# IlzeAmandaA/VAE-GP-ODE

Measured on AMD Instinct MI355X. Metric: latent_trajectories_per_sec, higher is better.
Workload: dtype f32; 1 GPU; configs[1]: ode1 DF q=6 M=100 S=256 T=16 batch=256; step = full ELBO training step (encoder, GP draw, rk4 rollout, decoder, ELBO, backward, Adam), L=1; global_batch=256, mc_draws=1, solver=rk4 (3/8 rule), parallelism=dp1, hip_graph=True, graph_scope=whole, gp_side_stream=True, batchnorm=per-process statistics

## Files before the change

### include/gpode.h

```cpp
#ifndef GPODE_H
#define GPODE_H
#include <stddef.h>
#ifdef __cplusplus
extern "C" {
#endif

#define GPODE_KERNEL_RBF 0
#define GPODE_KERNEL_DF 1
#define GPODE_METHOD_EULER 0
#define GPODE_METHOD_RK4 1
#define GPODE_METHOD_MIDPOINT 2
#define GPODE_METHOD_DOPRI5 3

const char* gpode_version(void);
const char* gpode_last_error(void);
const char* gpode_last_launch(void);
int gpode_supported(int kernel, int Di, int Do);

int gpode_cache_sizes(int kernel, int Di, int Do, int M, int S, size_t* pack_floats, size_t* ws_floats);

int gpode_cache_build_fwd(int kernel, int Di, int Do, int M, int S,
                          const float* raw_ell, const float* raw_var, const float* Z,
                          const float* Um, const float* Us_packed,
                          const float* eps_u, const float* rff_w, const float* rff_eps, const float* rff_u,
// ... 95 lines not shown
                              const float* pack, const float* xstage, const float* gzt, const float* ts, int N, int T,
                              float* gz0, float* astage, float* slab, int nchunk, float* gpack, void* stream);
int gpode_param_grad_n(int kernel, int Di, int Do, int M, int S, int ndraws, const float* pack,
                       const float* x, const float* a, int R, float* slab, int nchunk, float* gpack, int accumulate,
                       void* stream);
int gpode_cache_bwd_sizes_n(int kernel, int Di, int Do, int M, int S, int ndraws, size_t* bws_floats);
int gpode_cache_build_bwd_n(int kernel, int Di, int Do, int M, int S, int ndraws,
                            const float* raw_ell, const float* raw_var, const float* Z, const float* eps_u,
                            const float* pack, const float* ws, float* gpack, float* bws,
                            float* g_raw_ell, float* g_raw_var, float* g_Z, float* g_Um, float* g_Us, int prepared, void* stream);
int gpode_cache_bwd_prepare_n(int kernel, int Di, int Do, int M, int S, int ndraws, const float* ws, float* bws, void* stream);

int gpode_cache_info(const float* ws, int* host_info, void* stream);
int gpode_cache_pivots(const float* ws, float* host_min_max, void* stream);
int gpode_set_backward_solves(int mode);

int gpode_kernel_matrix(int kernel, int Di, int Do, const float* raw_ell, const float* raw_var,
                        const float* X, int N, const float* X2, int M2, float* out, void* stream);

size_t gpode_kern_scratch(int kernel, int Di, int Do, int M, int S);
int gpode_kern_cache(int kernel, int Di, int Do, int S, const float* raw_ell, const float* raw_var, const float* rff_w,
                     const float* rff_eps, const float* rff_u, float* pack, float* omega, float* phase, void* stream);
int gpode_compute_nu_ws(int kernel, int Di, int Do, int M, size_t* ws_floats);
int gpode_compute_nu(int kernel, int Di, int Do, int M, const float* Ku, const float* u_prior, const float* u, float* nu, float* ws,
                     void* stream);
int gpode_f_update(int kernel, int Di, int Do, int M, const float* raw_ell, const float* raw_var, const float* x2, const float* nu,
                   const float* x, int N, float* out, float* scratch, void* stream);

int gpode_conditional_ws(int Di, int Do, int M, int N, size_t* ws_floats);
int gpode_conditional(int Di, int Do, int M, int N, const float* raw_ell, const float* raw_var, const float* Z,
                      const float* Um, const float* Us, int us_rank1, const float* x, int full_cov, float* mean,
                      float* var, float* ws, void* stream);

int gpode_conditional_df_ws(int D, int M, int N, size_t* ws_floats);
int gpode_conditional_df(int D, int M, int N, const float* raw_ell, const float* raw_var, const float* Z, const float* Um,
                         const float* Us_packed, const float* x, int cov_mode, float* mean, float* var, float* ws,
                         void* stream);

int gpode_svgp_kl_fwd(int M, int Do, const float* Um, const float* Us_packed, float* kl, void* stream);
int gpode_svgp_kl_bwd(int M, int Do, const float* Um, const float* Us_packed, const float* g,
                      float* dUm, float* dUs, void* stream);

int gpode_conv2d_fwd(const float* x, const float* w, const float* bias, float* y, int B, int Ci, int H, int W, int Co,
                     int K, int S, int P, int Ho, int Wo, void* stream);
int gpode_conv2d_bwd_data(const float* gy, const float* w, const float* bias, float* gx, int B, int Ci, int H, int W, int Co,
                          int K, int S, int P, int Ho, int Wo, void* stream);
int gpode_conv2d_bwd_data_bn(const float* gy, const float* gy_bn, const float* w, const float* bias, float* gx, int B, int Ci, int H,
                             int W, int Co, int K, int S, int P, int Ho, int Wo, void* stream);
int gpode_conv2d_fwd_bs(const float* x, size_t x_batch_stride, const float* w, const float* bias, float* y, int B, int Ci, int H, int W, int Co,
                        int K, int S, int P, int Ho, int Wo, void* stream);
int gpode_conv2d_bwd_weight_bs(const float* x, size_t x_batch_stride, const float* gy, float* gw, float* gbias, float* scratch, int B, int Ci,
                               int H, int W, int Co, int K, int S, int P, int Ho, int Wo, void* stream);
size_t gpode_convT_fwd_stats_scratch(int Cout);
int gpode_convT_fwd_stats(const float* x, const float* x_bn, const float* w, const float* bias, float* y, int B, int Ci, int H, int W, int Co,
                          int K, int S, int P, int Ho, int Wo, const float* gamma, const float* beta, float* save_mean, float* save_invstd,
                          float* running_mean, float* running_var, long long* num_batches_tracked, float momentum, float eps, float* table,
                          float* scratch, int slot, void* stream);
size_t gpode_conv_wgrad_scratch(int B, int Ci, int Co, int K);
int gpode_conv2d_bwd_weight(const float* x, const float* gy, float* gw, float* gbias, float* scratch, int B, int Ci, int H, int W,
                            int Co, int K, int S, int P, int Ho, int Wo, void* stream);
int gpode_conv2d_bwd_weight_bn(const float* x, const float* gy, const float* gy_bn, float* gw, float* gbias, float* scratch, int B, int Ci,
                               int H, int W, int Co, int K, int S, int P, int Ho, int Wo, void* stream);
size_t gpode_bn_scratch(int B, int C);
int gpode_bn_fwd(const float* x, const float* gamma, const float* beta, float* y, float* save_mean, float* save_invstd,
                 float* running_mean, float* running_var, long long* num_batches_tracked, float momentum, float eps, int B, int C,
                 int HW, int relu, float* scratch, void* stream);
int gpode_bn_bwd(const float* x, const float* gy, const float* gamma, const float* beta, const float* save_mean,
                 const float* save_invstd, float* gx, float* ggamma, float* gbeta, float* gx_chansum, int B, int C, int HW,
                 int relu, float* scratch, void* stream);
int gpode_bn_stats(const float* x, const float* gamma, const float* beta, float* save_mean, float* save_invstd, float* running_mean,
                   float* running_var, long long* num_batches_tracked, float momentum, float eps, float* table, int B, int C, int HW,
                   float* scratch, void* stream);
int gpode_bn_moments(const float* x, float* moments, int B, int C, int HW, float* scratch, void* stream);
int gpode_bn_finalize(const float* gathered, int nranks, const float* gamma, const float* beta, float* save_mean, float* save_invstd,
                      float* running_mean, float* running_var, long long* num_batches_tracked, float momentum, float eps, float* table,
                      int C, void* stream);
int gpode_bn_apply(const float* x, const float* table, float* y, int B, int C, int HW, int relu, void* stream);
int gpode_bn_bwd_sums(const float* x, const float* gy, const float* gamma, const float* beta, const float* save_mean,
                      const float* save_invstd, float* sums, int B, int C, int HW, int relu, float* scratch, void* stream);
int gpode_bn_bwd_apply(const float* x, const float* gy, const float* gamma, const float* beta, const float* save_mean,
                       const float* save_invstd, const float* sums_gathered, const float* weights, int nranks, float count_all,
                       float* gx, float* ggamma, float* gbeta, float* gx_chansum, int B, int C, int HW, int relu, float* scratch,
                       void* stream);
void gpode_defer_reductions(int mode);
int gpode_flush_reductions(void* stream);
int gpode_dec10_bn_wgrad_scratch_floats(void);
int gpode_dec10_bn_bwd_sums_wgrad(const float* c, const float* gy, const float* w, const float* gamma, const float* beta, const float* save_mean,
                                  const float* save_invstd, float* sums, float* gw, float* gbias, int B, float* scratch, float* wscratch,
                                  void* stream);
int gpode_dec10_bn_scratch_floats(void);
int gpode_dec10_bn_bwd_sums(const float* c, const float* gy, const float* w, const float* gamma, const float* beta, const float* save_mean,
                            const float* save_invstd, float* sums, int B, float* scratch, void* stream);
int gpode_dec10_bn_bwd_apply(const float* c, const float* gy, const float* w, const float* gamma, const float* beta, const float* save_mean,
                             const float* save_invstd, const float* sums_gathered, const float* weights, int nranks, float count_all,
                             float* gc, float* ggamma, float* gbeta, float* gc_chansum, int B, float* scratch, void* stream);
int gpode_bn_eval(const float* x, const float* gy, const float* gamma, const float* beta, const float* running_mean,
                  const float* running_var, float eps, float* out, int B, int C, int HW, int relu, void* stream);
int gpode_bn_eval_table(const float* gamma, const float* beta, const float* running_mean, const float* running_var, float eps, float* table,
                        int C, void* stream);
int gpode_dec10_predict(const float* c, const float* table, const float* w, const float* bias, const float* X, int Lc, int F, int Th,
                        int T_obs, int done, float* pred_mean, float* pred_m2, float* se_state, void* stream);
int gpode_dec10_predict_ll(const float* c, const float* table, const float* w, const float* bias, const float* X, int Lc, int F, int Th,
                           int T_obs, int done, float* pred_mean, float* pred_m2, float* se_state, float* ell, int L_total, void* stream);
int gpode_dec10_predict_len(const float* c, const float* table, const float* w, const float* bias, const float* X, int Lc, int F, int Th,
                            int T_obs, int done, float* pred_mean, float* pred_m2, float* se_state, const int* n_obs, void* stream);
int gpode_dec10_predict_ll_len(const float* c, const float* table, const float* w, const float* bias, const float* X, int Lc, int F, int Th,
                               int T_obs, int done, float* pred_mean, float* pred_m2, float* se_state, float* ell, int L_total,
                               const int* n_obs, void* stream);
int gpode_chan_sum(const float* v, float* out, int B, int C, int HW, float* scratch, void* stream);
int gpode_act_fwd(const float* x, float* y, size_t n, int mode, void* stream);
int gpode_act_bwd(const float* y, const float* gy, float* gx, size_t n, int mode, void* stream);
int gpode_linear_fwd(const float* x, const float* w, const float* bias, float* y, int B, int In, int Out, void* stream);
size_t gpode_linear_bwd_scratch(int B, int In, int Out);
int gpode_linear_bwd(const float* x, const float* w, const float* gy, float* gx, float* gw, float* gb, int B, int In, int Out,
                     float* scratch, void* stream);
int gpode_linear_relu_fwd(const float* x, const float* w, const float* bias, float* y, int B, int In, int Out, void* stream);
int gpode_linear_relu_bwd(const float* x, const float* w, const float* gy, float* gx, float* gw, float* gb, int B, int In, int Out,
                          void* stream);

int gpode_loglik_fwd(const float* X, const float* z, float* ll, size_t n, size_t nX, void* stream);
int gpode_loglik_bwd(const float* X, const float* z, const float* g, float* gz, size_t n, size_t nX, void* stream);
int gpode_loglik_rowsum_fwd(const float* X, const float* z, float* out, size_t rows, size_t inner, size_t nX, void* stream);
int gpode_loglik_rowsum_bwd(const float* X, const float* z, const float* grow, float* gz, size_t rows, size_t inner, size_t nX,
                            void* stream);

int gpode_loglik_rowsum_fwd_len(const float* X, const float* z, float* out, size_t rows, size_t inner, size_t nX, const int* n_obs, int T,
                                size_t frame, void* stream);
int gpode_loglik_rowsum_bwd_len(const float* X, const float* z, const float* grow, float* gz, size_t rows, size_t inner, size_t nX,
                                const int* n_obs, int T, size_t frame, void* stream);

int gpode_sigmoid_loglik_splits(size_t rows, size_t inner);
int gpode_sigmoid_loglik_fwd(const float* X, const float* a, float* z, float* part, size_t rows, size_t inner, size_t nX, int nsplit,
                             void* stream);
int gpode_sigmoid_loglik_bwd(const float* X, const float* z, const float* grow, float* ga, size_t rows, size_t inner, size_t nX,
                             void* stream);
int gpode_elbo_all_fwd(const float* lpart, int nl_rows, int nl_values, const float* hs, const float* hv, int N, int q, int M, int Do,
                       const float* Um, const float* Us, float nobs, float* out, void* stream);
int gpode_elbo_all_bwd(const float* g_loss, const float* g_nll, const float* g_kl, const float* g_klu, int nl_rows, const float* hs,
                       const float* hv, int N, int q, int M, int Do, const float* Um, const float* Us, float nobs, float* glrow, float* ghs,
                       float* ghv, float* dUm, float* dUs, void* stream);
int gpode_elbo_all_bwd_ll(const float* g_loss, const float* g_nll, const float* g_kl, const float* g_klu, int nl_rows, const float* hs,
                          const float* hv, int N, int q, int M, int Do, const float* Um, const float* Us, float nobs, float* glrow, float* ghs,
                          float* ghv, float* dUm, float* dUs, const float* X, const float* z, float* ga, size_t n_logits, size_t nX,
                          void* stream);
int gpode_sigmoid_loglik_fwd_len(const float* X, const float* a, float* z, float* part, size_t rows, size_t inner, size_t nX, int nsplit,
                                 const int* n_obs, int T, size_t frame, void* stream);
int gpode_sigmoid_loglik_bwd_len(const float* X, const float* z, const float* grow, float* ga, size_t rows, size_t inner, size_t nX,
                                 const int* n_obs, int T, size_t frame, void* stream);
int gpode_elbo_all_bwd_ll_len(const float* g_loss, const float* g_nll, const float* g_kl, const float* g_klu, int nl_rows, const float* hs,
                              const float* hv, int N, int q, int M, int Do, const float* Um, const float* Us, float nobs, float* glrow, float* ghs,
                              float* ghv, float* dUm, float* dUs, const float* X, const float* z, float* ga, size_t n_logits, size_t nX,
                              const int* n_obs, int T, size_t frame, void* stream);
int gpode_gather_frames_fwd(const float* zt, int ld, int q, const int* src, int L, int N, int T, int P, float* out, void* stream);
int gpode_gather_frames_bwd(const float* gout, int ld, int q, const int* src, const int* off, int L, int N, int T, int P, float* gzt,
                            void* stream);
int gpode_sigmoid_loglik_fwd_pk(const float* X, const float* a, float* z, float* part, size_t rows, const int* off, int T, size_t frame,
                                size_t nX, int nsplit, void* stream);
int gpode_sigmoid_loglik_bwd_pk(const float* X, const float* z, const float* grow, float* ga, size_t rows, const int* src, int P, int T,
                                size_t frame, size_t nX, void* stream);
int gpode_noise_fill(float* out, long long n_normal, long long n_uniform, unsigned long long seed, unsigned long long* state, void* stream);
int gpode_reparam_kl_fwd(const float* mu, const float* logvar, int ld, const float* eps, float* z, float* klpart, int N, int q, void* stream);
int gpode_reparam_kl_bwd(const float* gz, const float* gklpart, const float* mu, const float* logvar, int ld, const float* eps, float* gmu,
                         float* glogvar, int ldg, int N, int q, void* stream);
int gpode_elbo_all_fwd_kl(const float* lpart, int nl_rows, int nl_values, const float* kls, int nks, const float* klv, int nkv, int N, int M,
                          int Do, const float* Um, const float* Us, float nobs, float* out, void* stream);
int gpode_elbo_all_bwd_ll_kl(const float* g_loss, const float* g_nll, const float* g_kl, const float* g_klu, int nl_rows, int N, int M, int Do,
// ... 27 lines not shown
```

### vae-gp-ode_amd/_lib.py

```python
import ctypes
import os

_HERE = os.path.dirname(os.path.abspath(__file__))
LIB_PATH = os.path.join(_HERE, 'libgpode_hip.so')

_vp = ctypes.c_void_p
_i = ctypes.c_int
_f = ctypes.c_float
_sz = ctypes.c_size_t
_sz_p = ctypes.POINTER(_sz)

SIGNATURES = {
    'gpode_version': (ctypes.c_char_p, []),
    'gpode_last_error': (ctypes.c_char_p, []),
    'gpode_last_launch': (ctypes.c_char_p, []),
    'gpode_supported': (_i, [_i, _i, _i]),
    'gpode_cache_sizes': (_i, [_i, _i, _i, _i, _i, _sz_p, _sz_p]),
    'gpode_cache_build_fwd': (_i, [_i] * 5 + [_vp] * 20),
    'gpode_cache_bwd_sizes': (_i, [_i, _i, _i, _i, _i, _sz_p]),
    'gpode_cache_build_bwd': (_i, [_i] * 5 + [_vp] * 13 + [_i, _vp]),
    'gpode_cache_bwd_prepare': (_i, [_i] * 5 + [_vp] * 2 + [_vp]),
    'gpode_cache_info': (_i, [_vp, ctypes.POINTER(_i), _vp]),
    'gpode_cache_pivots': (_i, [_vp, ctypes.POINTER(_f), _vp]),
    'gpode_set_backward_solves': (_i, [_i]),
    'gpode_kernel_matrix': (_i, [_i, _i, _i, _vp, _vp, _vp, _i, _vp, _i, _vp, _vp]),
    'gpode_conditional_ws': (_i, [_i, _i, _i, _i, _sz_p]),
    'gpode_conditional': (_i, [_i, _i, _i, _i] + [_vp] * 5 + [_i, _vp, _i] + [_vp] * 3 + [_vp]),
    'gpode_conditional_df_ws': (_i, [_i, _i, _i, _sz_p]),
    'gpode_conditional_df': (_i, [_i, _i, _i] + [_vp] * 6 + [_i] + [_vp] * 3 + [_vp]),
    'gpode_svgp_kl_fwd': (_i, [_i, _i, _vp, _vp, _vp, _vp]),
    'gpode_svgp_kl_bwd': (_i, [_i, _i] + [_vp] * 5 + [_vp]),
    'gpode_rhs_fwd': (_i, [_i] * 5 + [_vp, _vp, _i, _vp, _i, _vp]),
    'gpode_rollout_fwd': (_i, [_i] * 7 + [_vp, _vp, _vp, _i, _i, _vp, _vp, _vp]),
    'gpode_rollout_bwd': (_i, [_i] * 7 + [_vp] * 4 + [_i, _i, _vp, _vp, _vp]),
    'gpode_rhs_vjp': (_i, [_i] * 5 + [_vp, _vp, _vp, _i, _vp, _vp]),
    'gpode_param_grad': (_i, [_i] * 5 + [_vp, _vp, _vp, _i, _vp, _i, _vp, _i, _vp]),
    'gpode_cache_sizes_n': (_i, [_i] * 6 + [_sz_p, _sz_p]),
    'gpode_cache_build_fwd_n': (_i, [_i] * 6 + [_vp] * 20),
    'gpode_rollout_fwd_n': (_i, [_i] * 8 + [_vp, _vp, _vp, _i, _i, _vp, _vp, _vp]),
    'gpode_rollout_bwd_n': (_i, [_i] * 8 + [_vp] * 4 + [_i, _i, _vp, _vp, _vp]),
    'gpode_rollout_adaptive_fwd_n': (_i, [_i] * 8 + [_vp] * 3 + [_i, _i, _f, _f, _i] + [_vp] * 5 + [_vp]),
    'gpode_rollout_adaptive_bwd_n': (_i, [_i] * 8 + [_vp] * 5 + [_i, _i, _i, _vp, _vp, _vp]),
    'gpode_rollout_dense_fwd_n': (_i, [_i] * 8 + [_vp] * 3 + [_i, _i, _f, _f, _i] + [_vp] * 6 + [_vp]),
    'gpode_rollout_dense_bwd_n': (_i, [_i] * 8 + [_vp] * 6 + [_i, _i, _i, _vp, _vp, _vp]),
    'gpode_rollout_fwd_nz': (_i, [_i] * 8 + [_vp, _vp, _vp, _i, _i, _vp, _vp, _i, _vp]),
    'gpode_rollout_adaptive_fwd_nz': (_i, [_i] * 8 + [_vp] * 3 + [_i, _i, _f, _f, _i] + [_vp] * 5 + [_i, _vp]),
    'gpode_rollout_dense_fwd_nz': (_i, [_i] * 8 + [_vp] * 3 + [_i, _i, _f, _f, _i] + [_vp] * 6 + [_i, _vp]),
    'gpode_rollout_fwd_nt': (_i, [_i] * 8 + [_vp, _vp, _vp, _i, _i, _vp, _vp, _i, _i, _vp]),
    'gpode_rollout_adaptive_fwd_nt': (_i, [_i] * 8 + [_vp] * 3 + [_i, _i, _f, _f, _i] + [_vp] * 5 + [_i, _i, _vp]),
    'gpode_rollout_dense_fwd_nt': (_i, [_i] * 8 + [_vp] * 3 + [_i, _i, _f, _f, _i] + [_vp] * 6 + [_i, _i, _vp]),
    'gpode_rollout_bwd_nt': (_i, [_i] * 8 + [_vp] * 4 + [_i, _i, _vp, _vp, _i, _vp]),
    'gpode_rollout_bwd_pgrad_nt': (_i, [_i] * 8 + [_vp] * 4 + [_i, _i, _vp, _vp, _vp, _i, _vp, _i, _vp]),
    'gpode_test_substep_kernels': (_i, [_i]),
    'gpode_rollout_fwd_ns': (_i, [_i] * 8 + [_vp, _vp, _vp, _i, _i, _vp, _vp, _i, _i, _i, _vp]),
    'gpode_rollout_bwd_ns': (_i, [_i] * 8 + [_vp] * 4 + [_i, _i, _vp, _vp, _i, _i, _vp]),
    'gpode_rollout_bwd_pgrad_ns': (_i, [_i] * 8 + [_vp] * 4 + [_i, _i, _vp, _vp, _vp, _i, _vp, _i, _i, _vp]),
    'gpode_rollout_bwd_pgrad_chunks': (_i, [_i] * 8),
    'gpode_rollout_bwd_pgrad_n': (_i, [_i] * 8 + [_vp] * 4 + [_i, _i, _vp, _vp, _vp, _i, _vp, _vp]),
    'gpode_param_grad_n': (_i, [_i] * 6 + [_vp, _vp, _vp, _i, _vp, _i, _vp, _i, _vp]),
    'gpode_cache_bwd_sizes_n': (_i, [_i] * 6 + [_sz_p]),
    'gpode_cache_build_bwd_n': (_i, [_i] * 6 + [_vp] * 13 + [_i, _vp]),
    'gpode_cache_bwd_prepare_n': (_i, [_i] * 6 + [_vp] * 2 + [_vp]),
    'gpode_kern_scratch': (_sz, [_i] * 5),
    'gpode_kern_cache': (_i, [_i] * 4 + [_vp] * 8 + [_vp]),
    'gpode_compute_nu_ws': (_i, [_i] * 4 + [_sz_p]),
    'gpode_compute_nu': (_i, [_i] * 4 + [_vp] * 5 + [_vp]),
    'gpode_f_update': (_i, [_i] * 4 + [_vp] * 5 + [_i, _vp, _vp, _vp]),
    'gpode_conv2d_fwd': (_i, [_vp] * 4 + [_i] * 10 + [_vp]),
    'gpode_conv2d_bwd_data': (_i, [_vp] * 4 + [_i] * 10 + [_vp]),
    'gpode_conv2d_fwd_bs': (_i, [_vp, _sz] + [_vp] * 3 + [_i] * 10 + [_vp]),
    'gpode_conv2d_bwd_weight_bs': (_i, [_vp, _sz] + [_vp] * 4 + [_i] * 10 + [_vp]),
    'gpode_convT_fwd_stats_scratch': (_sz, [_i]),
    'gpode_convT_fwd_stats': (_i, [_vp] * 5 + [_i] * 10 + [_vp] * 6 + [_vp, _f, _f, _vp, _vp, _i, _vp]),
    'gpode_conv_wgrad_scratch': (_sz, [_i, _i, _i, _i]),
    'gpode_conv2d_bwd_weight': (_i, [_vp] * 5 + [_i] * 10 + [_vp]),
    'gpode_bn_scratch': (_sz, [_i, _i]),
    'gpode_bn_fwd': (_i, [_vp] * 8 + [_vp, _f, _f, _i, _i, _i, _i, _vp, _vp]),
    'gpode_bn_bwd': (_i, [_vp] * 10 + [_i, _i, _i, _i, _vp, _vp]),
    'gpode_conv2d_bwd_data_bn': (_i, [_vp] * 5 + [_i] * 10 + [_vp]),
    'gpode_conv2d_bwd_weight_bn': (_i, [_vp] * 6 + [_i] * 10 + [_vp]),
    'gpode_bn_stats': (_i, [_vp] * 7 + [_vp, _f, _f, _vp, _i, _i, _i, _vp, _vp]),
    'gpode_bn_moments': (_i, [_vp, _vp, _i, _i, _i, _vp, _vp]),
    'gpode_bn_finalize': (_i, [_vp, _i] + [_vp] * 6 + [_vp, _f, _f, _vp, _i, _vp]),
    'gpode_bn_apply': (_i, [_vp, _vp, _vp, _i, _i, _i, _i, _vp]),
    'gpode_bn_bwd_sums': (_i, [_vp] * 7 + [_i, _i, _i, _i, _vp, _vp]),
    'gpode_bn_bwd_apply': (_i, [_vp] * 8 + [_i, _f] + [_vp] * 4 + [_i, _i, _i, _i, _vp, _vp]),
    'gpode_defer_reductions': (None, [_i]),
    'gpode_flush_reductions': (_i, [_vp]),
    'gpode_dec10_bn_scratch_floats': (_i, []),
    'gpode_dec10_bn_wgrad_scratch_floats': (_i, []),
    'gpode_dec10_bn_bwd_sums_wgrad': (_i, [_vp] * 10 + [_i, _vp, _vp, _vp]),
    'gpode_dec10_bn_bwd_sums': (_i, [_vp] * 8 + [_i, _vp, _vp]),
    'gpode_dec10_bn_bwd_apply': (_i, [_vp] * 9 + [_i, _f] + [_vp] * 4 + [_i, _vp, _vp]),
    'gpode_bn_eval': (_i, [_vp] * 6 + [_f, _vp, _i, _i, _i, _i, _vp]),
    'gpode_bn_eval_table': (_i, [_vp] * 4 + [_f, _vp, _i, _vp]),
    'gpode_dec10_predict': (_i, [_vp] * 5 + [_i] * 5 + [_vp] * 3 + [_vp]),
    'gpode_dec10_predict_ll': (_i, [_vp] * 5 + [_i] * 5 + [_vp] * 4 + [_i, _vp]),
    'gpode_chan_sum': (_i, [_vp, _vp, _i, _i, _i, _vp, _vp]),
    'gpode_act_fwd': (_i, [_vp, _vp, _sz, _i, _vp]),
    'gpode_act_bwd': (_i, [_vp, _vp, _vp, _sz, _i, _vp]),
    'gpode_linear_fwd': (_i, [_vp] * 4 + [_i, _i, _i, _vp]),
    'gpode_linear_bwd_scratch': (_sz, [_i, _i, _i]),
    'gpode_linear_bwd': (_i, [_vp] * 6 + [_i, _i, _i, _vp, _vp]),
    'gpode_linear_relu_fwd': (_i, [_vp] * 4 + [_i, _i, _i, _vp]),
    'gpode_linear_relu_bwd': (_i, [_vp] * 6 + [_i, _i, _i, _vp]),
    'gpode_loglik_fwd': (_i, [_vp] * 3 + [_sz, _sz, _vp]),
    'gpode_loglik_bwd': (_i, [_vp] * 4 + [_sz, _sz, _vp]),
    'gpode_loglik_rowsum_fwd': (_i, [_vp] * 3 + [_sz, _sz, _sz, _vp]),
    'gpode_noise_fill': (_i, [_vp, ctypes.c_longlong, ctypes.c_longlong, ctypes.c_ulonglong, _vp, _vp]),
    'gpode_reparam_kl_fwd': (_i, [_vp, _vp, _i, _vp, _vp, _vp, _i, _i, _vp]),
    'gpode_reparam_kl_bwd': (_i, [_vp] * 4 + [_i] + [_vp] * 3 + [_i, _i, _i, _vp]),
    'gpode_elbo_all_fwd_kl': (_i, [_vp, _i, _i, _vp, _i, _vp, _i, _i, _i, _i, _vp, _vp, _f, _vp, _vp]),
    'gpode_elbo_all_bwd_ll_kl': (_i, [_vp] * 4 + [_i, _i, _i, _i, _vp, _vp, _f, _vp, _vp, _i, _vp, _i] + [_vp] * 5 + [_sz, _sz, _vp]),
    'gpode_reparam_fwd': (_i, [_vp, _vp, _i, _vp, _vp, _i, _i, _vp]),
    'gpode_reparam_draws_fwd': (_i, [_vp, _vp, _i, _vp, _vp, _i, _vp, _i, _i, _i, _i, _vp]),
    'gpode_reparam_bwd': (_i, [_vp, _vp, _i, _vp, _vp, _vp, _i, _i, _i, _vp]),
    'gpode_normal_kl_fwd': (_i, [_vp, _vp, _i, _vp, _i, _i, _vp]),
    'gpode_normal_kl_bwd': (_i, [_vp, _vp, _vp, _i, _vp, _vp, _i, _i, _i, _vp]),
    'gpode_sigmoid_loglik_splits': (_i, [_sz, _sz]),
    'gpode_sigmoid_loglik_fwd': (_i, [_vp] * 4 + [_sz, _sz, _sz, _i, _vp]),
    'gpode_sigmoid_loglik_bwd': (_i, [_vp] * 4 + [_sz, _sz, _sz, _vp]),
    'gpode_elbo_all_fwd': (_i, [_vp, _i, _i, _vp, _vp, _i, _i, _i, _i, _vp, _vp, _f, _vp, _vp]),
    'gpode_elbo_all_bwd': (_i, [_vp] * 4 + [_i, _vp, _vp, _i, _i, _i, _i, _vp, _vp, _f] + [_vp] * 5 + [_vp]),
    'gpode_elbo_all_bwd_ll': (_i, [_vp] * 4 + [_i, _vp, _vp, _i, _i, _i, _i, _vp, _vp, _f] + [_vp] * 8 + [_sz, _sz, _vp]),
    'gpode_elbo_fwd': (_i, [_vp, _i, _vp, _i, _vp, _f, _vp, _vp]),
    'gpode_elbo_bwd': (_i, [_vp, _i, _i, _f, _vp, _vp, _vp, _vp]),
    'gpode_gather_multi': (_i, [_vp, _vp, _i, ctypes.c_longlong, _vp, _vp]),
    'gpode_adam_multi': (_i, [_vp, _vp, _vp, _vp, _vp, _i, ctypes.c_longlong, _f, _f, _f, _f, _i, _vp, _vp]),
    'gpode_loglik_rowsum_bwd': (_i, [_vp] * 4 + [_sz, _sz, _sz, _vp]),
    'gpode_sigmoid_loglik_fwd_len': (_i, [_vp] * 4 + [_sz, _sz, _sz, _i, _vp, _i, _sz, _vp]),
    'gpode_sigmoid_loglik_bwd_len': (_i, [_vp] * 4 + [_sz, _sz, _sz, _vp, _i, _sz, _vp]),
    'gpode_loglik_rowsum_fwd_len': (_i, [_vp] * 3 + [_sz, _sz, _sz, _vp, _i, _sz, _vp]),
    'gpode_loglik_rowsum_bwd_len': (_i, [_vp] * 4 + [_sz, _sz, _sz, _vp, _i, _sz, _vp]),
    'gpode_elbo_all_bwd_ll_len': (_i, [_vp] * 4 + [_i, _vp, _vp, _i, _i, _i, _i, _vp, _vp, _f] + [_vp] * 8 + [_sz, _sz, _vp, _i, _sz, _vp]),
    'gpode_elbo_all_bwd_ll_kl_len': (_i, [_vp] * 4 + [_i, _i, _i, _i, _vp, _vp, _f, _vp, _vp, _i, _vp, _i] + [_vp] * 5 + [_sz, _sz, _vp, _i, _sz, _vp]),
    'gpode_gather_frames_fwd': (_i, [_vp, _i, _i, _vp, _i, _i, _i, _i, _vp, _vp]),
    'gpode_gather_frames_bwd': (_i, [_vp, _i, _i, _vp, _vp, _i, _i, _i, _i, _vp, _vp]),
    'gpode_sigmoid_loglik_fwd_pk': (_i, [_vp] * 4 + [_sz, _vp, _i, _sz, _sz, _i, _vp]),
    'gpode_sigmoid_loglik_bwd_pk': (_i, [_vp] * 4 + [_sz, _vp, _i, _i, _sz, _sz, _vp]),
    'gpode_dec10_predict_len': (_i, [_vp] * 5 + [_i] * 5 + [_vp] * 3 + [_vp, _vp]),
    'gpode_dec10_predict_ll_len': (_i, [_vp] * 5 + [_i] * 5 + [_vp] * 4 + [_i, _vp, _vp]),
}

_lib = None


class GpodeError(RuntimeError):
    pass


def load():
    global _lib
    if _lib is not None:
        return _lib
    if not os.path.exists(LIB_PATH):
        raise GpodeError('libgpode_hip.so not found at %s -- build the HIP extension first '
                         '(__graft_entry__.build()); there is no CPU fallback' % LIB_PATH)
    lib = ctypes.CDLL(LIB_PATH)
    for name, (res, args) in SIGNATURES.items():
        fn = getattr(lib, name)
        fn.restype = res
        fn.argtypes = args
    _lib = lib
    return lib


def call(name, *args):
    lib = load()
    rc = getattr(lib, name)(*args)
# ... 4 lines not shown
```

### vae-gp-ode_amd/csrc/bn_math.hpp

```cpp
#pragma once
#include <hip/hip_runtime.h>

namespace gp {

__device__ __forceinline__ float bn_xhat(float x, float m, float is) { return __fmul_rn(__fsub_rn(x, m), is); }
__device__ __forceinline__ float bn_affine(float x, float m, float is, float g, float b) { return __fmaf_rn(bn_xhat(x, m, is), g, b); }
__device__ __forceinline__ float bn_relu(float x, const float4& t) { return fmaxf(bn_affine(x, t.x, t.y, t.z, t.w), 0.f); }

}
```

### vae-gp-ode_amd/csrc/capi.hip

```cpp
#include "../../include/gpode.h"
#include "gp_launch.hpp"

namespace gp {
char* error_slot() {
  static thread_local char buf[512] = {0};
  return buf;
}
const char** last_launch_slot() {
  static thread_local const char* tag = "";
  return &tag;
}
bool* force_substep_kernels() {
  static bool on = false;
  return &on;
}
}

extern "C" {

const char* gpode_version(void) { return "gpode-hip 0.1 (gfx950)"; }
const char* gpode_last_error(void) { return gp::error_slot(); }
const char* gpode_last_launch(void) { return *gp::last_launch_slot(); }
int gpode_supported(int kernel, int Di, int Do) { return gp::dims_supported(kernel, Di, Do); }

// ... 447 lines not shown
  if (!x || !w || !y) return gp::set_error("gpode_conv2d_fwd_bs: null pointer");
  if (x_batch_stride < (size_t)Ci * H * W) return gp::set_error("gpode_conv2d_fwd_bs: images overlap");
  return gp::conv2d_fwd(x, w, bias, y, B, Ci, H, W, Co, K, S, P, Ho, Wo, GP_ST, x_batch_stride);
}
int gpode_conv2d_bwd_weight_bs(const float* x, size_t x_batch_stride, const float* gy, float* gw, float* gbias, float* scratch, int B, int Ci,
                               int H, int W, int Co, int K, int S, int P, int Ho, int Wo, void* stream) {
  if (!x || !gy || !gw || !scratch) return gp::set_error("gpode_conv2d_bwd_weight_bs: null pointer");
  if (x_batch_stride < (size_t)Ci * H * W) return gp::set_error("gpode_conv2d_bwd_weight_bs: images overlap");
  return gp::conv2d_bwd_weight(x, gy, gw, gbias, scratch, B, Ci, H, W, Co, K, S, P, Ho, Wo, nullptr, GP_ST, x_batch_stride);
}
size_t gpode_convT_fwd_stats_scratch(int Cout) { return gp::convT_fwd_stats_scratch(Cout); }
int gpode_convT_fwd_stats(const float* x, const float* x_bn, const float* w, const float* bias, float* y, int B, int Ci, int H, int W, int Co,
                          int K, int S, int P, int Ho, int Wo, const float* gamma, const float* beta, float* save_mean, float* save_invstd,
                          float* running_mean, float* running_var, long long* num_batches_tracked, float momentum, float eps, float* table,
                          float* scratch, int slot, void* stream) {
  if (!x || !w || !y || !gamma || !beta || !save_mean || !save_invstd || !table || !scratch)
    return gp::set_error("gpode_convT_fwd_stats: null pointer");
  if ((running_mean == nullptr) != (running_var == nullptr)) return gp::set_error("gpode_convT_fwd_stats: running_mean and running_var go together");
  return gp::convT_fwd_stats(x, x_bn, w, bias, y, B, Ci, H, W, Co, K, S, P, Ho, Wo, gamma, beta, save_mean, save_invstd, running_mean,
                             running_var, num_batches_tracked, momentum, eps, table, scratch, slot, GP_ST);
}
size_t gpode_conv_wgrad_scratch(int B, int Ci, int Co, int K) { return gp::conv_wgrad_scratch(B, Ci, Co, K); }
int gpode_conv2d_bwd_weight(const float* x, const float* gy, float* gw, float* gbias, float* scratch, int B, int Ci, int H, int W,
                            int Co, int K, int S, int P, int Ho, int Wo, void* stream) {
  if (!x || !gy || !gw || !scratch) return gp::set_error("gpode_conv2d_bwd_weight: null pointer");
  return gp::conv2d_bwd_weight(x, gy, gw, gbias, scratch, B, Ci, H, W, Co, K, S, P, Ho, Wo, nullptr, GP_ST);
}
int gpode_conv2d_bwd_weight_bn(const float* x, const float* gy, const float* gy_bn, float* gw, float* gbias, float* scratch, int B, int Ci,
                               int H, int W, int Co, int K, int S, int P, int Ho, int Wo, void* stream) {
  if (!x || !gy || !gy_bn || !gw || !scratch) return gp::set_error("gpode_conv2d_bwd_weight_bn: null pointer");
  return gp::conv2d_bwd_weight(x, gy, gw, gbias, scratch, B, Ci, H, W, Co, K, S, P, Ho, Wo, gy_bn, GP_ST);
}
size_t gpode_bn_scratch(int B, int C) { return gp::bn_scratch(B, C); }
int gpode_bn_fwd(const float* x, const float* gamma, const float* beta, float* y, float* save_mean, float* save_invstd,
                 float* running_mean, float* running_var, long long* num_batches_tracked, float momentum, float eps, int B, int C,
                 int HW, int relu, float* scratch, void* stream) {
  if (!x || !gamma || !beta || !y || !save_mean || !save_invstd || !scratch) return gp::set_error("gpode_bn_fwd: null pointer");
  return gp::bn_fwd(x, gamma, beta, y, save_mean, save_invstd, running_mean, running_var, num_batches_tracked, momentum, eps, B, C, HW, relu,
                    scratch, GP_ST);
}
int gpode_bn_bwd(const float* x, const float* gy, const float* gamma, const float* beta, const float* save_mean,
                 const float* save_invstd, float* gx, float* ggamma, float* gbeta, float* gx_chansum, int B, int C, int HW,
                 int relu, float* scratch, void* stream) {
  if (!x || !gy || !gamma || !beta || !save_mean || !save_invstd || !gx || !ggamma || !gbeta || !scratch)
    return gp::set_error("gpode_bn_bwd: null pointer");
  return gp::bn_bwd(x, gy, gamma, beta, save_mean, save_invstd, gx, ggamma, gbeta, gx_chansum, B, C, HW, relu, scratch, GP_ST);
}
int gpode_bn_stats(const float* x, const float* gamma, const float* beta, float* save_mean, float* save_invstd, float* running_mean,
                   float* running_var, long long* num_batches_tracked, float momentum, float eps, float* table, int B, int C, int HW,
                   float* scratch, void* stream) {
  if (!x || !gamma || !beta || !save_mean || !save_invstd || !table || !scratch) return gp::set_error("gpode_bn_stats: null pointer");
  return gp::bn_stats(x, gamma, beta, save_mean, save_invstd, running_mean, running_var, num_batches_tracked, momentum, eps, table, B, C, HW,
                      scratch, GP_ST);
}
int gpode_bn_moments(const float* x, float* moments, int B, int C, int HW, float* scratch, void* stream) {
  if (!x || !moments || !scratch) return gp::set_error("gpode_bn_moments: null pointer");
  return gp::bn_moments(x, moments, B, C, HW, scratch, GP_ST);
}
int gpode_bn_finalize(const float* gathered, int nranks, const float* gamma, const float* beta, float* save_mean, float* save_invstd,
                      float* running_mean, float* running_var, long long* num_batches_tracked, float momentum, float eps, float* table,
                      int C, void* stream) {
  if (!gathered || !gamma || !beta || !save_mean || !save_invstd || !table) return gp::set_error("gpode_bn_finalize: null pointer");
  return gp::bn_finalize(gathered, nranks, gamma, beta, save_mean, save_invstd, running_mean, running_var, num_batches_tracked, momentum, eps,
                         table, C, GP_ST);
}
int gpode_bn_apply(const float* x, const float* table, float* y, int B, int C, int HW, int relu, void* stream) {
  if (!x || !table || !y) return gp::set_error("gpode_bn_apply: null pointer");
  return gp::bn_apply(x, table, y, B, C, HW, relu, GP_ST);
}
int gpode_bn_bwd_sums(const float* x, const float* gy, const float* gamma, const float* beta, const float* save_mean,
                      const float* save_invstd, float* sums, int B, int C, int HW, int relu, float* scratch, void* stream) {
  if (!x || !gy || !gamma || !beta || !save_mean || !save_invstd || !sums || !scratch) return gp::set_error("gpode_bn_bwd_sums: null pointer");
  return gp::bn_bwd_sums(x, gy, gamma, beta, save_mean, save_invstd, sums, B, C, HW, relu, scratch, GP_ST);
}
int gpode_bn_bwd_apply(const float* x, const float* gy, const float* gamma, const float* beta, const float* save_mean,
                       const float* save_invstd, const float* sums_gathered, const float* weights, int nranks, float count_all,
                       float* gx, float* ggamma, float* gbeta, float* gx_chansum, int B, int C, int HW, int relu, float* scratch,
                       void* stream) {
  if (!x || !gy || !gamma || !beta || !save_mean || !save_invstd || !sums_gathered || !weights || !gx || !ggamma || !gbeta || !scratch)
    return gp::set_error("gpode_bn_bwd_apply: null pointer");
  return gp::bn_bwd_apply(x, gy, gamma, beta, save_mean, save_invstd, sums_gathered, weights, nranks, count_all, gx, ggamma, gbeta, gx_chansum, B, C, HW, relu,
                          scratch, GP_ST);
}
void gpode_defer_reductions(int mode) { gp::defer_reductions(mode); }
int gpode_flush_reductions(void* stream) { return gp::flush_reductions(GP_ST); }
int gpode_dec10_bn_scratch_floats(void) { return gp::dec10_bn_scratch_floats(); }
int gpode_dec10_bn_bwd_sums(const float* c, const float* gy, const float* w, const float* gamma, const float* beta, const float* save_mean,
                            const float* save_invstd, float* sums, int B, float* scratch, void* stream) {
  if (!c || !gy || !w || !gamma || !beta || !save_mean || !save_invstd || !scratch) return gp::set_error("gpode_dec10_bn_bwd_sums: null pointer");
  if (B < 1) return gp::set_error("gpode_dec10_bn_bwd_sums: B >= 1");
  return gp::dec10_bn_bwd_sums(c, gy, w, gamma, beta, save_mean, save_invstd, sums, B, scratch, GP_ST);
}
int gpode_dec10_bn_wgrad_scratch_floats(void) { return gp::dec10_bn_wgrad_scratch_floats(); }
int gpode_dec10_bn_bwd_sums_wgrad(const float* c, const float* gy, const float* w, const float* gamma, const float* beta, const float* save_mean,
                                  const float* save_invstd, float* sums, float* gw, float* gbias, int B, float* scratch, float* wscratch,
                                  void* stream) {
  if (!c || !gy || !w || !gamma || !beta || !save_mean || !save_invstd || !scratch || !gw || !wscratch)
    return gp::set_error("gpode_dec10_bn_bwd_sums_wgrad: null pointer");
  if (B < 1) return gp::set_error("gpode_dec10_bn_bwd_sums_wgrad: B >= 1");
  return gp::dec10_bn_bwd_sums(c, gy, w, gamma, beta, save_mean, save_invstd, sums, B, scratch, GP_ST, gw, wscratch, gbias);
}
int gpode_dec10_bn_bwd_apply(const float* c, const float* gy, const float* w, const float* gamma, const float* beta, const float* save_mean,
                             const float* save_invstd, const float* sums_gathered, const float* weights, int nranks, float count_all,
                             float* gc, float* ggamma, float* gbeta, float* gc_chansum, int B, float* scratch, void* stream) {
  if (!c || !gy || !w || !gamma || !beta || !save_mean || !save_invstd || !gc || !ggamma || !gbeta || !scratch)
    return gp::set_error("gpode_dec10_bn_bwd_apply: null pointer");
  if (B < 1) return gp::set_error("gpode_dec10_bn_bwd_apply: B >= 1");
  return gp::dec10_bn_bwd_apply(c, gy, w, gamma, beta, save_mean, save_invstd, sums_gathered, weights, nranks, count_all, gc, ggamma, gbeta, gc_chansum,
                                B, scratch, GP_ST);
}
int gpode_bn_eval(const float* x, const float* gy, const float* gamma, const float* beta, const float* running_mean,
                  const float* running_var, float eps, float* out, int B, int C, int HW, int relu, void* stream) {
  if (!x || !gamma || !beta || !running_mean || !running_var || !out) return gp::set_error("gpode_bn_eval: null pointer");
  return gp::bn_eval(x, gy, gamma, beta, running_mean, running_var, eps, out, B, C, HW, relu, GP_ST);
}
int gpode_bn_eval_table(const float* gamma, const float* beta, const float* running_mean, const float* running_var, float eps, float* table,
                        int C, void* stream) {
  if (!gamma || !beta || !running_mean || !running_var || !table) return gp::set_error("gpode_bn_eval_table: null pointer");
  return gp::bn_eval_table(gamma, beta, running_mean, running_var, eps, table, C, GP_ST);
}
int gpode_dec10_predict(const float* c, const float* table, const float* w, const float* bias, const float* X, int Lc, int F, int Th,
                        int T_obs, int done, float* pred_mean, float* pred_m2, float* se_state, void* stream) {
  if (!c || !table || !w || !X || !se_state) return gp::set_error("gpode_dec10_predict: null pointer");
  return gp::dec10_predict(c, table, w, bias, X, Lc, F, Th, T_obs, done, pred_mean, pred_m2, se_state, GP_ST);
}
int gpode_dec10_predict_ll(const float* c, const float* table, const float* w, const float* bias, const float* X, int Lc, int F, int Th,
                           int T_obs, int done, float* pred_mean, float* pred_m2, float* se_state, float* ell, int L_total, void* stream) {
  if (!c || !table || !w || !X || !se_state) return gp::set_error("gpode_dec10_predict_ll: null pointer");
  return gp::dec10_predict_ll(c, table, w, bias, X, Lc, F, Th, T_obs, done, pred_mean, pred_m2, se_state, ell, L_total, GP_ST);
}
int gpode_dec10_predict_len(const float* c, const float* table, const float* w, const float* bias, const float* X, int Lc, int F, int Th,
                            int T_obs, int done, float* pred_mean, float* pred_m2, float* se_state, const int* n_obs, void* stream) {
  if (!c || !table || !w || !X || !se_state) return gp::set_error("gpode_dec10_predict_len: null pointer");
  return gp::dec10_predict_len(c, table, w, bias, X, Lc, F, Th, T_obs, done, pred_mean, pred_m2, se_state, n_obs, GP_ST);
}
int gpode_dec10_predict_ll_len(const float* c, const float* table, const float* w, const float* bias, const float* X, int Lc, int F, int Th,
                               int T_obs, int done, float* pred_mean, float* pred_m2, float* se_state, float* ell, int L_total,
                               const int* n_obs, void* stream) {
  if (!c || !table || !w || !X || !se_state) return gp::set_error("gpode_dec10_predict_ll_len: null pointer");
  return gp::dec10_predict_ll_len(c, table, w, bias, X, Lc, F, Th, T_obs, done, pred_mean, pred_m2, se_state, ell, L_total, n_obs, GP_ST);
}
int gpode_chan_sum(const float* v, float* out, int B, int C, int HW, float* scratch, void* stream) {
  if (!v || !out || !scratch) return gp::set_error("gpode_chan_sum: null pointer");
  return gp::chan_sum(v, out, B, C, HW, scratch, GP_ST);
}
int gpode_act_fwd(const float* x, float* y, size_t n, int mode, void* stream) { return gp::act_fwd(x, y, n, mode, GP_ST); }
int gpode_act_bwd(const float* y, const float* gy, float* gx, size_t n, int mode, void* stream) { return gp::act_bwd(y, gy, gx, n, mode, GP_ST); }
int gpode_linear_fwd(const float* x, const float* w, const float* bias, float* y, int B, int In, int Out, void* stream) {
  if (!x || !w || !y) return gp::set_error("gpode_linear_fwd: null pointer");
  return gp::linear_fwd(x, w, bias, y, B, In, Out, GP_ST);
}
size_t gpode_linear_bwd_scratch(int B, int In, int Out) { return gp::linear_bwd_scratch(B, In, Out); }
int gpode_linear_bwd(const float* x, const float* w, const float* gy, float* gx, float* gw, float* gb, int B, int In, int Out,
                     float* scratch, void* stream) {
  if (!x || !w || !gy) return gp::set_error("gpode_linear_bwd: null pointer");
  return gp::linear_bwd(x, w, gy, gx, gw, gb, B, In, Out, scratch, GP_ST);
}
int gpode_linear_relu_fwd(const float* x, const float* w, const float* bias, float* y, int B, int In, int Out, void* stream) {
  if (!x || !w || !y) return gp::set_error("gpode_linear_relu_fwd: null pointer");
  return gp::linear_relu_fwd(x, w, bias, y, B, In, Out, GP_ST);
}
int gpode_linear_relu_bwd(const float* x, const float* w, const float* gy, float* gx, float* gw, float* gb, int B, int In, int Out,
                          void* stream) {
  if (!x || !w || !gy) return gp::set_error("gpode_linear_relu_bwd: null pointer");
  return gp::linear_relu_bwd(x, w, gy, gx, gw, gb, B, In, Out, GP_ST);
}
// ... 201 lines not shown
```

### vae-gp-ode_amd/csrc/conv_bwd_v2.hpp

```cpp
#pragma once
#include "conv_mfma.hpp"

namespace gp {

template <class L> struct BdV2 {
  using PL = BwdDataPolicy<L, L::CI>;
  static constexpr int KC = L::CO, NC = L::CI, KK = L::K * L::K;
  static constexpr int NCT = NC / 16;
  static constexpr int NKS = KK * (KC / 4);
  static constexpr int NPX = L::HI * L::HI;
  static constexpr int SRC = KC * L::HO * L::HO;
  static constexpr int PS = PL::PS, HP = PL::HP, IMG = KC * PS;
  static constexpr int CPS = NKS <= 100 ? 2 : 1;
  static constexpr int NCW = 4 * CPS, NTHR = 64 * (NCW + 4), NLT = NTHR - 64 * NCW;
  static constexpr int TSPLIT = NCW / NCT;
  static constexpr int TPW = CPS == 2 ? 2 : 4;
  static constexpr int WIN = 16 * TSPLIT * TPW;
  static constexpr int PF = 2;
  static constexpr int NTMIN = CPS == 2 ? 1 : TPW;
  static constexpr int NBUF = (2 * WIN - 2) / NPX + 2;
  static_assert(NCW % NCT == 0 && TSPLIT * NCT == NCW, "the consumers split the ci tiles evenly");
  static_assert(TPW * (PF + 1) <= 15, "LDS reads in flight within what lgkmcnt counts");
  static_assert(KC % 4 == 0 && SRC % 4 == 0, "float4 source");
  static constexpr bool ROW4 = L::HO % 4 == 0;
  static_assert(ROW4 || L::HO * L::HO <= NLT, "producer offset table");
  static constexpr int koff(int s) { return (s / (KC / 4)) / L::K * HP + (s / (KC / 4)) % L::K + (s % (KC / 4)) * 4 * PS; }
  static_assert(4 * koff(NKS - 1) < 65536, "operand offsets fit the ds_read immediate");
  static constexpr size_t lds_bytes() { return sizeof(float) * (size_t)NBUF * IMG; }
};

template <class E, int NT>
__device__ __forceinline__ void bdv2_tiles(const float* __restrict__ s_buf, const int (&base)[E::TPW], const float (&wr)[E::NKS],
                                           f32x4 (&acc)[E::TPW]) {
  float bf[E::PF + 1][NT];
  auto fetch = [&](auto sc) {
    constexpr int s = decltype(sc)::value;
#pragma unroll
    for (int t = 0; t < NT; ++t) bf[s % (E::PF + 1)][t] = s_buf[base[t] + E::koff(s)];
  };
#pragma unroll
  for (int t = 0; t < NT; ++t) acc[t] = f32x4{0.f, 0.f, 0.f, 0.f};
  static_for<E::PF>([&](auto sc) { fetch(sc); });
  static_for<E::NKS>([&](auto sc) {
    constexpr int s = decltype(sc)::value;
    if constexpr (s + E::PF < E::NKS) fetch(std::integral_constant<int, s + E::PF>{});
    __builtin_amdgcn_sched_barrier(0);
#pragma unroll
    for (int t = 0; t < NT; ++t) acc[t] = __builtin_amdgcn_mfma_f32_16x16x4f32(wr[s], bf[s % (E::PF + 1)][t], acc[t], 0, 0, 0);
    __builtin_amdgcn_sched_barrier(0);
  });
}

template <class E, int NT>
__device__ __forceinline__ void bdv2_window(int nt, const float* __restrict__ s_buf, const int (&base)[E::TPW], const float (&wr)[E::NKS],
                                            f32x4 (&acc)[E::TPW]) {
  if constexpr (NT > E::NTMIN) {
    if (nt < NT) { bdv2_window<E, NT - 1>(nt, s_buf, base, wr, acc); return; }
  }
  bdv2_tiles<E, NT>(s_buf, base, wr, acc);
}

template <class L>
__global__ __launch_bounds__(BdV2<L>::NTHR) void k_conv_bwd_data_v2(const float* __restrict__ gy, const float* __restrict__ w,
                                                                    float* __restrict__ gx, int B) {
  using E = BdV2<L>;
  using PL = typename E::PL;
  constexpr int KC = E::KC, NC = E::NC, KK = E::KK, NPX = E::NPX, IMG = E::IMG, PS = E::PS, HP = E::HP, WIN = E::WIN, NKS = E::NKS;
  constexpr int HO = L::HO, P = L::P, NLT = E::NLT, NBUF = E::NBUF, TPW = E::TPW, TSPLIT = E::TSPLIT;
  float* s_buf = igemm_smem;
  const int tid = threadIdx.x, lane = tid & 63, wave = __builtin_amdgcn_readfirstlane(tid >> 6);
  const int nit = ((int)blockIdx.x < B) ? (B - 1 - (int)blockIdx.x) / (int)gridDim.x + 1 : 0;
  const int npx = nit * NPX, nwin = (npx + WIN - 1) / WIN;
  auto last_img = [&](int i) { return min(nit - 1, (i * WIN + WIN - 1) / NPX); };

  for (int e = tid; e < NBUF * IMG / 4; e += E::NTHR) reinterpret_cast<float4*>(s_buf)[e] = float4{0.f, 0.f, 0.f, 0.f};
  __syncthreads();

  if (wave >= E::NCW) {
    __builtin_amdgcn_s_setprio(3);
    const int lt = tid - 64 * E::NCW;
    constexpr int N4 = E::SRC / 4;
    int otab[4];
#pragma unroll
    for (int k = 0; k < 4; ++k) {
      const int e = 4 * min(lt, HO * HO - 1) + k, pl = e / (HO * HO), q = e % (HO * HO);
      otab[k] = pl * PS + (q / HO + P) * HP + q % HO + P;
    }
    auto stage = [&](int j) __attribute__((always_inline)) {
      const float4* src = reinterpret_cast<const float4*>(gy) + (size_t)((int)blockIdx.x + j * (int)gridDim.x) * N4;
      float* buf = s_buf + (j % NBUF) * IMG;
      if constexpr (E::ROW4) {
        constexpr int NLD = (N4 + NLT - 1) / NLT;
        float4 v[NLD];
#pragma unroll
        for (int i = 0; i < NLD; ++i) v[i] = src[min(lt + NLT * i, N4 - 1)];
#pragma unroll
        for (int i = 0; i < NLD; ++i) {
          const int f = lt + NLT * i;
          const int pl = (4 * f) / (HO * HO), q = (4 * f) % (HO * HO), row = q / HO, col = q % HO;
          float* d = buf + pl * PS + (row + P) * HP + col + P;
          if (f < N4) { d[0] = v[i].x; d[1] = v[i].y; d[2] = v[i].z; d[3] = v[i].w; }
        }
      } else if (lt < HO * HO) {
        float4 v[KC / 4];
#pragma unroll
        for (int g = 0; g < KC / 4; ++g) v[g] = src[g * HO * HO + lt];
#pragma unroll
        for (int g = 0; g < KC / 4; ++g) {
          float* d = buf + 4 * g * PS;
          d[otab[0]] = v[g].x; d[otab[1]] = v[g].y; d[otab[2]] = v[g].z; d[otab[3]] = v[g].w;
        }
      }
    };
    int staged = -1;
    if (nit > 0)
      for (; staged < last_img(0); ) stage(++staged);
    __syncthreads();
    for (int i = 0; i < nwin; ++i) {
      if (i + 1 < nwin)
        for (const int j1 = last_img(i + 1); staged < j1; ) stage(++staged);
      __syncthreads();
    }
    return;
  }

  const int lr = lane & 15, lk = lane >> 4, ct = wave / TSPLIT, sm = wave % TSPLIT;
  float wr[NKS];
#pragma unroll
  for (int s = 0; s < NKS; ++s) wr[s] = w[((size_t)(16 * ct + lr) * KC + 4 * (s % (KC / 4)) + lk) * KK + s / (KC / 4)];
  __syncthreads();
  for (int i = 0; i < nwin; ++i) {
    const int t0 = i * WIN + 16 * sm;
    int base[TPW], mm[TPW];
#pragma unroll
    for (int t = 0; t < TPW; ++t) {
      mm[t] = t0 + 16 * TSPLIT * t + lr;
      const int m = min(mm[t], npx - 1);
      const int j = m / NPX, p = m - j * NPX;
      base[t] = (j % NBUF) * IMG + lk * PS + PL::template C<0>::pix_addr(p);
    }
    f32x4 acc[TPW];
    const int nt = t0 < npx ? min(TPW, (npx - t0 + 16 * TSPLIT - 1) / (16 * TSPLIT)) : 0;
    if (nt > 0) bdv2_window<E, TPW>(nt, s_buf, base, wr, acc);
#pragma unroll
    for (int t = 0; t < TPW; ++t) {
      if (t < nt && mm[t] < npx) {
        const int j = mm[t] / NPX, p = mm[t] - j * NPX;
        float* o = gx + ((size_t)((int)blockIdx.x + j * (int)gridDim.x) * NC + 16 * ct + 4 * lk) * NPX + p;
#pragma unroll
        for (int r = 0; r < 4; ++r) o[(size_t)r * NPX] = acc[t][r];
      }
    }
    __syncthreads();
  }
}

}
```

### vae-gp-ode_amd/csrc/conv_wgrad_v2.hpp

```cpp
#pragma once
#include "conv_mfma.hpp"
#ifndef WGV2_PRIO
#define WGV2_PRIO 3
#endif

namespace gp {

template <class L> constexpr size_t wgrad_v2_lds_floats(bool gtab) {
  return (size_t)2 * (WgradGeo<L>::IMGX + WgradGeo<L>::IMGG) + (size_t)4 * L::CI + (size_t)4 * (WgradGeo<L>::NKS + 1) +
         (gtab ? (size_t)L::CO * L::HO * L::HO : 0);
}

template <class L> struct WgV2 {
  using G = WgradGeo<L>;
  static constexpr int MT = L::CI / 16, NT = L::CO / 16, KK = L::K * L::K, NUA = KK * MT * NT, NCW = 8;
  static constexpr int ustart(int w) {
    int s = 0;
    for (int i = 0; i < w; ++i) s += NUA / NCW + (i < NUA % NCW ? 1 : 0);
    return s;
  }
  static constexpr int tap_of(int u) { return u / (MT * NT); }
  static constexpr int mt_of(int u) { return (u / NT) % MT; }
  static constexpr int nt_of(int u) { return u % NT; }
  static constexpr bool uses_a(int ub, int ue, int mt) {
    for (int u = ub; u < ue; ++u) if (mt_of(u) == mt) return true;
    return false;
  }
  static constexpr bool uses_b(int ub, int ue, int tap, int nt) {
    for (int u = ub; u < ue; ++u) if (tap_of(u) == tap && nt_of(u) == nt) return true;
    return false;
  }
  static constexpr int toff(int t) {
    return L::S == 2 ? ((t % L::K) & 1) * G::HPL + (t / L::K) * G::GPH + ((t % L::K) >> 1) : (t / L::K) * G::GPH + t % L::K;
  }
};

template <class L, int UB, int UE, bool PIPE>
__device__ __forceinline__ void wgrad_v2_image(const float* __restrict__ s_x, const float* __restrict__ s_g, const int* __restrict__ s_tab,
                                               int lr, int lk, f32x4 (&acc)[UE - UB]) {
  using W = WgV2<L>;
  using G = typename W::G;
  constexpr int MT = W::MT, NT = W::NT, T0 = W::tap_of(UB), T1 = W::tap_of(UE - 1), NTP = T1 - T0 + 1;
  constexpr int NKS = G::NKS, PSX = G::PSX, PSG = G::PSG;
  float afA[MT], bfA[NTP][NT], afB[MT], bfB[NTP][NT];
  const float* xq = s_x + lr * PSX + lk;
  const float* gq = s_g + lr * PSG;
  const int* tq = s_tab + lk;
  auto fetch = [&](const float* __restrict__ xp, const float* __restrict__ gp, float (&af)[MT], float (&bf)[NTP][NT]) {
    static_for<MT>([&](auto m) {
      constexpr int mt = decltype(m)::value;
#ifdef WGV2_NOLDS
      if constexpr (W::uses_a(UB, UE, mt)) af[mt] = __int_as_float((int)(size_t)xp + mt);
#else
      if constexpr (W::uses_a(UB, UE, mt)) af[mt] = xp[mt * 16 * PSX];
#endif
    });
    static_for<NTP>([&](auto tt) {
      static_for<NT>([&](auto nn) {
        constexpr int tp = decltype(tt)::value, nt = decltype(nn)::value;
#ifdef WGV2_NOLDS
        if constexpr (W::uses_b(UB, UE, T0 + tp, nt)) bf[tp][nt] = __int_as_float((int)(size_t)gp + tp * 2 + nt);
#else
        if constexpr (W::uses_b(UB, UE, T0 + tp, nt)) bf[tp][nt] = gp[nt * 16 * PSG + W::toff(T0 + tp)];
#endif
      });
    });
  };
  auto mma = [&](const float (&af)[MT], const float (&bf)[NTP][NT]) {
    static_for<UE - UB>([&](auto j) {
      constexpr int u = UB + decltype(j)::value;
      acc[u - UB] = __builtin_amdgcn_mfma_f32_16x16x4f32(af[W::mt_of(u)], bf[W::tap_of(u) - T0][W::nt_of(u)], acc[u - UB], 0, 0, 0);
    });
  };
  if constexpr (PIPE) {
    int g1 = tq[4];
    fetch(xq, gq + tq[0], afA, bfA);
    int s = 0;
#pragma nounroll
    for (; s + 2 < NKS; s += 2) {
      fetch(xq + 4 * (s + 1), gq + g1, afB, bfB);
      const int g2 = tq[4 * (s + 2)];
      __builtin_amdgcn_sched_barrier(0);
      mma(afA, bfA);
      __builtin_amdgcn_sched_barrier(0);
      fetch(xq + 4 * (s + 2), gq + g2, afA, bfA);
      g1 = tq[4 * (s + 3)];
      __builtin_amdgcn_sched_barrier(0);
      mma(afB, bfB);
      __builtin_amdgcn_sched_barrier(0);
    }
    if (NKS % 2 == 0) {
      fetch(xq + 4 * (s + 1), gq + g1, afB, bfB);
      __builtin_amdgcn_sched_barrier(0);
      mma(afA, bfA);
      mma(afB, bfB);
    } else {
      mma(afA, bfA);
    }
  } else {
#pragma nounroll
    for (int s = 0; s < NKS; ++s) {
      fetch(xq + 4 * s, gq + tq[4 * s], afA, bfA);
      mma(afA, bfA);
    }
  }
}

template <class L, int WV, bool PIPE>
__device__ __forceinline__ void wgrad_v2_consumer(const float* __restrict__ s_buf, const int* __restrict__ s_tab, int nit, int lane,
                                                  float* __restrict__ pp) {
  using W = WgV2<L>;
  using G = typename W::G;
  constexpr int UB = W::ustart(WV), UE = W::ustart(WV + 1), IMG = G::IMGX + G::IMGG;
  const int lr = lane & 15, lk = lane >> 4;
  f32x4 acc[UE - UB];
#pragma unroll
  for (int j = 0; j < UE - UB; ++j) acc[j] = f32x4{0.f, 0.f, 0.f, 0.f};
  __syncthreads();
#ifdef WGV2_PROBE
  long long t_mma = 0, t_bar = 0, t0 = clock64();
  const long long c_start = __builtin_amdgcn_s_memtime(), r_start = __builtin_amdgcn_s_memrealtime();
#endif
#pragma nounroll
  for (int it = 0; it < nit; ++it) {
    const float* cur = s_buf + (it & 1) * IMG;
    wgrad_v2_image<L, UB, UE, PIPE>(cur, cur + G::IMGX, s_tab, lr, lk, acc);
#ifdef WGV2_PROBE
    { const long long t = clock64(); t_mma += t - t0; t0 = t; }
#endif
    __syncthreads();
#ifdef WGV2_PROBE
    { const long long t = clock64(); t_bar += t - t0; t0 = t; }
#endif
  }
#ifdef WGV2_PROBE
  if (blockIdx.x == 0 && lane == 0) {
    const long long dc = __builtin_amdgcn_s_memtime() - c_start, dr = __builtin_amdgcn_s_memrealtime() - r_start;
    printf("wgrad_v2 consumer %d: %d images, mma %lld cycles, barrier wait %lld; loop %lld cycles in %lld ticks of 100 MHz = %.0f MHz\n", WV, nit,
           t_mma, t_bar, dc, dr, 100.0 * (double)dc / (double)dr);
  }
#endif
#pragma unroll
  for (int j = 0; j < UE - UB; ++j)
#pragma unroll
    for (int r = 0; r < 4; ++r) pp[((size_t)(UB + j) * 4 + r) * 64 + lane] = acc[j][r];
}

template <class L, bool HAS_BN, bool PIPE>
__global__ __launch_bounds__(768) void k_convT_wgrad_v2(const float* __restrict__ x, const float* __restrict__ gy,
                                                         float* __restrict__ part, int B, const float* __restrict__ in_bn) {
  using W = WgV2<L>;
  using G = typename W::G;
  constexpr int CI = L::CI, CO = L::CO, HO = L::HO, S = L::S, P = L::P, KK = W::KK;
  constexpr int NPIX = G::NPIX, PSX = G::PSX, PSG = G::PSG, GPH = G::GPH, HPL = G::HPL, IMGX = G::IMGX, IMGG = G::IMGG;
  constexpr int IMG = IMGX + IMGG;
  constexpr int SRCX = CI * NPIX, SRCG = CO * HO * HO, NTHR = 768, NLT = 256;
  static_assert(SRCX % 4 == 0 && SRCG % 4 == 0 && IMG % 4 == 0, "float4 access");
  float* s_buf = igemm_smem;
  float4* s_tf = reinterpret_cast<float4*>(igemm_smem + 2 * IMG);
  int* s_tab = reinterpret_cast<int*>(igemm_smem + 2 * IMG + 4 * CI);
  constexpr bool GTAB = !(S == 2 && HO % 4 == 0 && P == 1) && wgrad_v2_lds_floats<L>(true) * sizeof(float) <= 160 * 1024;
  int* s_gtab = s_tab + 4 * (G::NKS + 1);
  const int tid = threadIdx.x, lane = tid & 63, wave = __builtin_amdgcn_readfirstlane(tid >> 6);
  const bool producer = wave >= W::NCW;
  const int lt = tid - 64 * W::NCW;
  if (HAS_BN)
    for (int e = tid; e < CI; e += NTHR) s_tf[e] = reinterpret_cast<const float4*>(in_bn)[e];
  if (GTAB)
    for (int e = tid; e < SRCG; e += NTHR) {
      const int pl = e / (HO * HO), q = e % (HO * HO), rr = q / HO + P, cc = q % HO + P;
      s_gtab[e] = pl * PSG + (S == 2 ? (cc & 1) * HPL + rr * GPH + (cc >> 1) : rr * GPH + cc);
    }
  for (int p = tid; p < 4 * (G::NKS + 1); p += NTHR) {
    const int pc = min(p, NPIX - 1), iy = pc / L::HI, ix = pc % L::HI;
    s_tab[p] = S == 2 ? S * iy * GPH + ix : iy * GPH + ix;
  }
  for (int e = tid; e < 2 * IMG / 4; e += NTHR) reinterpret_cast<float4*>(s_buf)[e] = float4{0.f, 0.f, 0.f, 0.f};
  const int nit = ((int)blockIdx.x < B) ? (B - 1 - (int)blockIdx.x) / (int)gridDim.x + 1 : 0;

  __syncthreads();
  if (producer) {
    __builtin_amdgcn_s_setprio(WGV2_PRIO);
    constexpr int CH = 4, NX4 = SRCX / 4, NG4 = SRCG / 4, NCX = (NX4 + NLT * CH - 1) / (NLT * CH), NCG = (NG4 + NLT * CH - 1) / (NLT * CH);
    auto load = [&](const float4* __restrict__ src, int n4, int c, float4 (&v)[CH]) __attribute__((always_inline)) {
#pragma unroll
      for (int i = 0; i < CH; ++i) v[i] = src[min(lt + NLT * (c * CH + i), n4 - 1)];
    };
    auto scatter_x = [&](float* __restrict__ s_x, int c, const float4 (&vv)[CH]) __attribute__((always_inline)) {
#pragma unroll
      for (int i = 0; i < CH; ++i) {
        const int f = lt + NLT * (c * CH + i);
        const float v[4] = {vv[i].x, vv[i].y, vv[i].z, vv[i].w};
        const bool on = f < NX4;
        int pl = (4 * f) / NPIX, q = (4 * f) % NPIX;
        const int pl0 = min(pl, CI - 1);
        float4 tf0 = float4{0.f, 0.f, 0.f, 0.f}, tf1 = tf0;
        if (HAS_BN) { tf0 = s_tf[pl0]; if (NPIX % 4 != 0) tf1 = s_tf[min(pl0 + 1, CI - 1)]; }
        if constexpr (NPIX % 4 == 0) {
          float* base = s_x + pl * PSX + q;
          if (on) {
#pragma unroll
            for (int k = 0; k < 4; ++k) base[k] = HAS_BN ? bn_relu(v[k], tf0) : v[k];
          }
        } else {
#pragma unroll
          for (int k = 0; k < 4; ++k) {
            if (on) s_x[pl * PSX + q] = HAS_BN ? bn_relu(v[k], pl == pl0 ? tf0 : tf1) : v[k];
            if (k < 3) { if (++q == NPIX) { q = 0; ++pl; } }
          }
        }
      }
    };
    auto scatter_g = [&](float* __restrict__ s_g, int c, const float4 (&vv)[CH]) __attribute__((always_inline)) {
#pragma unroll
      for (int i = 0; i < CH; ++i) {
        const int f = lt + NLT * (c * CH + i);
        const float v[4] = {vv[i].x, vv[i].y, vv[i].z, vv[i].w};
        const bool on = f < NG4;
        int pl = (4 * f) / (HO * HO), q = (4 * f) % (HO * HO), row = q / HO, col = q % HO;
        if constexpr (S == 2 && HO % 4 == 0 && P == 1) {
          float* base = s_g + pl * PSG + (row + P) * GPH + (col >> 1);
          if (on) { base[HPL] = v[0]; base[1] = v[1]; base[HPL + 1] = v[2]; base[2] = v[3]; }
        } else if constexpr (GTAB) {
          const int4 o = reinterpret_cast<const int4*>(s_gtab)[min(f, NG4 - 1)];
          if (on) { s_g[o.x] = v[0]; s_g[o.y] = v[1]; s_g[o.z] = v[2]; s_g[o.w] = v[3]; }
        } else {
#pragma unroll
          for (int k = 0; k < 4; ++k) {
            const int rr = row + P, cc = col + P;
            if (on) s_g[pl * PSG + (S == 2 ? (cc & 1) * HPL + rr * GPH + (cc >> 1) : rr * GPH + cc)] = v[k];
            if (HO % 4 != 0 || k < 3) { if (++col == HO) { col = 0; if (++row == HO) { row = 0; ++pl; } } }
          }
        }
      }
    };
    auto stage = [&](int img, float* __restrict__ buf) __attribute__((always_inline)) {
      const float4* sx = reinterpret_cast<const float4*>(x) + (size_t)img * NX4;
      const float4* sg = reinterpret_cast<const float4*>(gy) + (size_t)img * NG4;
      float4 va[CH], vb[CH];
      load(sx, NX4, 0, va);
      static_for<NCX>([&](auto cc) {
        constexpr int c = decltype(cc)::value;
        float4 (&cur)[CH] = (c % 2 == 0) ? va : vb;
        float4 (&nxt)[CH] = (c % 2 == 0) ? vb : va;
        if constexpr (c + 1 < NCX) load(sx, NX4, c + 1, nxt);
        else load(sg, NG4, 0, nxt);
        scatter_x(buf, c, cur);
      });
      float4 (&g0)[CH] = (NCX % 2 == 0) ? va : vb;
      float4 (&g1)[CH] = (NCX % 2 == 0) ? vb : va;
#pragma nounroll
      for (int c = 0; c < NCG; c += 2) {
        if (c + 1 < NCG) load(sg, NG4, c + 1, g1);
        scatter_g(buf + IMGX, c, g0);
        if (c + 1 < NCG) {
          if (c + 2 < NCG) load(sg, NG4, c + 2, g0);
          scatter_g(buf + IMGX, c + 1, g1);
        }
      }
    };
    if (nit > 0) stage(blockIdx.x, s_buf);
    __syncthreads();
#ifdef WGV2_PROBE
    long long t_st = 0, t_bar = 0, t0 = clock64();
#endif
    for (int it = 0; it < nit; ++it) {
#ifdef WGV2_NOPROD
      if (it + 1 < 2)
#endif
      if (it + 1 < nit) stage(blockIdx.x + (it + 1) * gridDim.x, s_buf + ((it + 1) & 1) * IMG);
#ifdef WGV2_PROBE
      { const long long t = clock64(); t_st += t - t0; t0 = t; }
#endif
      __syncthreads();
#ifdef WGV2_PROBE
      { const long long t = clock64(); t_bar += t - t0; t0 = t; }
#endif
    }
#ifdef WGV2_PROBE
    if (blockIdx.x == 0 && lane == 0) printf("wgrad_v2 producer %d: stage %lld cycles, barrier wait %lld\n", wave, t_st, t_bar);
#endif
    return;
  }
  float* pp = part + (size_t)blockIdx.x * CI * CO * KK;
  switch (wave) {
    case 0: wgrad_v2_consumer<L, 0, PIPE>(s_buf, s_tab, nit, lane, pp); break;
    case 1: wgrad_v2_consumer<L, 1, PIPE>(s_buf, s_tab, nit, lane, pp); break;
    case 2: wgrad_v2_consumer<L, 2, PIPE>(s_buf, s_tab, nit, lane, pp); break;
    case 3: wgrad_v2_consumer<L, 3, PIPE>(s_buf, s_tab, nit, lane, pp); break;
    case 4: wgrad_v2_consumer<L, 4, PIPE>(s_buf, s_tab, nit, lane, pp); break;
    case 5: wgrad_v2_consumer<L, 5, PIPE>(s_buf, s_tab, nit, lane, pp); break;
    case 6: wgrad_v2_consumer<L, 6, PIPE>(s_buf, s_tab, nit, lane, pp); break;
    default: wgrad_v2_consumer<L, 7, PIPE>(s_buf, s_tab, nit, lane, pp); break;
  }
}

template <class L> constexpr size_t wgrad_v2_lds_bytes() {
  constexpr bool gtab = !(L::S == 2 && L::HO % 4 == 0 && L::P == 1) && wgrad_v2_lds_floats<L>(true) * sizeof(float) <= 160 * 1024;
  return sizeof(float) * wgrad_v2_lds_floats<L>(gtab);
}

}
```

### vae-gp-ode_amd/csrc/gp_launch.hpp

```cpp
#pragma once
#include <cstdint>
#include <cstdlib>
#include <hip/hip_runtime.h>
#include <cstdarg>
#include <cstdio>
#include <mutex>
#include <unordered_map>

namespace gp {

char* error_slot();
const char** last_launch_slot();

inline int set_error(const char* fmt, ...) {
  va_list ap;
  va_start(ap, fmt);
  vsnprintf(error_slot(), 512, fmt, ap);
  va_end(ap);
  return 1;
}

inline int check_launch(const char* what) {
  *last_launch_slot() = what;
  hipError_t e = hipGetLastError();
// ... 65 lines not shown
                      const float* xstage, const float* hstep, const int* istep, const float* theta, const float* gzt, int N, int T,
                      int K, float* gz0, float* astage, hipStream_t st);
int rhs_vjp(int kernel, int Di, int Do, int M, int S, const float* pack, const float* x, const float* a, int R, float* gx,
            int prior_only, hipStream_t st, Draws dw = Draws{});
int param_grad(int kernel, int Di, int Do, int M, int S, const float* pack, const float* xr, const float* ar, int R,
               float* slab, int nchunk, float* gpack, int accumulate, int prior_only, hipStream_t st, Draws dw = Draws{});
int cache_sizes(int kernel, int Di, int Do, int M, int S, size_t* pack_floats, size_t* ws_floats, int nd = 1);
int cache_build_fwd(int kernel, int Di, int Do, int M, int S, int nd,
                    const float* raw_ell, const float* raw_var, const float* Z, const float* Um, const float* Us_packed,
                    const float* eps_u, const float* rff_w, const float* rff_eps, const float* rff_u,
                    float* pack, float* ws, float* ell, float* var, float* omega, float* phase, float* u,
                    float* Lu, float* nu, float* u_prior, hipStream_t st);

size_t kern_scratch_floats(int kernel, int Di, int Do, int M, int S);
int kern_cache(int kernel, int Di, int Do, int S, const float* raw_ell, const float* raw_var, const float* rff_w, const float* rff_eps,
               const float* rff_u, float* pack, float* omega, float* phase, hipStream_t st);
int compute_nu_ws(int kernel, int Di, int Do, int M, size_t* ws_floats);
int compute_nu(int kernel, int Di, int Do, int M, const float* Ku, const float* u_prior, const float* u, float* nu, float* ws, hipStream_t st);
int f_update(int kernel, int Di, int Do, int M, const float* raw_ell, const float* raw_var, const float* x2, const float* nu,
             const float* x, int N, float* out, float* pack, hipStream_t st);
int kernel_matrix(int kernel, int Di, int Do, const float* raw_ell, const float* raw_var, const float* X, int N,
                  const float* X2, int M2, float* out, hipStream_t st);
int conditional_ws(int Di, int Do, int M, int N, size_t* ws_floats);
int conditional(int Di, int Do, int M, int N, const float* raw_ell, const float* raw_var, const float* Z, const float* Um,
                const float* Us_packed, int us_rank1, const float* x, int full_cov, float* mean, float* var, float* ws, hipStream_t st);
int conditional_df_ws(int D, int M, int N, size_t* ws_floats);
int conditional_df(int D, int M, int N, const float* raw_ell, const float* raw_var, const float* Z, const float* Um,
                   const float* Us_packed, const float* x, int cov_mode, float* mean, float* var, float* ws, hipStream_t st);
int svgp_kl_fwd(int M, int Do, const float* Um, const float* Us, float* kl, hipStream_t st);
int noise_fill(float* out, long long n_normal, long long n_uniform, unsigned long long seed, unsigned long long* state, hipStream_t st);
int svgp_kl_bwd(int M, int Do, const float* Um, const float* Us, const float* g, float* dUm, float* dUs, hipStream_t st);

void set_backward_solves(int mode);
int get_backward_solves();
int cache_bwd_sizes(int kernel, int Di, int Do, int M, int S, int nd, size_t* bws_floats);
int cache_build_bwd(int kernel, int Di, int Do, int M, int S, int nd, const float* raw_ell, const float* raw_var, const float* Z,
                    const float* eps_u, const float* pack, const float* ws, float* gpack, float* bws,
                    float* g_raw_ell, float* g_raw_var, float* g_Z, float* g_Um, float* g_Us, int prepared, hipStream_t st);
int cache_bwd_prepare(int kernel, int Di, int Do, int M, int S, int nd, const float* ws, float* bws, hipStream_t st);

int conv2d_fwd(const float* x, const float* w, const float* bias, float* y, int B, int Ci, int H, int W, int Co, int K, int S,
               int P, int Ho, int Wo, hipStream_t st, size_t xbs = 0);
size_t convT_fwd_stats_scratch(int Co_out);
int convT_fwd_stats(const float* x, const float* x_bn, const float* w, const float* bias, float* y, int B, int Ci, int H, int W, int Co, int K,
                    int S, int P, int Ho, int Wo, const float* gamma, const float* beta, float* save_mean, float* save_invstd,
                    float* running_mean, float* running_var, long long* nbt, float momentum, float eps, float* table, float* scratch,
                    int slot, hipStream_t st);
int conv2d_bwd_data(const float* gy, const float* w, const float* bias, float* gx, int B, int Ci, int H, int W, int Co, int K, int S,
                    int P, int Ho, int Wo, const float* gy_bn, hipStream_t st);
size_t conv_wgrad_scratch(int B, int Ci, int Co, int K);
int conv2d_bwd_weight(const float* x, const float* gy, float* gw, float* gbias, float* scratch, int B, int Ci, int H, int W, int Co,
                      int K, int S, int P, int Ho, int Wo, const float* gy_bn, hipStream_t st, size_t xbs = 0);
size_t bn_scratch(int B, int C);
int bn_fwd(const float* x, const float* gamma, const float* beta, float* y, float* save_mean, float* save_invstd,
           float* running_mean, float* running_var, long long* num_batches_tracked, float momentum, float eps, int B, int C, int HW,
           int relu, float* scratch, hipStream_t st);
int bn_bwd(const float* x, const float* gy, const float* gamma, const float* beta, const float* save_mean, const float* save_invstd,
           float* gx, float* ggamma, float* gbeta, float* gx_chansum, int B, int C, int HW, int relu, float* scratch, hipStream_t st);
int bn_stats(const float* x, const float* gamma, const float* beta, float* save_mean, float* save_invstd, float* running_mean,
             float* running_var, long long* num_batches_tracked, float momentum, float eps, float* table, int B, int C, int HW,
             float* scratch, hipStream_t st);
int bn_moments(const float* x, float* mom, int B, int C, int HW, float* scratch, hipStream_t st);
int bn_finalize(const float* gathered, int W, const float* gamma, const float* beta, float* save_mean, float* save_invstd,
                float* running_mean, float* running_var, long long* num_batches_tracked, float momentum, float eps, float* table, int C,
                hipStream_t st);
int bn_apply(const float* x, const float* table, float* y, int B, int C, int HW, int relu, hipStream_t st);
int dec10_bn_scratch_floats();
int dec10_bn_bwd_sums(const float* c, const float* gy, const float* w, const float* gamma, const float* beta, const float* mean,
                      const float* invstd, float* sums, int B, float* scratch, hipStream_t st, float* gw = nullptr, float* wscratch = nullptr, float* gbias = nullptr);
int dec10_bn_wgrad_scratch_floats();
int dec10_bn_bwd_apply(const float* c, const float* gy, const float* w, const float* gamma, const float* beta, const float* mean,
                       const float* invstd, const float* gathered, const float* wts, int W, float count_all, float* gc, float* ggamma,
                       float* gbeta, float* gc_chansum, int B, float* scratch, hipStream_t st);
struct RedJob { const float* part; float* out; int nsplit, n, kind, a, b, c; };
int reduce_job(const RedJob& job, hipStream_t st);
int reduce_jobs(const RedJob* jobs, int nj, hipStream_t st);
void defer_reductions(int mode);
int flush_reductions(hipStream_t st);
int bn_bwd_sums(const float* x, const float* gy, const float* gamma, const float* beta, const float* save_mean, const float* save_invstd,
                float* sums, int B, int C, int HW, int relu, float* scratch, hipStream_t st);
int bn_bwd_apply(const float* x, const float* gy, const float* gamma, const float* beta, const float* save_mean, const float* save_invstd,
                 const float* gathered, const float* wts, int W, float count, float* gx, float* ggamma, float* gbeta, float* gx_chansum, int B, int C, int HW, int relu,
                 float* scratch, hipStream_t st);
int bn_eval(const float* x, const float* gy, const float* gamma, const float* beta, const float* running_mean, const float* running_var,
            float eps, float* out, int B, int C, int HW, int relu, hipStream_t st);
int bn_eval_table(const float* gamma, const float* beta, const float* running_mean, const float* running_var, float eps, float* table, int C,
                  hipStream_t st);
int dec10_predict(const float* c, const float* table, const float* w, const float* bias, const float* X, int Lc, int F, int Th, int T_obs,
                  int done, float* pred_mean, float* pred_m2, float* se_state, hipStream_t st);
int dec10_predict_ll(const float* c, const float* table, const float* w, const float* bias, const float* X, int Lc, int F, int Th, int T_obs,
                     int done, float* pred_mean, float* pred_m2, float* se_state, float* ell, int L_total, hipStream_t st);
int chan_sum(const float* v, float* out, int B, int C, int HW, float* scratch, hipStream_t st);
int act_fwd(const float* x, float* y, size_t n, int mode, hipStream_t st);
int act_bwd(const float* y, const float* gy, float* gx, size_t n, int mode, hipStream_t st);
int linear_fwd(const float* x, const float* w, const float* bias, float* y, int B, int In, int Out, hipStream_t st);
int linear_bwd(const float* x, const float* w, const float* gy, float* gx, float* gw, float* gb, int B, int In, int Out, float* scratch, hipStream_t st);
size_t linear_bwd_scratch(int B, int In, int Out);
int linear_relu_fwd(const float* x, const float* w, const float* bias, float* y, int B, int In, int Out, hipStream_t st);
int linear_relu_bwd(const float* x, const float* w, const float* gy, float* gx, float* gw, float* gb, int B, int In, int Out, hipStream_t st);
int loglik_fwd(const float* X, const float* z, float* ll, size_t n, size_t nX, hipStream_t st);
int loglik_bwd(const float* X, const float* z, const float* g, float* gz, size_t n, size_t nX, hipStream_t st);
int loglik_rowsum_fwd(const float* X, const float* z, float* out, size_t rows, size_t inner, size_t nX, hipStream_t st);
int loglik_rowsum_bwd(const float* X, const float* z, const float* grow, float* gz, size_t rows, size_t inner, size_t nX, hipStream_t st);
int elbo_all_bwd_ll(const float* g0, const float* g1, const float* g2, const float* g3, int nl_rows, const float* hs, const float* hv, int N,
                    int q, int M, int Do, const float* Um, const float* Us, float nobs, float* glrow, float* ghs, float* ghv, float* dUm,
                    float* dUs, const float* X, const float* z, float* ga, size_t n, size_t nX, hipStream_t st);
int reparam_kl_fwd(const float* mu, const float* logvar, int ld, const float* eps, float* z, float* klpart, int N, int q, hipStream_t st);
int reparam_kl_bwd(const float* gz, const float* gklpart, const float* mu, const float* logvar, int ld, const float* eps, float* gmu,
                   float* glogvar, int ldg, int N, int q, hipStream_t st);
int elbo_all_fwd_kl(const float* lpart, int nl_rows, int nl_values, const float* kls, int nks, const float* klv, int nkv, int N, int M, int Do,
                    const float* Um, const float* Us, float nobs, float* out, hipStream_t st);
int elbo_all_bwd_ll_kl(const float* g0, const float* g1, const float* g2, const float* g3, int nl_rows, int N, int M, int Do, const float* Um,
                       const float* Us, float nobs, float* glrow, float* gkls, int nks, float* gklv, int nkv, float* dUm, float* dUs,
                       const float* X, const float* z, float* ga, size_t n, size_t nX, hipStream_t st);
int reparam_fwd(const float* mu, const float* logvar, int ld, const float* eps, float* z, int N, int q, hipStream_t st);
int reparam_draws_fwd(const float* mu, const float* logvar, int ld, const float* eps, float* z, int ldz, float* lw, int accumulate, int L, int N,
                      int q, hipStream_t st);
int reparam_bwd(const float* gz, const float* logvar, int ld, const float* eps, float* gmu, float* glogvar, int ldg, int N, int q, hipStream_t st);
int normal_kl_fwd(const float* mu, const float* logvar, int ld, float* klrow, int N, int q, hipStream_t st);
int normal_kl_bwd(const float* grow, const float* mu, const float* logvar, int ld, float* gmu, float* glogvar, int ldg, int N, int q, hipStream_t st);
int sigmoid_loglik_splits(size_t rows, size_t inner);
int sigmoid_loglik_fwd(const float* X, const float* a, float* z, float* part, size_t rows, size_t inner, size_t nX, int nsplit, hipStream_t st);
int sigmoid_loglik_bwd(const float* X, const float* z, const float* grow, float* ga, size_t rows, size_t inner, size_t nX, hipStream_t st);
int elbo_all_fwd(const float* lpart, int nl_rows, int nl_values, const float* hs, const float* hv, int N, int q, int M, int Do,
                 const float* Um, const float* Us, float nobs, float* out, hipStream_t st);
int elbo_all_bwd(const float* g0, const float* g1, const float* g2, const float* g3, int nl_rows, const float* hs, const float* hv, int N,
                 int q, int M, int Do, const float* Um, const float* Us, float nobs, float* glrow, float* ghs, float* ghv, float* dUm,
                 float* dUs, hipStream_t st);
int sigmoid_loglik_fwd_len(const float* X, const float* a, float* z, float* part, size_t rows, size_t inner, size_t nX, int nsplit,
                           const int* n_obs, int T, size_t frame, hipStream_t st);
int sigmoid_loglik_bwd_len(const float* X, const float* z, const float* grow, float* ga, size_t rows, size_t inner, size_t nX,
                           const int* n_obs, int T, size_t frame, hipStream_t st);
int loglik_rowsum_fwd_len(const float* X, const float* z, float* out, size_t rows, size_t inner, size_t nX, const int* n_obs, int T,
                          size_t frame, hipStream_t st);
int loglik_rowsum_bwd_len(const float* X, const float* z, const float* grow, float* gz, size_t rows, size_t inner, size_t nX,
                          const int* n_obs, int T, size_t frame, hipStream_t st);
int elbo_all_bwd_ll_len(const float* g0, const float* g1, const float* g2, const float* g3, int nl_rows, const float* hs, const float* hv, int N,
                        int q, int M, int Do, const float* Um, const float* Us, float nobs, float* glrow, float* ghs, float* ghv, float* dUm,
                        float* dUs, const float* X, const float* z, float* ga, size_t n, size_t nX, const int* n_obs, int T, size_t frame,
                        hipStream_t st);
int elbo_all_bwd_ll_kl_len(const float* g0, const float* g1, const float* g2, const float* g3, int nl_rows, int N, int M, int Do, const float* Um,
                           const float* Us, float nobs, float* glrow, float* gkls, int nks, float* gklv, int nkv, float* dUm, float* dUs,
                           const float* X, const float* z, float* ga, size_t n, size_t nX, const int* n_obs, int T, size_t frame,
                           hipStream_t st);
int gather_frames_fwd(const float* zt, int ld, int q, const int* src, int L, int N, int T, int P, float* out, hipStream_t st);
int gather_frames_bwd(const float* gout, int ld, int q, const int* off, int L, int N, int T, int P, float* gzt, hipStream_t st);
int sigmoid_loglik_fwd_pk(const float* X, const float* a, float* z, float* part, size_t rows, const int* off, int T, size_t frame, size_t nX,
                          int nsplit, hipStream_t st);
int sigmoid_loglik_bwd_pk(const float* X, const float* z, const float* grow, float* ga, size_t rows, const int* src, int P, int T, size_t frame,
                          size_t nX, hipStream_t st);
int dec10_predict_len(const float* c, const float* table, const float* w, const float* bias, const float* X, int Lc, int F, int Th, int T_obs,
                      int done, float* pred_mean, float* pred_m2, float* se_state, const int* n_obs, hipStream_t st);
int dec10_predict_ll_len(const float* c, const float* table, const float* w, const float* bias, const float* X, int Lc, int F, int Th, int T_obs,
                         int done, float* pred_mean, float* pred_m2, float* se_state, float* ell, int L_total, const int* n_obs,
                         hipStream_t st);
int elbo_fwd(const float* lhood, int nl, const float* klrow, int nk, const float* kl_u, float nobs, float* out, hipStream_t st);
int elbo_bwd(const float* gout, int nl, int nk, float nobs, float* glhood, float* gklrow, float* gklu, hipStream_t st);
int gather_multi(const float* const* grads, const long long* offs, int ntensors, long long total, float* flat, hipStream_t st);
int adam_multi(float* const* params, const float* const* grads, float* const* m1, float* const* m2, const long long* offs,
               int ntensors, long long total, float lr, float beta1, float beta2, float eps, int step, int* step_dev, hipStream_t st);

inline bool big_factor(int np) {
  static const bool off = env_flag("GPODE_SMALL_FACTOR_KERNELS");
  return !off && np % 128 == 0 && np >= 1024;
}

// ... 2 lines not shown
```

### vae-gp-ode_amd/csrc/vae_conv_tiled.hip

```cpp
#include <hip/hip_runtime.h>
#include <cstdlib>
#include "gp_launch.hpp"
#include "conv_layers.hpp"
#include "conv_mfma.hpp"
#include "conv_dec10_mfma.hpp"
#include "conv_dec1_mfma.hpp"
#include "conv_dec4_mfma.hpp"

namespace gp {

extern __shared__ __attribute__((aligned(16))) float tsm[];

template <class L, int IPB>
__global__ __launch_bounds__(256) void k_convT_fwd(const float* __restrict__ x, const float* __restrict__ w,
                                                    const float* __restrict__ bias, float* __restrict__ y, int B) {
  constexpr int CI = L::CI, CO = L::CO, HI = L::HI, HO = L::HO, HP = L::HP, K = L::K, S = L::S, P = L::P, PL = L::PL;
  constexpr int CPT = CO % 16 == 0 ? 16 : 8;
  static_assert(CO % CPT == 0, "8 or 16 output channels per thread");
  constexpr int NG = CO / CPT;
  constexpr int IMG = CI * HP * HP;
  float* s_img = tsm;
  float* s_w = tsm + IPB * IMG;
  const int tid = threadIdx.x;
  const int b0 = blockIdx.x * IPB;
// ... 601 lines not shown
    if (ipb == 4) rc = launch_dec10_bn<4, 0, true>(B, st, gy, w, c, gamma, beta, mean, invstd, B, scratch, 0, 0.f, cnp, cnp, 0, np_, np_, np_, np_, wscratch, part_b);
    else rc = launch_dec10_bn<2, 0, true>(B, st, gy, w, c, gamma, beta, mean, invstd, B, scratch, 0, 0.f, cnp, cnp, 0, np_, np_, np_, np_, wscratch, part_b);
    if (!rc) {
      const RedJob jobs[2] = {RedJob{wscratch, gw, nwg, dec10::CI * dec10::KK, 0, 0, 0, 0}, RedJob{part_b, gbias, nwg, 1, 0, 0, 0, 0}};
      if (reduce_jobs(jobs, gbias ? 2 : 1, st)) return 1;
    }
  } else if (ipb == 4) rc = launch_dec10_bn<4, 0>(B, st, gy, w, c, gamma, beta, mean, invstd, B, scratch, 0, 0.f, cnp, cnp, 0, np_, np_, np_, np_, np_, np_);
  else rc = launch_dec10_bn<2, 0>(B, st, gy, w, c, gamma, beta, mean, invstd, B, scratch, 0, 0.f, cnp, cnp, 0, np_, np_, np_, np_, np_, np_);
  if (rc) return rc;
  if (sums) hipLaunchKernelGGL(k_dec10_parts_reduce, 1, 512, 0, st, scratch, nwg, sums, 1);
  return check_launch(gw ? "dec10_bn_bwd_sums_wgrad" : "dec10_bn_bwd_sums");
}

int dec10_bn_bwd_apply(const float* c, const float* gy, const float* w, const float* gamma, const float* beta, const float* mean,
                       const float* invstd, const float* gathered, const float* wts, int W, float count_all, float* gc, float* ggamma,
                       float* gbeta, float* gc_chansum, int B, float* scratch, hipStream_t st) {
  if (!aligned16(gy, c, gc))
    return set_error("gpode_dec10_bn_bwd_apply: c / gy / gc must be 16-byte aligned");
  if (gathered && (W < 1 || !wts)) return set_error("gpode_dec10_bn_bwd_apply: gathered sums need their weights");
  int ipb;
  const int nwg = dec10_bn_nwg(B, ipb);
  float* part_gx = gc_chansum ? scratch + (size_t)kDec10BnMaxWg * dec10::CI * 2 : nullptr;
  const float count = gathered ? count_all : (float)B * dec10::NP;
  int rc;
  if (ipb == 4) rc = launch_dec10_bn<4, 1>(B, st, gy, w, c, gamma, beta, mean, invstd, B, scratch, nwg, count, gathered, wts, W, ggamma, gbeta, gc, part_gx, (float*)nullptr, (float*)nullptr);
  else rc = launch_dec10_bn<2, 1>(B, st, gy, w, c, gamma, beta, mean, invstd, B, scratch, nwg, count, gathered, wts, W, ggamma, gbeta, gc, part_gx, (float*)nullptr, (float*)nullptr);
  if (rc) return rc;
  if (gc_chansum && reduce_job(RedJob{part_gx, gc_chansum, nwg, dec10::CI, 2, 0, 0, 0}, st)) return 1;
  return check_launch("dec10_bn_bwd_apply");
}

int wgrad_v2_dec7(const float* x, const float* gy, float* gw, float* scratch, int B, hipStream_t st, const float* in_bn);
int wgrad_v2_dec4(const float* x, const float* gy, float* gw, float* scratch, int B, hipStream_t st, const float* in_bn);

int tiled_bwd_weight(const float* x, const float* gy, float* gw, float* scratch, int B, int Ci, int H, int W, int Co, int K, int S,
                     int P, int Ho, int Wo, const float* in_bn, hipStream_t st) {
  if (H != W || Ho != Wo) return -1;
  const bool mfma = use_mfma() && aligned16(x, gy, in_bn);
  if (matches<Dec7>(Ci, Co, H, Ho, K, S, P)) {
    if (mfma) return wgrad_v2_dec7(gy, x, gw, scratch, B, st, in_bn);
    return launch_T3<Dec7, 16>(gy, x, gw, scratch, B, st, in_bn);
  }
  if (matches<Dec4>(Ci, Co, H, Ho, K, S, P)) {
    if (mfma) return wgrad_v2_dec4(gy, x, gw, scratch, B, st, in_bn);
    return launch_T3<Dec4, 16>(gy, x, gw, scratch, B, st, in_bn);
  }
  if (matches<Dec1>(Ci, Co, H, Ho, K, S, P)) {
    if (!in_bn && mfma) {
      const size_t lds = sizeof(float) * 2 * dec1::GYF;
      const int cap = 2 * num_cus() < 256 ? 2 * num_cus() : 256;
      const int nwg = B < cap ? B : cap;
      hipLaunchKernelGGL(dec1::k_wgrad, nwg, 256, lds, st, gy, x, scratch, B);
      if (reduce_job(RedJob{scratch, gw, nwg, dec1::CI * dec1::NN, 0, 0, 0, 0}, st)) return 1;
      return check_launch("dec1_wgrad_mfma");
    }
    if (mfma) return launch_wgrad_mfma<Dec1, 2, 4, 1>(gy, x, gw, scratch, B, st, in_bn);
    return launch_T3<Dec1, 32>(gy, x, gw, scratch, B, st, in_bn);
  }
  if (matches<Enc6>(Ci, Co, H, Ho, K, S, P) && mfma)
    return launch_wgrad_mfma<Enc6, 2, 1, 4>(gy, x, gw, scratch, B, st, in_bn);
  if (matches<Dec10>(Ci, Co, H, Ho, K, S, P) && mfma) {
    constexpr int IPB = 1;
    const size_t fl = (size_t)IPB * dec10::PLANE > 8 * 16 * 32 ? (size_t)IPB * dec10::PLANE : 8 * 16 * 32;
    const int ngroups = (B + IPB - 1) / IPB;
    const int nwg = ngroups < num_cus() ? ngroups : num_cus();
    hipLaunchKernelGGL(dec10::k_wgrad<IPB>, nwg, 512, sizeof(float) * fl, st, gy, x, scratch, B, in_bn);
    if (reduce_job(RedJob{scratch, gw, nwg, 400, 0, 0, 0, 0}, st)) return 1;
    return check_launch("dec10_wgrad_mfma");
  }
  if (matches<Dec10>(Ci, Co, H, Ho, K, S, P)) {
    if (in_bn) return set_error("convT weight gradient with a fused BatchNorm input needs the matrix-core path (16-byte aligned operands, GPODE_CONV_VALU unset)");
    int nsplit = B < 256 ? B : 256;
    const int bps = (B + nsplit - 1) / nsplit;
    nsplit = (B + bps - 1) / bps;
    const size_t lds = sizeof(float) * (16 * 785 + 32 * 32);
    if (set_max_lds((const void*)k_dec10_wgrad, lds)) return 1;
    hipLaunchKernelGGL(k_dec10_wgrad, nsplit, 256, lds, st, gy, x, scratch, B, bps);
    if (reduce_job(RedJob{scratch, gw, nsplit, 400, 0, 0, 0, 0}, st)) return 1;
    return check_launch("dec10_wgrad");
  }
  return -1;
}

}
```

### vae-gp-ode_amd/csrc/vae_conv_v2.hip

```cpp
#include <hip/hip_runtime.h>
#include <cstdint>
#include "gp_launch.hpp"
#include "conv_layers.hpp"
#include "conv_bwd_v2.hpp"
#include "conv_fwd_v2.hpp"

namespace gp {

template <class L> static int launch_bwd_data_v2(const float* gy, const float* w, float* gx, int B, hipStream_t st, const char* what) {
  using E = BdV2<L>;
  constexpr size_t lds = E::lds_bytes();
  static_assert(lds <= 160 * 1024, "LDS budget");
  auto km = k_conv_bwd_data_v2<L>;
  if (set_max_lds((const void*)km, lds)) return 1;
  hipLaunchKernelGGL(km, B < num_cus() ? B : num_cus(), E::NTHR, lds, st, gy, w, gx, B);
  return check_launch(what);
}

int conv_v2_dec7_bwd_data(const float* gy, const float* w, float* gx, int B, hipStream_t st) {
  return launch_bwd_data_v2<Dec7>(gy, w, gx, B, st, "conv_v2_dec7_bwd_data");
}

int conv_v2_dec4_bwd_data(const float* gy, const float* w, float* gx, int B, hipStream_t st) {
  return launch_bwd_data_v2<Dec4>(gy, w, gx, B, st, "conv_v2_dec4_bwd_data");
}

template <class L, bool HAS_BN, bool STATS>
static int launch_fwd_v2(const float* x, const float* w, const float* bias, float* y, int B, const float* in_bn, const BnSink* sink,
                         hipStream_t st, const char* what) {
  using E = FwV2<L>;
  constexpr size_t lds = E::lds_bytes(STATS);
  static_assert(lds + (STATS ? sizeof(float) * (E::NTHR + 1) : 0) <= 160 * 1024, "LDS budget (with bn_sink_publish's static arrays)");
  auto km = k_conv_fwd_v2<L, HAS_BN, STATS>;
  if (set_max_lds((const void*)km, lds)) return 1;
  if (STATS && num_cus() > 512) return set_error("%s: more workgroups than the statistics scratch holds", what);
  const int nwork = STATS ? (B + E::IPG - 1) / E::IPG : B;
  hipLaunchKernelGGL(km, nwork < num_cus() ? nwork : num_cus(), E::NTHR, lds, st, x, w, bias, y, B, in_bn, STATS ? *sink : BnSink{});
  return check_launch(what);
}

int conv_v2_dec7_fwd(const float* x, const float* w, const float* bias, float* y, int B, const float* in_bn, const BnSink* sink,
                     hipStream_t st) {
  if (in_bn && sink) return launch_fwd_v2<Dec7, true, true>(x, w, bias, y, B, in_bn, sink, st, "conv_v2_dec7_fwd_bn_stats");
  if (sink) return launch_fwd_v2<Dec7, false, true>(x, w, bias, y, B, in_bn, sink, st, "conv_v2_dec7_fwd_stats");
  if (in_bn) return launch_fwd_v2<Dec7, true, false>(x, w, bias, y, B, in_bn, sink, st, "conv_v2_dec7_fwd_bn");
  return launch_fwd_v2<Dec7, false, false>(x, w, bias, y, B, in_bn, sink, st, "conv_v2_dec7_fwd");
}

}
```

### vae-gp-ode_amd/csrc/vae_norm.hip

```cpp
#include <hip/hip_runtime.h>
#include <mutex>
#include "gp_launch.hpp"
#include "wave_reduce.hpp"
#include "bn_math.hpp"

namespace gp {

namespace {

template <class F4, class F1>
__device__ __forceinline__ void chan_slab(int C, int HW, int c, int b0, int nb, F4&& f4, F1&& f1) {
  if ((HW & 3) == 0) {
    const int hw4 = HW >> 2, work = nb * hw4;
    int q = threadIdx.x, b = q / hw4, p = q - b * hw4;
    const int sb = 256 / hw4, sp = 256 - sb * hw4;
#pragma unroll 4
    for (; q < work; q += 256) {
      f4(((size_t)(b0 + b) * C + c) * HW + 4 * p);
      p += sp; b += sb;
      if (p >= hw4) { p -= hw4; ++b; }
    }
  } else {
    const int work = nb * HW;
    int q = threadIdx.x, b = q / HW, p = q - b * HW;
    const int sb = 256 / HW, sp = 256 - sb * HW;
#pragma unroll 4
    for (; q < work; q += 256) {
      f1(((size_t)(b0 + b) * C + c) * HW + p);
      p += sp; b += sb;
      if (p >= HW) { p -= HW; ++b; }
    }
  }
}

template <int NV> __device__ __forceinline__ void block_sum_store(const float (&v)[NV], float* __restrict__ dst) {
  __shared__ float red[4][NV];
  float out[NV];
  wave_sum_multi<NV>(v, out);
  if ((threadIdx.x & 63) == 0) {
#pragma unroll
    for (int i = 0; i < NV; ++i) red[threadIdx.x >> 6][i] = out[i];
  }
  __syncthreads();
  if (threadIdx.x < NV) dst[threadIdx.x] = (red[0][threadIdx.x] + red[1][threadIdx.x]) + (red[2][threadIdx.x] + red[3][threadIdx.x]);
}

__device__ __forceinline__ void split_sums(const float* __restrict__ part, int nsplit, int C, int c, float& a, float& b) {
  const int lane = threadIdx.x & 63;
  const float in2[2] = {lane < nsplit ? part[((size_t)lane * C + c) * 2] : 0.f, lane < nsplit ? part[((size_t)lane * C + c) * 2 + 1] : 0.f};
  float out2[2];
  wave_sum_multi<2>(in2, out2);
  a = out2[0];
  b = out2[1];
}

__device__ __forceinline__ float chan_shift(const float* __restrict__ x, int HW, int c) {
  const int n = HW < 64 ? HW : 64, lane = threadIdx.x & 63;
  const float in1[1] = {lane < n ? x[(size_t)c * HW + lane] : 0.f};
  float out1[1];
  wave_sum_multi<1>(in1, out1);
  return out1[0] / (float)n;
}

__global__ __launch_bounds__(256) void k_bn_stats(const float* __restrict__ x, int B, int C, int HW, int bps, float* __restrict__ part,
                                                   float* __restrict__ shift) {
  const int c = blockIdx.x, b0 = blockIdx.y * bps, nb = min(B, b0 + bps) - b0;
  const float k = chan_shift(x, HW, c);
  float s0 = 0.f, s1 = 0.f, t0 = 0.f, t1 = 0.f;
  chan_slab(C, HW, c, b0, nb,
            [&](size_t i) {
              const float4 v = *reinterpret_cast<const float4*>(x + i);
              const float a = v.x - k, b = v.y - k, d = v.z - k, e = v.w - k;
              s0 += a; t0 += b; s0 += d; t0 += e;
              s1 = fmaf(a, a, s1); t1 = fmaf(b, b, t1); s1 = fmaf(d, d, s1); t1 = fmaf(e, e, t1);
            },
            [&](size_t i) {
              const float a = x[i] - k;
              s0 += a;
              s1 = fmaf(a, a, s1);
            });
  const float in2[2] = {s0 + t0, s1 + t1};
  block_sum_store<2>(in2, part + ((size_t)blockIdx.y * C + c) * 2);
  if (blockIdx.y == 0 && threadIdx.x == 0) shift[c] = k;
}

__global__ __launch_bounds__(256) void k_bn_apply(const float* __restrict__ x, const float* __restrict__ gamma, const float* __restrict__ beta,
                                                   const float* __restrict__ part, const float* __restrict__ shift, int nsplit, float count,
                                                   float eps, float momentum, float* __restrict__ save_mean, float* __restrict__ save_invstd,
                                                   float* __restrict__ running_mean, float* __restrict__ running_var,
                                                   long long* __restrict__ num_batches_tracked, float* __restrict__ y,
                                                   int B, int C, int HW, int bps, int relu) {
  const int c = blockIdx.x, b0 = blockIdx.y * bps, nb = min(B, b0 + bps) - b0;
  float s0, s1;
  split_sums(part, nsplit, C, c, s0, s1);
  const float d = s0 / count;
  const float m = shift[c] + d;
  const float var = fmaxf(s1 / count - d * d, 0.f);
  const float is = rsqrtf(var + eps);
  if (blockIdx.y == 0 && threadIdx.x == 0) {
    save_mean[c] = m;
    save_invstd[c] = is;
    if (running_mean) {
      running_mean[c] = (1.f - momentum) * running_mean[c] + momentum * m;
      running_var[c] = (1.f - momentum) * running_var[c] + momentum * var * (count / (count - 1.f));
    }
    if (c == 0 && num_batches_tracked) *num_batches_tracked += 1;
  }
  const float g = gamma[c], bt = beta[c];
  const float lo = relu ? 0.f : -INFINITY;
  chan_slab(C, HW, c, b0, nb,
            [&](size_t i) {
              const float4 v = *reinterpret_cast<const float4*>(x + i);
              float4 o;
              o.x = fmaxf(bn_affine(v.x, m, is, g, bt), lo); o.y = fmaxf(bn_affine(v.y, m, is, g, bt), lo);
              o.z = fmaxf(bn_affine(v.z, m, is, g, bt), lo); o.w = fmaxf(bn_affine(v.w, m, is, g, bt), lo);
              *reinterpret_cast<float4*>(y + i) = o;
            },
            [&](size_t i) { y[i] = fmaxf(bn_affine(x[i], m, is, g, bt), lo); });
}

__global__ __launch_bounds__(64) void k_bn_table(const float* __restrict__ gamma, const float* __restrict__ beta, const float* __restrict__ part,
                                                 const float* __restrict__ shift, int nsplit, int C, float count, float eps, float momentum,
                                                 float* __restrict__ save_mean, float* __restrict__ save_invstd,
                                                 float* __restrict__ running_mean, float* __restrict__ running_var,
                                                 long long* __restrict__ num_batches_tracked, float* __restrict__ table) {
  const int c = blockIdx.x;
  float s0, s1;
  split_sums(part, nsplit, C, c, s0, s1);
  if (threadIdx.x != 0) return;
  const float d = s0 / count;
  const float m = shift[c] + d;
  const float var = fmaxf(s1 / count - d * d, 0.f);
  const float is = rsqrtf(var + eps);
  save_mean[c] = m;
  save_invstd[c] = is;
  if (running_mean) {
    running_mean[c] = (1.f - momentum) * running_mean[c] + momentum * m;
    running_var[c] = (1.f - momentum) * running_var[c] + momentum * var * (count / (count - 1.f));
  }
  if (c == 0 && num_batches_tracked) *num_batches_tracked += 1;
  table[4 * c + 0] = m; table[4 * c + 1] = is; table[4 * c + 2] = gamma[c]; table[4 * c + 3] = beta[c];
}

__global__ __launch_bounds__(256) void k_bn_bwd_sums(const float* __restrict__ x, const float* __restrict__ gy, const float* __restrict__ gamma,
                                                      const float* __restrict__ beta, const float* __restrict__ mean,
                                                      const float* __restrict__ invstd, int B, int C, int HW, int bps, int relu,
                                                      float* __restrict__ part) {
  const int c = blockIdx.x, b0 = blockIdx.y * bps, nb = min(B, b0 + bps) - b0;
  const float m = mean[c], is = invstd[c], g = gamma[c], bt = beta[c];
  float s0 = 0.f, s1 = 0.f, t0 = 0.f, t1 = 0.f;
  auto one = [&](float xv, float gv, float& a0, float& a1) {
    const float xh = bn_xhat(xv, m, is);
    if (relu && !(__fmaf_rn(xh, g, bt) > 0.f)) gv = 0.f;
    a0 += gv;
    a1 = fmaf(gv, xh, a1);
  };
  chan_slab(C, HW, c, b0, nb,
            [&](size_t i) {
              const float4 v = *reinterpret_cast<const float4*>(x + i), w = *reinterpret_cast<const float4*>(gy + i);
              one(v.x, w.x, s0, s1); one(v.y, w.y, t0, t1); one(v.z, w.z, s0, s1); one(v.w, w.w, t0, t1);
            },
            [&](size_t i) { one(x[i], gy[i], s0, s1); });
  const float in2[2] = {s0 + t0, s1 + t1};
  block_sum_store<2>(in2, part + ((size_t)blockIdx.y * C + c) * 2);
}

__global__ __launch_bounds__(256) void k_bn_bwd_apply(const float* __restrict__ x, const float* __restrict__ gy, const float* __restrict__ gamma,
                                                       const float* __restrict__ beta, const float* __restrict__ mean,
                                                       const float* __restrict__ invstd, const float* __restrict__ part, int nsplit,
                                                       float count, float* __restrict__ ggamma, float* __restrict__ gbeta,
                                                       float* __restrict__ gx, float* __restrict__ part_gx, int B, int C, int HW, int bps,
                                                       int relu, const float* __restrict__ gathered, const float* __restrict__ wts, int W) {
  const int c = blockIdx.x, b0 = blockIdx.y * bps, nb = min(B, b0 + bps) - b0;
  const float m = mean[c], is = invstd[c], g = gamma[c], bt = beta[c];
  float sa, sb;
  split_sums(part, nsplit, C, c, sa, sb);
  if (blockIdx.y == 0 && threadIdx.x == 0) { gbeta[c] = sa; ggamma[c] = sb; }
  if (gathered) {
    const int lane = threadIdx.x & 63;
    const float wr = lane < W ? wts[lane] : 0.f;
    const float in2[2] = {lane < W ? wr * gathered[(size_t)lane * 2 * C + 2 * c] : 0.f, lane < W ? wr * gathered[(size_t)lane * 2 * C + 2 * c + 1] : 0.f};
    float out2[2];
    wave_sum_multi<2>(in2, out2);
    sa = out2[0];
    sb = out2[1];
  }
  const float ic = 1.f / count, ca = sa * ic, cb = sb * ic, sc = g * is;
  auto one = [&](float xv, float gv) {
    const float xh = bn_xhat(xv, m, is);
    if (relu && !(__fmaf_rn(xh, g, bt) > 0.f)) gv = 0.f;
    return sc * (gv - ca - xh * cb);
  };
  float s0 = 0.f, t0 = 0.f;
  chan_slab(C, HW, c, b0, nb,
            [&](size_t i) {
              const float4 v = *reinterpret_cast<const float4*>(x + i), w = *reinterpret_cast<const float4*>(gy + i);
              float4 o;
              o.x = one(v.x, w.x); o.y = one(v.y, w.y); o.z = one(v.z, w.z); o.w = one(v.w, w.w);
              *reinterpret_cast<float4*>(gx + i) = o;
              s0 += o.x; t0 += o.y; s0 += o.z; t0 += o.w;
            },
            [&](size_t i) {
              const float o = one(x[i], gy[i]);
              gx[i] = o;
              s0 += o;
            });
  if (part_gx) {
    const float in2[2] = {s0 + t0, 0.f};
    block_sum_store<2>(in2, part_gx + ((size_t)blockIdx.y * C + c) * 2);
  }
}

__device__ __forceinline__ void block_sum2(float a, float b, float& sa, float& sb) {
  __shared__ float red2[4][2];
  const float in2[2] = {a, b};
  float out2[2];
  wave_sum_multi<2>(in2, out2);
  __syncthreads();
  if ((threadIdx.x & 63) == 0) { red2[threadIdx.x >> 6][0] = out2[0]; red2[threadIdx.x >> 6][1] = out2[1]; }
  __syncthreads();
  sa = (red2[0][0] + red2[1][0]) + (red2[2][0] + red2[3][0]);
  sb = (red2[0][1] + red2[1][1]) + (red2[2][1] + red2[3][1]);
}

__global__ __launch_bounds__(256) void k_bn_fwd_small(const float* __restrict__ x, const float* __restrict__ gamma, const float* __restrict__ beta,
                                                       float count, float eps, float momentum, float* __restrict__ save_mean,
                                                       float* __restrict__ save_invstd, float* __restrict__ running_mean,
                                                       float* __restrict__ running_var, long long* __restrict__ num_batches_tracked,
                                                       float* __restrict__ y, float* __restrict__ table, int B, int C, int HW, int relu) {
  const int c = blockIdx.x;
  const float k = chan_shift(x, HW, c);
  float s0 = 0.f, s1 = 0.f, t0 = 0.f, t1 = 0.f;
  chan_slab(C, HW, c, 0, B,
            [&](size_t i) {
              const float4 v = *reinterpret_cast<const float4*>(x + i);
              const float a = v.x - k, b = v.y - k, d = v.z - k, e = v.w - k;
              s0 += a; t0 += b; s0 += d; t0 += e;
              s1 = fmaf(a, a, s1); t1 = fmaf(b, b, t1); s1 = fmaf(d, d, s1); t1 = fmaf(e, e, t1);
            },
            [&](size_t i) {
              const float a = x[i] - k;
              s0 += a;
              s1 = fmaf(a, a, s1);
            });
  float sa, sb;
  block_sum2(s0 + t0, s1 + t1, sa, sb);
  const float d = sa / count;
  const float m = k + d;
  const float var = fmaxf(sb / count - d * d, 0.f);
  const float is = rsqrtf(var + eps);
  const float g = gamma[c], bt = beta[c];
  if (threadIdx.x == 0) {
    save_mean[c] = m;
    save_invstd[c] = is;
    if (running_mean) {
      running_mean[c] = (1.f - momentum) * running_mean[c] + momentum * m;
      running_var[c] = (1.f - momentum) * running_var[c] + momentum * var * (count / (count - 1.f));
    }
    if (c == 0 && num_batches_tracked) *num_batches_tracked += 1;
    if (table) { table[4 * c + 0] = m; table[4 * c + 1] = is; table[4 * c + 2] = g; table[4 * c + 3] = bt; }
  }
  if (!y) return;
  const float lo = relu ? 0.f : -INFINITY;
  chan_slab(C, HW, c, 0, B,
            [&](size_t i) {
              const float4 v = *reinterpret_cast<const float4*>(x + i);
              float4 o;
              o.x = fmaxf(bn_affine(v.x, m, is, g, bt), lo); o.y = fmaxf(bn_affine(v.y, m, is, g, bt), lo);
              o.z = fmaxf(bn_affine(v.z, m, is, g, bt), lo); o.w = fmaxf(bn_affine(v.w, m, is, g, bt), lo);
              *reinterpret_cast<float4*>(y + i) = o;
            },
            [&](size_t i) { y[i] = fmaxf(bn_affine(x[i], m, is, g, bt), lo); });
}

__global__ __launch_bounds__(256) void k_bn_bwd_small(const float* __restrict__ x, const float* __restrict__ gy, const float* __restrict__ gamma,
// ... 75 lines not shown
  chan_slab(C, HW, c, b0, nb,
            [&](size_t i) {
              const float4 a = *reinterpret_cast<const float4*>(v + i);
              s0 += a.x; t0 += a.y; s0 += a.z; t0 += a.w;
            },
            [&](size_t i) { s0 += v[i]; });
  const float in2[2] = {s0 + t0, 0.f};
  block_sum_store<2>(in2, part + ((size_t)blockIdx.y * C + c) * 2);
}

__global__ __launch_bounds__(64) void k_reduce_chan(const float* __restrict__ part, int nsplit, int C, float* __restrict__ out) {
  float a, b;
  split_sums(part, nsplit, C, blockIdx.x, a, b);
  if (threadIdx.x == 0) out[blockIdx.x] = a;
}


__global__ __launch_bounds__(64) void k_bn_moments(const float* __restrict__ part, const float* __restrict__ shift, int nsplit, int C,
                                                   float count, float* __restrict__ mom) {
  const int c = blockIdx.x;
  if (c == C) { if (threadIdx.x == 0) mom[2 * C] = count; return; }
  float s0, s1;
  split_sums(part, nsplit, C, c, s0, s1);
  if (threadIdx.x != 0) return;
  const float d = s0 / count;
  mom[2 * c] = shift[c] + d;
  mom[2 * c + 1] = fmaxf(s1 - s0 * d, 0.f);
}

__global__ __launch_bounds__(64) void k_bn_finalize(const float* __restrict__ gathered, int W, const float* __restrict__ gamma,
                                                    const float* __restrict__ beta, int C, float eps, float momentum,
                                                    float* __restrict__ save_mean, float* __restrict__ save_invstd,
                                                    float* __restrict__ running_mean, float* __restrict__ running_var,
                                                    long long* __restrict__ num_batches_tracked, float* __restrict__ table) {
  const int c = blockIdx.x, lane = threadIdx.x;
  const size_t stride = 2 * (size_t)C + 1;
  const float nr = lane < W ? gathered[lane * stride + 2 * C] : 0.f;
  const float mr = lane < W ? gathered[lane * stride + 2 * c] : 0.f;
  const float qr = lane < W ? gathered[lane * stride + 2 * c + 1] : 0.f;
  const float m0 = gathered[2 * c];
  const float in2[2] = {nr, nr * (mr - m0)};
  float out2[2];
  wave_sum_multi<2>(in2, out2);
  const float count = out2[0], m = m0 + out2[1] / count;
  const float dm = mr - m;
  const float in1[1] = {fmaf(nr * dm, dm, qr)};
  float out1[1];
  wave_sum_multi<1>(in1, out1);
  if (lane != 0) return;
  const float var = fmaxf(out1[0] / count, 0.f);
  const float is = rsqrtf(var + eps);
  save_mean[c] = m;
  save_invstd[c] = is;
  if (running_mean) {
    running_mean[c] = (1.f - momentum) * running_mean[c] + momentum * m;
    running_var[c] = (1.f - momentum) * running_var[c] + momentum * var * (count / (count - 1.f));
  }
  if (c == 0 && num_batches_tracked) *num_batches_tracked += 1;
  table[4 * c + 0] = m; table[4 * c + 1] = is; table[4 * c + 2] = gamma[c]; table[4 * c + 3] = beta[c];
}

__global__ __launch_bounds__(256) void k_bn_apply_table(const float* __restrict__ x, const float* __restrict__ table, float* __restrict__ y,
                                                         int B, int C, int HW, int bps, int relu) {
  const int c = blockIdx.x, b0 = blockIdx.y * bps, nb = min(B, b0 + bps) - b0;
  const float m = table[4 * c], is = table[4 * c + 1], g = table[4 * c + 2], bt = table[4 * c + 3];
  const float lo = relu ? 0.f : -INFINITY;
  chan_slab(C, HW, c, b0, nb,
            [&](size_t i) {
              const float4 v = *reinterpret_cast<const float4*>(x + i);
              float4 o;
              o.x = fmaxf(bn_affine(v.x, m, is, g, bt), lo); o.y = fmaxf(bn_affine(v.y, m, is, g, bt), lo);
              o.z = fmaxf(bn_affine(v.z, m, is, g, bt), lo); o.w = fmaxf(bn_affine(v.w, m, is, g, bt), lo);
              *reinterpret_cast<float4*>(y + i) = o;
            },
            [&](size_t i) { y[i] = fmaxf(bn_affine(x[i], m, is, g, bt), lo); });
}

__global__ __launch_bounds__(64) void k_reduce_chan2(const float* __restrict__ part, int nsplit, int C, float* __restrict__ out) {
  float a, b;
  split_sums(part, nsplit, C, blockIdx.x, a, b);
  if (threadIdx.x == 0) { out[2 * blockIdx.x] = a; out[2 * blockIdx.x + 1] = b; }
}

struct Split { int ns, bps, used; };
inline Split pick(int B) {
  Split s;
  s.ns = B < 64 ? B : 64;
  s.bps = (B + s.ns - 1) / s.ns;
  s.used = (B + s.bps - 1) / s.bps;
  return s;
}
constexpr size_t kBnSmallFwd = 20000, kBnSmallBwd = 2048;
inline bool bn_small(size_t per_channel, size_t limit) {
  static const bool off = [] { const char* e = getenv("GPODE_BN_ONE_LAUNCH"); return e && e[0] == '0'; }();
  return !off && per_channel <= limit;
}
constexpr const char* kBnOneValue = "Expected more than 1 value per channel when training";

}

size_t bn_scratch(int B, int C) { return (size_t)(B < 64 ? B : 64) * C * 4 + (size_t)C * 3; }

int bn_fwd(const float* x, const float* gamma, const float* beta, float* y, float* save_mean, float* save_invstd,
           float* running_mean, float* running_var, long long* num_batches_tracked, float momentum, float eps, int B, int C, int HW,
           int relu, float* scratch, hipStream_t st) {
  if ((HW & 3) == 0 && !(aligned16(x) && aligned16(y))) return set_error("gpode_bn_fwd: x / y must be 16-byte aligned");
  if ((size_t)B * HW < 2) return set_error("gpode_bn_fwd: %s, got B * HW = %d", kBnOneValue, B * HW);
  if (bn_small((size_t)B * HW, kBnSmallFwd)) {
    hipLaunchKernelGGL(k_bn_fwd_small, C, 256, 0, st, x, gamma, beta, (float)B * HW, eps, momentum, save_mean, save_invstd, running_mean, running_var,
                       num_batches_tracked, y, (float*)nullptr, B, C, HW, relu);
    return check_launch("bn_fwd (one launch)");
  }
  const Split sp = pick(B);
  float* shift = scratch + (size_t)sp.ns * C * 2 + (size_t)C * 2;
  hipLaunchKernelGGL(k_bn_stats, dim3(C, sp.used), 256, 0, st, x, B, C, HW, sp.bps, scratch, shift);
  hipLaunchKernelGGL(k_bn_apply, dim3(C, sp.used), 256, 0, st, x, gamma, beta, scratch, shift, sp.used, (float)B * HW, eps, momentum, save_mean,
                     save_invstd, running_mean, running_var, num_batches_tracked, y, B, C, HW, sp.bps, relu);
  return check_launch("bn_fwd");
}

int bn_stats(const float* x, const float* gamma, const float* beta, float* save_mean, float* save_invstd, float* running_mean,
             float* running_var, long long* num_batches_tracked, float momentum, float eps, float* table, int B, int C, int HW,
             float* scratch, hipStream_t st) {
  if ((HW & 3) == 0 && !aligned16(x)) return set_error("gpode_bn_stats: x must be 16-byte aligned");
  if ((size_t)B * HW < 2) return set_error("gpode_bn_stats: %s, got B * HW = %d", kBnOneValue, B * HW);
  if (bn_small((size_t)B * HW, kBnSmallFwd)) {
    hipLaunchKernelGGL(k_bn_fwd_small, C, 256, 0, st, x, gamma, beta, (float)B * HW, eps, momentum, save_mean, save_invstd, running_mean, running_var,
                       num_batches_tracked, (float*)nullptr, table, B, C, HW, 0);
    return check_launch("bn_stats (one launch)");
  }
  const Split sp = pick(B);
  float* shift = scratch + (size_t)sp.ns * C * 2 + (size_t)C * 2;
  hipLaunchKernelGGL(k_bn_stats, dim3(C, sp.used), 256, 0, st, x, B, C, HW, sp.bps, scratch, shift);
  hipLaunchKernelGGL(k_bn_table, C, 64, 0, st, gamma, beta, scratch, shift, sp.used, C, (float)B * HW, eps, momentum, save_mean, save_invstd,
                     running_mean, running_var, num_batches_tracked, table);
  return check_launch("bn_stats");
}

int bn_bwd(const float* x, const float* gy, const float* gamma, const float* beta, const float* save_mean,
           const float* save_invstd, float* gx, float* ggamma, float* gbeta, float* gx_chansum, int B, int C, int HW, int relu,
           float* scratch, hipStream_t st) {
  if ((HW & 3) == 0 && !(aligned16(x) && aligned16(gy) && aligned16(gx))) return set_error("gpode_bn_bwd: x / gy / gx must be 16-byte aligned");
  if (bn_small((size_t)B * HW, kBnSmallBwd)) {
    hipLaunchKernelGGL(k_bn_bwd_small, C, 256, 0, st, x, gy, gamma, beta, save_mean, save_invstd, (float)B * HW, ggamma, gbeta, gx, gx_chansum, B, C,
                       HW, relu);
    return check_launch("bn_bwd (one launch)");
  }
  const Split sp = pick(B);
  hipLaunchKernelGGL(k_bn_bwd_sums, dim3(C, sp.used), 256, 0, st, x, gy, gamma, beta, save_mean, save_invstd, B, C, HW, sp.bps, relu, scratch);
  float* part_gx = gx_chansum ? scratch + (size_t)sp.ns * C * 2 + (size_t)C * 3 : nullptr;
  hipLaunchKernelGGL(k_bn_bwd_apply, dim3(C, sp.used), 256, 0, st, x, gy, gamma, beta, save_mean, save_invstd, scratch, sp.used, (float)B * HW,
                     ggamma, gbeta, gx, part_gx, B, C, HW, sp.bps, relu, (const float*)nullptr, (const float*)nullptr, 0);
  if (gx_chansum && reduce_job(RedJob{part_gx, gx_chansum, sp.used, C, 2, 0, 0, 0}, st)) return 1;
  return check_launch("bn_bwd");
}

int bn_moments(const float* x, float* mom, int B, int C, int HW, float* scratch, hipStream_t st) {
  if ((HW & 3) == 0 && !aligned16(x)) return set_error("gpode_bn_moments: x must be 16-byte aligned");
  const Split sp = pick(B);
  float* shift = scratch + (size_t)sp.ns * C * 2 + (size_t)C * 2;
  hipLaunchKernelGGL(k_bn_stats, dim3(C, sp.used), 256, 0, st, x, B, C, HW, sp.bps, scratch, shift);
  hipLaunchKernelGGL(k_bn_moments, C + 1, 64, 0, st, scratch, shift, sp.used, C, (float)B * HW, mom);
  return check_launch("bn_moments");
}

int bn_finalize(const float* gathered, int W, const float* gamma, const float* beta, float* save_mean, float* save_invstd,
                float* running_mean, float* running_var, long long* num_batches_tracked, float momentum, float eps, float* table, int C,
                hipStream_t st) {
  if (W < 1 || W > 64) return set_error("gpode_bn_finalize: %d ranks (1..64 supported)", W);
  hipLaunchKernelGGL(k_bn_finalize, C, 64, 0, st, gathered, W, gamma, beta, C, eps, momentum, save_mean, save_invstd, running_mean, running_var,
                     num_batches_tracked, table);
  return check_launch("bn_finalize");
}

int bn_apply(const float* x, const float* table, float* y, int B, int C, int HW, int relu, hipStream_t st) {
  if ((HW & 3) == 0 && !(aligned16(x) && aligned16(y))) return set_error("gpode_bn_apply: x / y must be 16-byte aligned");
  const Split sp = pick(B);
  hipLaunchKernelGGL(k_bn_apply_table, dim3(C, sp.used), 256, 0, st, x, table, y, B, C, HW, sp.bps, relu);
  return check_launch("bn_apply");
}

int bn_bwd_sums(const float* x, const float* gy, const float* gamma, const float* beta, const float* save_mean, const float* save_invstd,
                float* sums, int B, int C, int HW, int relu, float* scratch, hipStream_t st) {
  if ((HW & 3) == 0 && !(aligned16(x) && aligned16(gy))) return set_error("gpode_bn_bwd_sums: x / gy must be 16-byte aligned");
  const Split sp = pick(B);
  hipLaunchKernelGGL(k_bn_bwd_sums, dim3(C, sp.used), 256, 0, st, x, gy, gamma, beta, save_mean, save_invstd, B, C, HW, sp.bps, relu, scratch);
  hipLaunchKernelGGL(k_reduce_chan2, C, 64, 0, st, scratch, sp.used, C, sums);
  return check_launch("bn_bwd_sums");
}

int bn_bwd_apply(const float* x, const float* gy, const float* gamma, const float* beta, const float* save_mean, const float* save_invstd,
                 const float* gathered, const float* wts, int W, float count, float* gx, float* ggamma, float* gbeta, float* gx_chansum, int B, int C, int HW, int relu,
                 float* scratch, hipStream_t st) {
  if ((HW & 3) == 0 && !(aligned16(x) && aligned16(gy) && aligned16(gx))) return set_error("gpode_bn_bwd_apply: x / gy / gx must be 16-byte aligned");
  if (W < 1 || W > 64) return set_error("gpode_bn_bwd_apply: %d ranks (1..64 supported)", W);
  const Split sp = pick(B);
  float* part_gx = gx_chansum ? scratch + (size_t)sp.ns * C * 2 + (size_t)C * 3 : nullptr;
  hipLaunchKernelGGL(k_bn_bwd_apply, dim3(C, sp.used), 256, 0, st, x, gy, gamma, beta, save_mean, save_invstd, scratch, sp.used, count,
                     ggamma, gbeta, gx, part_gx, B, C, HW, sp.bps, relu, gathered, wts, W);
  if (gx_chansum && reduce_job(RedJob{part_gx, gx_chansum, sp.used, C, 2, 0, 0, 0}, st)) return 1;
  return check_launch("bn_bwd_apply");
}

__global__ __launch_bounds__(64) void k_bn_eval_table(const float* __restrict__ gamma, const float* __restrict__ beta, const float* __restrict__ rmean,
                                                      const float* __restrict__ rvar, float eps, float* __restrict__ table, int C) {
  const int c = blockIdx.x * 64 + threadIdx.x;
  if (c < C) reinterpret_cast<float4*>(table)[c] = float4{rmean[c], rsqrtf(rvar[c] + eps), gamma[c], beta[c]};
}

int bn_eval_table(const float* gamma, const float* beta, const float* running_mean, const float* running_var, float eps, float* table, int C,
                  hipStream_t st) {
  if (C < 1) return set_error("gpode_bn_eval_table: C >= 1");
  if (!aligned16(table)) return set_error("gpode_bn_eval_table: the table must be 16-byte aligned");
  hipLaunchKernelGGL(k_bn_eval_table, (C + 63) / 64, 64, 0, st, gamma, beta, running_mean, running_var, eps, table, C);
  return check_launch("bn_eval_table");
}

int bn_eval(const float* x, const float* gy, const float* gamma, const float* beta, const float* running_mean, const float* running_var,
            float eps, float* out, int B, int C, int HW, int relu, hipStream_t st) {
  if ((HW & 3) == 0 && !(aligned16(x) && aligned16(out) && (!gy || aligned16(gy)))) return set_error("gpode_bn_eval: tensors must be 16-byte aligned");
  const Split sp = pick(B);
  hipLaunchKernelGGL(k_bn_eval, dim3(C, sp.used), 256, 0, st, x, gy, gamma, beta, running_mean, running_var, eps, out, B, C, HW, sp.bps, relu);
  return check_launch("bn_eval");
}

namespace {
constexpr int kMaxRedJobs = 24;
struct RedJobs { RedJob j[kMaxRedJobs]; };
std::mutex g_red_mu;
RedJob g_red_jobs[kMaxRedJobs];
int g_red_n = 0, g_red_defer = 0;

__global__ __launch_bounds__(1024) void k_reduce_multi(RedJobs jobs) {
  __shared__ float red[16][64];
  const RedJob& jb = jobs.j[blockIdx.y];
  const int n = jb.n;
  if ((int)blockIdx.x * 64 >= n) return;
  const int ex = threadIdx.x & 63, sg = threadIdx.x >> 6;
  const int e = blockIdx.x * 64 + ex;
  float acc = 0.f;
  if (e < n) {
    const float* p = jb.part;
    if (jb.kind == 2) {
#pragma unroll 4
      for (int s = sg; s < jb.nsplit; s += 16) acc += p[((size_t)s * n + e) * 2];
    } else {
#pragma unroll 8
      for (int s = sg; s < jb.nsplit; s += 16) acc += p[(size_t)s * n + e];
    }
  }
  red[sg][ex] = acc;
  __syncthreads();
  if (sg == 0 && e < n) {
    float v = 0.f;
#pragma unroll
    for (int g = 0; g < 16; ++g) v += red[g][ex];
    if (jb.kind == 1) {
      const int MT = jb.a, NT = jb.b, KK = jb.c;
      const int lane = e & 63, r = (e >> 6) & 3, tile = e >> 8;
      const int nt = tile % NT, mt = (tile / NT) % MT, t = tile / (NT * MT);
      const int ci = mt * 16 + 4 * (lane >> 4) + r, co = nt * 16 + (lane & 15);
      jb.out[((size_t)ci * (NT * 16) + co) * KK + t] = v;
    } else {
      jb.out[e] = v;
    }
  }
}

int launch_red(const RedJob* jobs, int nj, hipStream_t st) {
  RedJobs all;
  int maxn = 0;
  for (int i = 0; i < nj; ++i) { all.j[i] = jobs[i]; maxn = jobs[i].n > maxn ? jobs[i].n : maxn; }
// ... 56 lines not shown
```

### vae-gp-ode_amd/csrc/vae_wgrad_v2.hip

```cpp
#include <hip/hip_runtime.h>
#include <cstdint>
#include "gp_launch.hpp"
#include "conv_layers.hpp"
#include "conv_wgrad_v2.hpp"

namespace gp {

template <class L, bool PIPE>
static int launch_wgrad_v2(const float* x, const float* gy, float* gw, float* scratch, int B, hipStream_t st, const float* in_bn) {
  constexpr size_t lds = wgrad_v2_lds_bytes<L>();
  static_assert(lds <= 160 * 1024, "LDS budget");
  auto km = k_convT_wgrad_v2<L, false, PIPE>;
  auto kb = k_convT_wgrad_v2<L, true, PIPE>;
  if (set_max_lds((const void*)km, lds) || set_max_lds((const void*)kb, lds)) return 1;
  const int nwg = B < num_cus() ? B : num_cus();
  if (in_bn) hipLaunchKernelGGL(kb, nwg, 768, lds, st, x, gy, scratch, B, in_bn);
  else hipLaunchKernelGGL(km, nwg, 768, lds, st, x, gy, scratch, B, in_bn);
  const size_t n = (size_t)L::CI * L::CO * L::K * L::K;
  if (reduce_job(RedJob{scratch, gw, nwg, (int)n, 1, L::CI / 16, L::CO / 16, L::K * L::K}, st)) return 1;
  return check_launch("convT_wgrad_v2");
}

int wgrad_v2_dec7(const float* x, const float* gy, float* gw, float* scratch, int B, hipStream_t st, const float* in_bn) {
  return launch_wgrad_v2<Dec7, true>(x, gy, gw, scratch, B, st, in_bn);
}
int wgrad_v2_dec4(const float* x, const float* gy, float* gw, float* scratch, int B, hipStream_t st, const float* in_bn) {
  return launch_wgrad_v2<Dec4, true>(x, gy, gw, scratch, B, st, in_bn);
}

}
```

### vae-gp-ode_amd/vae_ops.py

```python
import ctypes
import os

import torch

from . import _lib, ops
from .ops import _chk, _ptr, _stream




def _new(shape, like):
    return torch.empty(shape, dtype=torch.float32, device=like.device)


def _bchw(x):
    return x.shape[0], x.shape[1], x[0, 0].numel()


def _convT_out(Hi, Wi, K, stride, pad, out_pad):
    return (Hi - 1) * stride - 2 * pad + K + out_pad, (Wi - 1) * stride - 2 * pad + K + out_pad


def _scratch(n, like):
    return torch.empty(max(int(n), 4), dtype=torch.float32, device=like.device)
# ... 97 lines not shown
    return _bn_bwd_apply(sync, sync.gather(sums), scratch, x, gy, gamma, beta, mean, invstd, relu)


def _bn_bwd(sync, x, gy, gamma, beta, mean, invstd, relu):
    if sync is not None:
        return _bn_global_bwd(sync, x, gy, gamma, beta, mean, invstd, relu)
    B, C, HW = _bchw(x)
    gx, gg, gb, cs = _new(x.shape, x), _new((C,), x), _new((C,), x), _new((C,), x)
    bs = _bn_scratch(B, C, x)
    _bwd_call('gpode_bn_bwd', _ptr(x), _ptr(gy.contiguous()), _ptr(gamma), _ptr(beta), _ptr(mean), _ptr(invstd), _ptr(gx), _ptr(gg),
              _ptr(gb), _ptr(cs), B, C, HW, relu, _ptr(bs), _stream(), keep=(bs,))
    return gx, gg, gb, cs


_pack_bn = {'on': os.environ.get('GPODE_PACK_BN_GATHERS', '0') == '1'}


def set_pack_bn_gathers(on):
    _pack_bn['on'] = bool(on)


def pack_bn_gathers():
    return _pack_bn['on'] and _bn_sync is not None


class _BatchNormTrainPair(torch.autograd.Function):

    @staticmethod
    def forward(ctx, x1, g1, b1, rm1, rv1, nbt1, x2, g2, b2, rm2, rv2, nbt2, momentum, eps, relu):
        xs = (_chk(x1, 'x1'), _chk(x2, 'x2'))
        gathered = _bn_sync.gather_many([_bn_moments(x) for x in xs])
        ys, saved = [], []
        for x, gam, bet, rm, rv, nbt, got in zip(xs, (g1, g2), (b1, b2), (rm1, rm2), (rv1, rv2), (nbt1, nbt2), gathered):
            mean, invstd, table = _bn_finalize(got, x, gam, bet, rm, rv, nbt, momentum, eps)
            ys.append(_bn_apply(x, table, relu))
            saved += [x, gam, bet, mean, invstd]
        ctx.save_for_backward(*saved)
        ctx.sync, ctx.relu = _bn_sync, int(relu)
        return ys[0], ys[1]

    @staticmethod
    def backward(ctx, gy1, gy2):
        sv, sync = ctx.saved_tensors, ctx.sync
        layers = [(x, gy, *rest, ctx.relu) for (x, *rest), gy in zip((sv[:5], sv[5:]), (gy1, gy2))]
        sums = [_bn_bwd_sums(*layer) for layer in layers]
        gathered = sync.gather_many([s for s, _, _ in sums])
        out = []
        for (x, _, *rest), (_, gy, scratch), got in zip(layers, sums, gathered):
            gx, gg, gb, cs = _bn_bwd_apply(sync, got, scratch, x, gy, *rest)
            gx._gpode_chansum = cs
            out += [gx, gg, gb, None, None, None]
        return (*out, None, None, None)


def batch_norm_train_pair(x1, bn1, x2, bn2, relu):
    return _BatchNormTrainPair.apply(x1, bn1.weight, bn1.bias, bn1.running_mean, bn1.running_var, bn1.num_batches_tracked,
                                     x2, bn2.weight, bn2.bias, bn2.running_mean, bn2.running_var, bn2.num_batches_tracked,
                                     bn1.momentum, bn1.eps, relu)


_dec10_fused = os.environ.get('GPODE_DEC10_BN_UNFUSED', '0') != '1'


def _dec10_bn_bwd(sync, c, gy, w, gamma, beta, mean, invstd, gw=None, gbias=None):
    B = c.shape[0]
    scratch = _scratch(_lib.load().gpode_dec10_bn_scratch_floats(), c)
    gc, gg, gb, cs = _new(c.shape, c), _new((16,), c), _new((16,), c), _new((16,), c)
    head = (_ptr(c), _ptr(gy), _ptr(w), _ptr(gamma), _ptr(beta), _ptr(mean), _ptr(invstd))
    sums = _new((32,), c) if sync is not None else None
    if gw is not None:
        ws = _scratch(_lib.load().gpode_dec10_bn_wgrad_scratch_floats(), c)
        _bwd_call('gpode_dec10_bn_bwd_sums_wgrad', *head, _ptr(sums), _ptr(gw), _ptr(gbias), B, _ptr(scratch), _ptr(ws), _stream(),
                  keep=(ws, scratch))
    else:
        _lib.call('gpode_dec10_bn_bwd_sums', *head, _ptr(sums), B, _ptr(scratch), _stream())
    if sync is None:
        _bwd_call('gpode_dec10_bn_bwd_apply', *head, _ptr(None), _ptr(None), 0, ctypes.c_float(0.0), _ptr(gc), _ptr(gg), _ptr(gb), _ptr(cs),
                  B, _ptr(scratch), _stream(), keep=(scratch,))
    else:
        gathered = sync.gather(sums)
        _bwd_call('gpode_dec10_bn_bwd_apply', *head, _ptr(gathered), _ptr(sync.weights(c.device)), sync.world,
                  ctypes.c_float(sync.count_all(B * 784)), _ptr(gc), _ptr(gg), _ptr(gb), _ptr(cs), B, _ptr(scratch), _stream(), keep=(scratch,))
    return gc, gg, gb, cs


fused_bias_grads = 0


def _fused_chansum(gy, C):
    global fused_bias_grads
    cs = getattr(gy, '_gpode_chansum', None)
    if cs is None or tuple(cs.shape) != (C,):
        return None
    del gy._gpode_chansum
    fused_bias_grads += 1
    return cs


def _batch_strided(x):
    if x.dim() != 4 or x.is_contiguous() or x.dtype != torch.float32 or not x.is_cuda or x.shape[1] % 4 == 0 or x.shape[0] < 2:
        return 0
    B, C, H, W = x.shape
    if x.stride()[1:] != (H * W, W, 1) or x.stride(0) < C * H * W:
        return 0
    return x.stride(0)


class _Conv2d(torch.autograd.Function):
    @staticmethod
    def forward(ctx, x, w, b, stride, pad):
        xbs = _batch_strided(x)
        if not xbs:
            x = _chk(x, 'x')
        w = _chk(w, 'weight')
        B, Ci, H, W = x.shape
        Co, _, K, _ = w.shape
        Ho, Wo = (H + 2 * pad - K) // stride + 1, (W + 2 * pad - K) // stride + 1
        y = _new((B, Co, Ho, Wo), x)
        if xbs:
            _lib.call('gpode_conv2d_fwd_bs', _ptr(x), xbs, _ptr(w), _ptr(b), _ptr(y), B, Ci, H, W, Co, K, stride, pad, Ho, Wo, _stream())
        else:
            _lib.call('gpode_conv2d_fwd', _ptr(x), _ptr(w), _ptr(b), _ptr(y), B, Ci, H, W, Co, K, stride, pad, Ho, Wo, _stream())
        ctx.save_for_backward(x, w)
        ctx.geom = (B, Ci, H, W, Co, K, stride, pad, Ho, Wo, b is not None)
        ctx.xbs = xbs
        return y

    @staticmethod
    def backward(ctx, gy):
        x, w = ctx.saved_tensors
        B, Ci, H, W, Co, K, S, P, Ho, Wo, has_b = ctx.geom
        gy = gy.contiguous()
        gx = gw = gb = None
        if ctx.needs_input_grad[0]:
            gx = _new(x.shape, x)
            _lib.call('gpode_conv2d_bwd_data', _ptr(gy), _ptr(w), _ptr(None), _ptr(gx), B, Ci, H, W, Co, K, S, P, Ho, Wo, _stream())
        if ctx.needs_input_grad[1]:
            gw = _new(w.shape, x)
            pre = _fused_chansum(gy, Co) if has_b else None
            gb = _new((Co,), x) if (has_b and pre is None) else None
            ws = _wgrad_scratch(B, Ci, Co, K, x)
            if ctx.xbs:
                _bwd_call('gpode_conv2d_bwd_weight_bs', _ptr(x), ctx.xbs, _ptr(gy), _ptr(gw), _ptr(gb), _ptr(ws),
                          B, Ci, H, W, Co, K, S, P, Ho, Wo, _stream(), keep=(ws, gy))
            else:
                _bwd_call('gpode_conv2d_bwd_weight', _ptr(x), _ptr(gy), _ptr(gw), _ptr(gb), _ptr(ws),
                          B, Ci, H, W, Co, K, S, P, Ho, Wo, _stream(), keep=(ws, gy))
            if pre is not None:
                gb = pre
        return gx, gw, gb, None, None


_STATS_GEOMS = {(32, 64, 3, 1, 0, 4), (64, 32, 5, 2, 1, 6), (32, 16, 5, 2, 1, 13)}
_fused_stats = os.environ.get('GPODE_BN_STATS_PASS', '0') != '1'
_FUSED_STATS_MIN_IMAGES = int(os.environ.get('GPODE_BN_STATS_FUSED_MIN', '512'))
_slots = {'next': 0}


def _stats_slot(bn):
    s = getattr(bn, '_gpode_slot', None)
    if s is None:
        s = bn._gpode_slot = _slots['next'] % 64
        _slots['next'] += 1
    return s


def _can_fuse_stats(bn, x, Cin, Cout, K, stride, pad, Hi):
    return (_fused_stats and bn is not None and bn.training and _bn_sync is None and (Cin, Cout, K, stride, pad, Hi) in _STATS_GEOMS
            and x.shape[0] >= _FUSED_STATS_MIN_IMAGES and x.data_ptr() % 16 == 0 and os.environ.get('GPODE_CONV_VALU', '0') != '1')


def _convT_fwd_stats(x, table_in, w, b, y, geom, bn):
    B, Cout, Ht, Wt, Cin, K, stride, pad, Hi, Wi = geom
    mean, invstd, table = _new((Cout,), x), _new((Cout,), x), _new((Cout, 4), x)
    scratch = _scratch(_lib.load().gpode_convT_fwd_stats_scratch(Cout), x)
    _lib.call('gpode_convT_fwd_stats', _ptr(x), _ptr(table_in), _ptr(w), _ptr(b), _ptr(y), B, Cout, Ht, Wt, Cin, K, stride, pad, Hi, Wi,
              _ptr(_chk(bn.weight, 'gamma')), _ptr(_chk(bn.bias, 'beta')), _ptr(mean), _ptr(invstd), _ptr(bn.running_mean),
              _ptr(bn.running_var), _ptr(bn.num_batches_tracked), ctypes.c_float(bn.momentum), ctypes.c_float(bn.eps), _ptr(table),
              _ptr(scratch), _stats_slot(bn), _stream())
    y._gpode_bnstats = (bn, mean, invstd, table)


class _ConvT2d(torch.autograd.Function):

    @staticmethod
    def forward(ctx, x, w, b, stride, pad, out_pad, stats_for=None):
        x, w = _chk(x, 'x'), _chk(w, 'weight')
        B, Cin, Hi, Wi = x.shape
        _, Cout, K, _ = w.shape
        Ht, Wt = _convT_out(Hi, Wi, K, stride, pad, out_pad)
        y = _new((B, Cout, Ht, Wt), x)
        if _can_fuse_stats(stats_for, x, Cin, Cout, K, stride, pad, Hi):
            _convT_fwd_stats(x, None, w, b, y, (B, Cout, Ht, Wt, Cin, K, stride, pad, Hi, Wi), stats_for)
        else:
            _lib.call('gpode_conv2d_bwd_data', _ptr(x), _ptr(w), _ptr(b), _ptr(y), B, Cout, Ht, Wt, Cin, K, stride, pad, Hi, Wi, _stream())
        ctx.save_for_backward(x, w)
        ctx.geom = (B, Cout, Ht, Wt, Cin, K, stride, pad, Hi, Wi, b is not None)
        return y

    @staticmethod
    def backward(ctx, gy):
        x, w = ctx.saved_tensors
        B, Cout, Ht, Wt, Cin, K, S, P, Hi, Wi, has_b = ctx.geom
        gy = gy.contiguous()
        gx = gw = gb = None
        if ctx.needs_input_grad[0]:
            gx = _new(x.shape, x)
            _lib.call('gpode_conv2d_fwd', _ptr(gy), _ptr(w), _ptr(None), _ptr(gx), B, Cout, Ht, Wt, Cin, K, S, P, Hi, Wi, _stream())
        if ctx.needs_input_grad[1]:
            gw = _new(w.shape, x)
            ws = _wgrad_scratch(B, Cout, Cin, K, x)
            _bwd_call('gpode_conv2d_bwd_weight', _ptr(gy), _ptr(x), _ptr(gw), _ptr(None), _ptr(ws),
                      B, Cout, Ht, Wt, Cin, K, S, P, Hi, Wi, _stream(), keep=(ws,))
            if has_b:
                gb = _fused_chansum(gy, Cout)
                if gb is None:
                    gb, bs = _new((Cout,), x), _bn_scratch(B, Cout, x)
                    _bwd_call('gpode_chan_sum', _ptr(gy), _ptr(gb), B, Cout, Ht * Wt, _ptr(bs), _stream(), keep=(bs,))
        return gx, gw, gb, None, None, None, None


class _BnReluConvT(torch.autograd.Function):

    @staticmethod
    def forward(ctx, c, gamma, beta, running_mean, running_var, nbt, momentum, eps, w, b, stride, pad, out_pad, bn=None, stats_for=None):
        pre = getattr(c, '_gpode_bnstats', None)
        c, w = _chk(c, 'c'), _chk(w, 'weight')
        B, Cin, Hi, Wi = c.shape
        _, Cout, K, _ = w.shape
        Ht, Wt = _convT_out(Hi, Wi, K, stride, pad, out_pad)
        ctx.sync = _bn_sync
        if pre is not None and pre[0] is bn and bn is not None and _bn_sync is None:
            _, mean, invstd, table = pre
        elif _bn_sync is not None:
            mean, invstd, table = _bn_global_stats(c, gamma, beta, running_mean, running_var, nbt, momentum, eps)
        else:
            mean, invstd, table = _new((Cin,), c), _new((Cin,), c), _new((Cin, 4), c)
            _lib.call('gpode_bn_stats', _ptr(c), _ptr(_chk(gamma, 'gamma')), _ptr(_chk(beta, 'beta')), _ptr(mean), _ptr(invstd),
                      _ptr(running_mean), _ptr(running_var), _ptr(nbt), ctypes.c_float(momentum), ctypes.c_float(eps), _ptr(table),
                      B, Cin, Hi * Wi, _ptr(_bn_scratch(B, Cin, c)), _stream())
        y = _new((B, Cout, Ht, Wt), c)
        if _can_fuse_stats(stats_for, c, Cin, Cout, K, stride, pad, Hi):
            _convT_fwd_stats(c, table, w, b, y, (B, Cout, Ht, Wt, Cin, K, stride, pad, Hi, Wi), stats_for)
        else:
            _lib.call('gpode_conv2d_bwd_data_bn', _ptr(c), _ptr(table), _ptr(w), _ptr(b), _ptr(y), B, Cout, Ht, Wt, Cin, K, stride, pad, Hi, Wi,
                      _stream())
        ctx.save_for_backward(c, gamma, beta, mean, invstd, table, w)
        ctx.geom = (B, Cout, Ht, Wt, Cin, K, stride, pad, Hi, Wi, b is not None)
        return y

    @staticmethod
    def backward(ctx, gy):
        c, gamma, beta, mean, invstd, table, w = ctx.saved_tensors
        B, Cout, Ht, Wt, Cin, K, S, P, Hi, Wi, has_b = ctx.geom
        gy = gy.contiguous()
        gw = gb = None
        last_stage = _dec10_fused and (Cout, Cin, K, S, P, Hi, Wi, Ht, Wt) == (1, 16, 5, 1, 2, 28, 28, 28, 28)
        gw_rides = last_stage and ctx.needs_input_grad[8] and c.data_ptr() % 16 == 0
        if ctx.needs_input_grad[8]:
            gw = _new(w.shape, c)
            if not gw_rides:
                ws = _wgrad_scratch(B, Cout, Cin, K, c)
                _bwd_call('gpode_conv2d_bwd_weight_bn', _ptr(gy), _ptr(c), _ptr(table), _ptr(gw), _ptr(None),
                          _ptr(ws), B, Cout, Ht, Wt, Cin, K, S, P, Hi, Wi, _stream(), keep=(ws,))
            gb = _fused_chansum(gy, Cout) if has_b else None
        to_sum = has_b and gw is not None and gb is None
        if to_sum:
            gb = _new((Cout,), c)
            if not gw_rides:
                bs = _bn_scratch(B, Cout, c)
                _bwd_call('gpode_chan_sum', _ptr(gy), _ptr(gb), B, Cout, Ht * Wt, _ptr(bs), _stream(), keep=(bs,))
        gb_rides = gb if (to_sum and gw_rides) else None
        if last_stage:
            gc, gg, gbeta, cs = _dec10_bn_bwd(ctx.sync, c, gy, w, gamma, beta, mean, invstd, gw=gw if gw_rides else None, gbias=gb_rides)
        else:
            ga = _new(c.shape, c)
            _lib.call('gpode_conv2d_fwd', _ptr(gy), _ptr(w), _ptr(None), _ptr(ga), B, Cout, Ht, Wt, Cin, K, S, P, Hi, Wi, _stream())
            gc, gg, gbeta, cs = _bn_bwd(ctx.sync, c, ga, gamma, beta, mean, invstd, 1)
        gc._gpode_chansum = cs
        return gc, gg, gbeta, None, None, None, None, None, gw, gb, None, None, None, None, None


class _BatchNormTrain(torch.autograd.Function):
    @staticmethod
    def forward(ctx, x, gamma, beta, running_mean, running_var, momentum, eps, relu, nbt=None):
        x = _chk(x, 'x')
        B, C, HW = _bchw(x)
        if nbt is not None and not (nbt.is_cuda and nbt.dtype == torch.int64):
            raise _lib.GpodeError('num_batches_tracked must be an int64 CUDA/HIP scalar')
        ctx.sync = _bn_sync
        if _bn_sync is not None:
            mean, invstd, table = _bn_global_stats(x, gamma, beta, running_mean, running_var, nbt, momentum, eps)
            y = _bn_apply(x, table, relu)
        else:
            y, mean, invstd = _new(x.shape, x), _new((C,), x), _new((C,), x)
            _lib.call('gpode_bn_fwd', _ptr(x), _ptr(_chk(gamma, 'gamma')), _ptr(_chk(beta, 'beta')), _ptr(y), _ptr(mean), _ptr(invstd),
                      _ptr(running_mean), _ptr(running_var), _ptr(nbt), ctypes.c_float(momentum), ctypes.c_float(eps), B, C, HW, int(relu),
                      _ptr(_bn_scratch(B, C, x)), _stream())
        ctx.save_for_backward(x, gamma, beta, mean, invstd)
        ctx.relu = int(relu)
        return y

    @staticmethod
    def backward(ctx, gy):
        x, gamma, beta, mean, invstd = ctx.saved_tensors
        gx, gg, gb, cs = _bn_bwd(ctx.sync, x, gy, gamma, beta, mean, invstd, ctx.relu)
        gx._gpode_chansum = cs
        return gx, gg, gb, None, None, None, None, None, None


class _BatchNormEval(torch.autograd.Function):

    @staticmethod
    def forward(ctx, x, gamma, beta, running_mean, running_var, eps, relu):
        x = _chk(x, 'x')
        B, C, HW = _bchw(x)
        y = _new(x.shape, x)
        _lib.call('gpode_bn_eval', _ptr(x), _ptr(None), _ptr(_chk(gamma, 'gamma')), _ptr(_chk(beta, 'beta')), _ptr(running_mean),
                  _ptr(running_var), ctypes.c_float(eps), _ptr(y), B, C, HW, int(relu), _stream())
        ctx.save_for_backward(x, gamma, beta, running_mean, running_var)
        ctx.eps, ctx.relu = eps, int(relu)
        return y

    @staticmethod
    def backward(ctx, gy):
        if ctx.needs_input_grad[1] or ctx.needs_input_grad[2]:
            raise _lib.GpodeError('eval-mode BatchNorm is built for frozen layers (main.py:160-161 sets requires_grad=False)')
        x, gamma, beta, rm, rv = ctx.saved_tensors
        B, C, HW = _bchw(x)
        gx = _new(x.shape, x)
        _lib.call('gpode_bn_eval', _ptr(x), _ptr(gy.contiguous()), _ptr(gamma), _ptr(beta), _ptr(rm), _ptr(rv), ctypes.c_float(ctx.eps),
                  _ptr(gx), B, C, HW, ctx.relu, _stream())
        return gx, None, None, None, None, None, None


class _Act(torch.autograd.Function):
    @staticmethod
    def forward(ctx, x, mode):
        x = _chk(x, 'x')
        y = _new(x.shape, x)
        _lib.call('gpode_act_fwd', _ptr(x), _ptr(y), x.numel(), mode, _stream())
        ctx.save_for_backward(y)
        ctx.mode = mode
        return y

    @staticmethod
    def backward(ctx, gy):
        (y,) = ctx.saved_tensors
        gx = _new(y.shape, y)
        _lib.call('gpode_act_bwd', _ptr(y), _ptr(gy.contiguous()), _ptr(gx), y.numel(), ctx.mode, _stream())
        return gx, None


class _Linear(torch.autograd.Function):
    @staticmethod
    def forward(ctx, x, w, b):
        x, w = _chk(x, 'x'), _chk(w, 'weight')
        B, In = x.shape
        Out = w.shape[0]
        y = _new((B, Out), x)
# ... 585 lines not shown
```

Before: 107,600 trajectories/s.

## Fold BatchNorm-ReLU backward apply into the next conv's data and weight gradient kernels

Measured after the change: 108,600 trajectories/s, median of 6. Within noise of the previous version (+1.0%).

```diff
diff --git a/include/gpode.h b/include/gpode.h
--- a/include/gpode.h
+++ b/include/gpode.h
@@ -201,6 +201,16 @@
                        const float* save_invstd, const float* sums_gathered, const float* weights, int nranks, float count_all,
                        float* gx, float* ggamma, float* gbeta, float* gx_chansum, int B, int C, int HW, int relu, float* scratch,
                        void* stream);
+int gpode_bn_bwd_sums_split(const float* x, const float* gy, const float* gamma, const float* beta, const float* save_mean,
+                            const float* save_invstd, float* ggamma, float* gbeta, int B, int C, int HW, int relu, float* scratch,
+                            void* stream);
+int gpode_conv2d_fwd_bnb(const float* g, const float* x, const float* gamma, const float* beta, const float* save_mean,
+                         const float* save_invstd, const float* bn_part, float count, const float* w, float* y, int B, int Ci, int H,
+                         int W, int Co, int K, int S, int P, int Ho, int Wo, void* stream);
+int gpode_conv2d_bwd_weight_bnb(const float* g, const float* x, const float* gamma, const float* beta, const float* save_mean,
+                                const float* save_invstd, const float* bn_part, float count, const float* a, const float* a_bn,
+                                float* gw, float* gbias, float* scratch, int B, int Ci, int H, int W, int Co, int K, int S, int P,
+                                int Ho, int Wo, void* stream);
 void gpode_defer_reductions(int mode);
 int gpode_flush_reductions(void* stream);
 int gpode_dec10_bn_wgrad_scratch_floats(void);
diff --git a/vae-gp-ode_amd/_lib.py b/vae-gp-ode_amd/_lib.py
--- a/vae-gp-ode_amd/_lib.py
+++ b/vae-gp-ode_amd/_lib.py
@@ -85,6 +85,9 @@
     'gpode_bn_apply': (_i, [_vp, _vp, _vp, _i, _i, _i, _i, _vp]),
     'gpode_bn_bwd_sums': (_i, [_vp] * 7 + [_i, _i, _i, _i, _vp, _vp]),
     'gpode_bn_bwd_apply': (_i, [_vp] * 8 + [_i, _f] + [_vp] * 4 + [_i, _i, _i, _i, _vp, _vp]),
+    'gpode_bn_bwd_sums_split': (_i, [_vp] * 8 + [_i, _i, _i, _i, _vp, _vp]),
+    'gpode_conv2d_fwd_bnb': (_i, [_vp] * 7 + [_f, _vp, _vp] + [_i] * 10 + [_vp]),
+    'gpode_conv2d_bwd_weight_bnb': (_i, [_vp] * 7 + [_f] + [_vp] * 5 + [_i] * 10 + [_vp]),
     'gpode_defer_reductions': (None, [_i]),
     'gpode_flush_reductions': (_i, [_vp]),
     'gpode_dec10_bn_scratch_floats': (_i, []),
diff --git a/vae-gp-ode_amd/csrc/bn_math.hpp b/vae-gp-ode_amd/csrc/bn_math.hpp
--- a/vae-gp-ode_amd/csrc/bn_math.hpp
+++ b/vae-gp-ode_amd/csrc/bn_math.hpp
@@ -1,5 +1,6 @@
 #pragma once
 #include <hip/hip_runtime.h>
+#include "wave_reduce.hpp"
 
 namespace gp {
 
@@ -7,4 +8,62 @@
 __device__ __forceinline__ float bn_affine(float x, float m, float is, float g, float b) { return __fmaf_rn(bn_xhat(x, m, is), g, b); }
 __device__ __forceinline__ float bn_relu(float x, const float4& t) { return fmaxf(bn_affine(x, t.x, t.y, t.z, t.w), 0.f); }
 
+__device__ __forceinline__ float bn_bwd_core(float x, float g, float m, float is, float gamma, float beta, float ca, float cb, int relu) {
+  const float xh = bn_xhat(x, m, is);
+  if (relu && !(__fmaf_rn(xh, gamma, beta) > 0.f)) g = 0.f;
+  return __fmaf_rn(-xh, cb, __fsub_rn(g, ca));
 }
+__device__ __forceinline__ float bn_bwd_gx(float x, float g, float m, float is, float gamma, float beta, float ca, float cb, float sc,
+                                           int relu) {
+  return __fmul_rn(sc, bn_bwd_core(x, g, m, is, gamma, beta, ca, cb, relu));
+}
+
+__device__ __forceinline__ void split_sums(const float* __restrict__ part, int nsplit, int C, int c, float& a, float& b) {
+  const int lane = threadIdx.x & 63;
+  const float in2[2] = {lane < nsplit ? part[((size_t)lane * C + c) * 2] : 0.f, lane < nsplit ? part[((size_t)lane * C + c) * 2 + 1] : 0.f};
+  float out2[2];
+  wave_sum_multi<2>(in2, out2);
+  a = out2[0];
+  b = out2[1];
+}
+
+__device__ __forceinline__ void bn_bwd_consts(float sa, float sb, float count, float gamma, float is, float& ca, float& cb, float& sc) {
+  const float ic = 1.f / count;
+  ca = __fmul_rn(sa, ic);
+  cb = __fmul_rn(sb, ic);
+  sc = __fmul_rn(gamma, is);
+}
+
+struct BnBwdArgs {
+  const float *x, *gamma, *beta, *mean, *invstd, *part;
+  int nsplit;
+  float count;
+};
+
+__device__ __forceinline__ void bn_bwd_table(float4* __restrict__ s_bt, int C, int wave, int nwaves, const BnBwdArgs& bn) {
+  for (int c = wave; c < C; c += nwaves) {
+    float sa, sb, ca, cb, sc;
+    split_sums(bn.part, bn.nsplit, C, c, sa, sb);
+    const float m = bn.mean[c], is = bn.invstd[c], g = bn.gamma[c], bt = bn.beta[c];
+    bn_bwd_consts(sa, sb, bn.count, g, is, ca, cb, sc);
+    if ((threadIdx.x & 63) == 0) {
+      s_bt[2 * c] = float4{m, is, g, bt};
+      s_bt[2 * c + 1] = float4{ca, cb, sc, 0.f};
+    }
+  }
+}
+
+typedef float bn_f2 __attribute__((ext_vector_type(2)));
+__device__ __forceinline__ bn_f2 bn_bwd_gx2(bn_f2 x, bn_f2 g, const float4& t0, const float4& t1) {
+  const bn_f2 xh = (x - t0.x) * t0.y;
+  const bn_f2 y = __builtin_elementwise_fma(xh, bn_f2{t0.z, t0.z}, bn_f2{t0.w, t0.w});
+  if (!(y.x > 0.f)) g.x = 0.f;
+  if (!(y.y > 0.f)) g.y = 0.f;
+  return __builtin_elementwise_fma(-xh, bn_f2{t1.y, t1.y}, g - t1.x) * t1.z;
+}
+template <class V4> __device__ __forceinline__ void bn_bwd_gx4(const V4& x, const V4& g, const float4& t0, const float4& t1, float (&o)[4]) {
+  const bn_f2 a = bn_bwd_gx2(bn_f2{x[0], x[1]}, bn_f2{g[0], g[1]}, t0, t1), b = bn_bwd_gx2(bn_f2{x[2], x[3]}, bn_f2{g[2], g[3]}, t0, t1);
+  o[0] = a.x; o[1] = a.y; o[2] = b.x; o[3] = b.y;
+}
+
+}
diff --git a/vae-gp-ode_amd/csrc/capi.hip b/vae-gp-ode_amd/csrc/capi.hip
--- a/vae-gp-ode_amd/csrc/capi.hip
+++ b/vae-gp-ode_amd/csrc/capi.hip
@@ -553,6 +553,28 @@
   return gp::bn_bwd_apply(x, gy, gamma, beta, save_mean, save_invstd, sums_gathered, weights, nranks, count_all, gx, ggamma, gbeta, gx_chansum, B, C, HW, relu,
                           scratch, GP_ST);
 }
+int gpode_bn_bwd_sums_split(const float* x, const float* gy, const float* gamma, const float* beta, const float* save_mean,
+                            const float* save_invstd, float* ggamma, float* gbeta, int B, int C, int HW, int relu, float* scratch,
+                            void* stream) {
+  if (!x || !gy || !gamma || !beta || !save_mean || !save_invstd || !ggamma || !gbeta || !scratch)
+    return gp::set_error("gpode_bn_bwd_sums_split: null pointer");
+  return gp::bn_bwd_sums_split(x, gy, gamma, beta, save_mean, save_invstd, ggamma, gbeta, B, C, HW, relu, scratch, GP_ST);
+}
+int gpode_conv2d_fwd_bnb(const float* g, const float* x, const float* gamma, const float* beta, const float* save_mean,
+                         const float* save_invstd, const float* bn_part, float count, const float* w, float* y, int B, int Ci, int H,
+                         int W, int Co, int K, int S, int P, int Ho, int Wo, void* stream) {
+  if (!g || !x || !gamma || !beta || !save_mean || !save_invstd || !bn_part || !w || !y) return gp::set_error("gpode_conv2d_fwd_bnb: null pointer");
+  return gp::conv2d_fwd_bnb(g, x, gamma, beta, save_mean, save_invstd, bn_part, count, w, y, B, Ci, H, W, Co, K, S, P, Ho, Wo, GP_ST);
+}
+int gpode_conv2d_bwd_weight_bnb(const float* g, const float* x, const float* gamma, const float* beta, const float* save_mean,
+                                const float* save_invstd, const float* bn_part, float count, const float* a, const float* a_bn,
+                                float* gw, float* gbias, float* scratch, int B, int Ci, int H, int W, int Co, int K, int S, int P,
+                                int Ho, int Wo, void* stream) {
+  if (!g || !x || !gamma || !beta || !save_mean || !save_invstd || !bn_part || !a || !gw || !scratch)
+    return gp::set_error("gpode_conv2d_bwd_weight_bnb: null pointer");
+  return gp::conv2d_bwd_weight_bnb(g, x, gamma, beta, save_mean, save_invstd, bn_part, count, a, a_bn, gw, gbias, scratch, B, Ci, H, W, Co, K,
+                                   S, P, Ho, Wo, GP_ST);
+}
 void gpode_defer_reductions(int mode) { gp::defer_reductions(mode); }
 int gpode_flush_reductions(void* stream) { return gp::flush_reductions(GP_ST); }
 int gpode_dec10_bn_scratch_floats(void) { return gp::dec10_bn_scratch_floats(); }
diff --git a/vae-gp-ode_amd/csrc/conv_bwd_v2.hpp b/vae-gp-ode_amd/csrc/conv_bwd_v2.hpp
--- a/vae-gp-ode_amd/csrc/conv_bwd_v2.hpp
+++ b/vae-gp-ode_amd/csrc/conv_bwd_v2.hpp
@@ -1,5 +1,6 @@
 #pragma once
 #include "conv_mfma.hpp"
+#include "bn_math.hpp"
 
 namespace gp {
 
@@ -26,7 +27,7 @@
   static_assert(ROW4 || L::HO * L::HO <= NLT, "producer offset table");
   static constexpr int koff(int s) { return (s / (KC / 4)) / L::K * HP + (s / (KC / 4)) % L::K + (s % (KC / 4)) * 4 * PS; }
   static_assert(4 * koff(NKS - 1) < 65536, "operand offsets fit the ds_read immediate");
-  static constexpr size_t lds_bytes() { return sizeof(float) * (size_t)NBUF * IMG; }
+  static constexpr size_t lds_bytes(bool bnb = false) { return sizeof(float) * ((size_t)NBUF * IMG + (bnb ? 8 * KC : 0)); }
 };
 
 template <class E, int NT>
@@ -60,10 +61,11 @@
   bdv2_tiles<E, NT>(s_buf, base, wr, acc);
 }
 
-template <class L>
+template <class L, bool BNB = false>
 __global__ __launch_bounds__(BdV2<L>::NTHR) void k_conv_bwd_data_v2(const float* __restrict__ gy, const float* __restrict__ w,
-                                                                    float* __restrict__ gx, int B) {
+                                                                    float* __restrict__ gx, int B, BnBwdArgs bn) {
   using E = BdV2<L>;
+  static_assert(!BNB || !E::ROW4, "the BatchNorm-backward staging is written for the offset-table path");
   using PL = typename E::PL;
   constexpr int KC = E::KC, NC = E::NC, KK = E::KK, NPX = E::NPX, IMG = E::IMG, PS = E::PS, HP = E::HP, WIN = E::WIN, NKS = E::NKS;
   constexpr int HO = L::HO, P = L::P, NLT = E::NLT, NBUF = E::NBUF, TPW = E::TPW, TSPLIT = E::TSPLIT;
@@ -74,6 +76,9 @@
   auto last_img = [&](int i) { return min(nit - 1, (i * WIN + WIN - 1) / NPX); };
 
   for (int e = tid; e < NBUF * IMG / 4; e += E::NTHR) reinterpret_cast<float4*>(s_buf)[e] = float4{0.f, 0.f, 0.f, 0.f};
+  float4* s_bt = reinterpret_cast<float4*>(s_buf + NBUF * IMG);
+  if constexpr (BNB)
+    bn_bwd_table(s_bt, KC, wave, E::NTHR / 64, bn);
   __syncthreads();
 
   if (wave >= E::NCW) {
@@ -86,10 +91,36 @@
       const int e = 4 * min(lt, HO * HO - 1) + k, pl = e / (HO * HO), q = e % (HO * HO);
       otab[k] = pl * PS + (q / HO + P) * HP + q % HO + P;
     }
+    constexpr int NIT = (HO * HO + 3) / 4;
+    static_assert(!BNB || (4 * NIT <= NLT && HO * HO >= 4), "the items of four planes fit the producer threads");
+    typedef float f4u __attribute__((ext_vector_type(4), aligned(4)));
+    const int bpq = min(lt, 4 * NIT - 1) / NIT, bq0 = min(4 * (min(lt, 4 * NIT - 1) - bpq * NIT), HO * HO - 4);
+    int botab[4];
+#pragma unroll
+    for (int k = 0; k < 4; ++k) botab[k] = bpq * PS + ((bq0 + k) / HO + P) * HP + (bq0 + k) % HO + P;
+    const float4* bct = s_bt + 2 * bpq;
     auto stage = [&](int j) __attribute__((always_inline)) {
       const float4* src = reinterpret_cast<const float4*>(gy) + (size_t)((int)blockIdx.x + j * (int)gridDim.x) * N4;
       float* buf = s_buf + (j % NBUF) * IMG;
-      if constexpr (E::ROW4) {
+      if constexpr (BNB) {
+        if (lt < 4 * NIT) {
+          const size_t e0 = (size_t)((int)blockIdx.x + j * (int)gridDim.x) * E::SRC + bpq * (HO * HO) + bq0;
+          f4u v[KC / 4], u[KC / 4];
+#pragma unroll
+          for (int g = 0; g < KC / 4; ++g) v[g] = *reinterpret_cast<const f4u*>(gy + e0 + g * 4 * HO * HO);
+#pragma unroll
+          for (int g = 0; g < KC / 4; ++g) u[g] = *reinterpret_cast<const f4u*>(bn.x + e0 + g * 4 * HO * HO);
+#pragma unroll
+          for (int g = 0; g < KC / 4; ++g) {
+            const float4 t0 = bct[8 * g], t1 = bct[8 * g + 1];
+            float* d = buf + 4 * g * PS;
+            float o[4];
+            bn_bwd_gx4(u[g], v[g], t0, t1, o);
+#pragma unroll
+            for (int k = 0; k < 4; ++k) d[botab[k]] = o[k];
+          }
+        }
+      } else if constexpr (E::ROW4) {
         constexpr int NLD = (N4 + NLT - 1) / NLT;
         float4 v[NLD];
 #pragma unroll
diff --git a/vae-gp-ode_amd/csrc/conv_wgrad_v2.hpp b/vae-gp-ode_amd/csrc/conv_wgrad_v2.hpp
--- a/vae-gp-ode_amd/csrc/conv_wgrad_v2.hpp
+++ b/vae-gp-ode_amd/csrc/conv_wgrad_v2.hpp
@@ -1,14 +1,15 @@
 #pragma once
 #include "conv_mfma.hpp"
+#include "bn_math.hpp"
 #ifndef WGV2_PRIO
 #define WGV2_PRIO 3
 #endif
 
 namespace gp {
 
-template <class L> constexpr size_t wgrad_v2_lds_floats(bool gtab) {
+template <class L> constexpr size_t wgrad_v2_lds_floats(bool gtab, bool bnb = false) {
   return (size_t)2 * (WgradGeo<L>::IMGX + WgradGeo<L>::IMGG) + (size_t)4 * L::CI + (size_t)4 * (WgradGeo<L>::NKS + 1) +
-         (gtab ? (size_t)L::CO * L::HO * L::HO : 0);
+         (gtab ? (bnb ? (size_t)L::CO * ((L::HO * L::HO + 3) / 4) * 4 : (size_t)L::CO * L::HO * L::HO) : 0) + (bnb ? (size_t)8 * L::CO : 0);
 }
 
 template <class L> struct WgV2 {
@@ -106,7 +107,7 @@
   }
 }
 
-template <class L, int WV, bool PIPE>
+template <class L, int WV, bool PIPE, bool BNB = false>
 __device__ __forceinline__ void wgrad_v2_consumer(const float* __restrict__ s_buf, const int* __restrict__ s_tab, int nit, int lane,
                                                   float* __restrict__ pp) {
   using W = WgV2<L>;
@@ -144,11 +145,13 @@
   for (int j = 0; j < UE - UB; ++j)
 #pragma unroll
     for (int r = 0; r < 4; ++r) pp[((size_t)(UB + j) * 4 + r) * 64 + lane] = acc[j][r];
-}
-
-template <class L, bool HAS_BN, bool PIPE>
+  if constexpr (BNB) __syncthreads();
+}
+
+template <class L, bool HAS_BN, bool PIPE, bool BNB = false>
 __global__ __launch_bounds__(768) void k_convT_wgrad_v2(const float* __restrict__ x, const float* __restrict__ gy,
-                                                         float* __restrict__ part, int B, const float* __restrict__ in_bn) {
+                                                         float* __restrict__ part, int B, const float* __restrict__ in_bn, BnBwdArgs bn,
+                                                         float* __restrict__ part_b) {
   using W = WgV2<L>;
   using G = typename W::G;
   constexpr int CI = L::CI, CO = L::CO, HO = L::HO, S = L::S, P = L::P, KK = W::KK;
@@ -161,12 +164,27 @@
   int* s_tab = reinterpret_cast<int*>(igemm_smem + 2 * IMG + 4 * CI);
   constexpr bool GTAB = !(S == 2 && HO % 4 == 0 && P == 1) && wgrad_v2_lds_floats<L>(true) * sizeof(float) <= 160 * 1024;
   int* s_gtab = s_tab + 4 * (G::NKS + 1);
+  static_assert(!BNB || GTAB, "the BatchNorm-backward staging is written for the scatter-table path");
+  constexpr int NITP = (HO * HO + 3) / 4, NITEM = CO * NITP, NEWT = HO * HO - 4 * (NITP - 1);
+  static_assert(!BNB || HO * HO >= 4, "a tail item of four elements");
+  float4* s_bt = reinterpret_cast<float4*>(igemm_smem + wgrad_v2_lds_floats<L>(GTAB, BNB) - 8 * CO);
   const int tid = threadIdx.x, lane = tid & 63, wave = __builtin_amdgcn_readfirstlane(tid >> 6);
   const bool producer = wave >= W::NCW;
   const int lt = tid - 64 * W::NCW;
   if (HAS_BN)
     for (int e = tid; e < CI; e += NTHR) s_tf[e] = reinterpret_cast<const float4*>(in_bn)[e];
-  if (GTAB)
+  if constexpr (BNB)
+    bn_bwd_table(s_bt, CO, wave, NTHR / 64, bn);
+  if constexpr (BNB) {
+    for (int e = tid; e < NITEM; e += NTHR) {
+      const int pl = e / NITP, q0 = min(4 * (e % NITP), HO * HO - 4);
+#pragma unroll
+      for (int k = 0; k < 4; ++k) {
+        const int rr = (q0 + k) / HO + P, cc = (q0 + k) % HO + P;
+        s_gtab[4 * e + k] = pl * PSG + (S == 2 ? (cc & 1) * HPL + rr * GPH + (cc >> 1) : rr * GPH + cc);
+      }
+    }
+  } else if (GTAB)
     for (int e = tid; e < SRCG; e += NTHR) {
       const int pl = e / (HO * HO), q = e % (HO * HO), rr = q / HO + P, cc = q % HO + P;
       s_gtab[e] = pl * PSG + (S == 2 ? (cc & 1) * HPL + rr * GPH + (cc >> 1) : rr * GPH + cc);
@@ -234,10 +252,63 @@
         }
       }
     };
+    constexpr int NSLOT = (NITEM + NLT - 1) / NLT;
+    typedef float f4u __attribute__((ext_vector_type(4), aligned(4)));
+    float bacc[BNB ? NSLOT : 1];
+    int be0[BNB ? NSLOT : 1], bpl[BNB ? NSLOT : 1];
+    bool btail[BNB ? NSLOT : 1];
+    if constexpr (BNB) {
+#pragma unroll
+      for (int j = 0; j < NSLOT; ++j) {
+        const int it = min(lt + NLT * j, NITEM - 1), i = it % NITP;
+        bpl[j] = it / NITP;
+        be0[j] = bpl[j] * (HO * HO) + min(4 * i, HO * HO - 4);
+        btail[j] = i == NITP - 1;
+        bacc[j] = 0.f;
+      }
+    }
+    auto scatter_gb = [&](float* __restrict__ s_g, const auto& gv, const auto& uv) __attribute__((always_inline)) {
+      static_for<NSLOT>([&](auto jj) {
+        constexpr int j = decltype(jj)::value;
+        const int it = lt + NLT * j;
+        if (it < NITEM) {
+          const float4 t0 = s_bt[2 * bpl[j]], t1 = s_bt[2 * bpl[j] + 1];
+          const int4 o = reinterpret_cast<const int4*>(s_gtab)[it];
+          const int off[4] = {o.x, o.y, o.z, o.w};
+          float gx[4], sdup = 0.f, snew = 0.f;
+          bn_bwd_gx4(uv[j], gv[j], t0, t1, gx);
+#pragma unroll
+          for (int k = 0; k < 4; ++k) {
+            s_g[off[k]] = gx[k];
+            if (k < 4 - NEWT) sdup += gx[k]; else snew += gx[k];
+          }
+          bacc[j] += (btail[j] ? 0.f : sdup) + snew;
+        }
+      });
+    };
     auto stage = [&](int img, float* __restrict__ buf) __attribute__((always_inline)) {
       const float4* sx = reinterpret_cast<const float4*>(x) + (size_t)img * NX4;
       const float4* sg = reinterpret_cast<const float4*>(gy) + (size_t)img * NG4;
       float4 va[CH], vb[CH];
+      if constexpr (BNB) {
+        f4u gv[NSLOT], uv[NSLOT];
+        load(sx, NX4, 0, va);
+        static_for<NCX>([&](auto cc) {
+          constexpr int c = decltype(cc)::value;
+          float4 (&cur)[CH] = (c % 2 == 0) ? va : vb;
+          float4 (&nxt)[CH] = (c % 2 == 0) ? vb : va;
+          if constexpr (c + 1 < NCX) load(sx, NX4, c + 1, nxt);
+          else {
+#pragma unroll
+            for (int j = 0; j < NSLOT; ++j) gv[j] = *reinterpret_cast<const f4u*>(gy + (size_t)img * SRCG + be0[j]);
+#pragma unroll
+            for (int j = 0; j < NSLOT; ++j) uv[j] = *reinterpret_cast<const f4u*>(bn.x + (size_t)img * SRCG + be0[j]);
+          }
+          scatter_x(buf, c, cur);
+        });
+        scatter_gb(buf + IMGX, gv, uv);
+        return;
+      }
       load(sx, NX4, 0, va);
       static_for<NCX>([&](auto cc) {
         constexpr int c = decltype(cc)::value;
@@ -280,24 +351,38 @@
 #ifdef WGV2_PROBE
     if (blockIdx.x == 0 && lane == 0) printf("wgrad_v2 producer %d: stage %lld cycles, barrier wait %lld\n", wave, t_st, t_bar);
 #endif
+    if constexpr (BNB) {
+      float* s_red = s_buf;
+      static_assert(NSLOT * NLT <= 2 * IMG, "the channel sums fit the plane buffers");
+      static_for<NSLOT>([&](auto jj) {
+        constexpr int j = decltype(jj)::value;
+        s_red[lt + NLT * j] = bacc[j];
+      });
+      __syncthreads();
+      if (lt < CO && part_b) {
+        float s = 0.f;
+        for (int i = 0; i < NITP; ++i) s += s_red[lt * NITP + i];
+        part_b[(size_t)blockIdx.x * CO + lt] = s;
+      }
+    }
     return;
   }
   float* pp = part + (size_t)blockIdx.x * CI * CO * KK;
   switch (wave) {
-    case 0: wgrad_v2_consumer<L, 0, PIPE>(s_buf, s_tab, nit, lane, pp); break;
-    case 1: wgrad_v2_consumer<L, 1, PIPE>(s_buf, s_tab, nit, lane, pp); break;
-    case 2: wgrad_v2_consumer<L, 2, PIPE>(s_buf, s_tab, nit, lane, pp); break;
-    case 3: wgrad_v2_consumer<L, 3, PIPE>(s_buf, s_tab, nit, lane, pp); break;
-    case 4: wgrad_v2_consumer<L, 4, PIPE>(s_buf, s_tab, nit, lane, pp); break;
-    case 5: wgrad_v2_consumer<L, 5, PIPE>(s_buf, s_tab, nit, lane, pp); break;
-    case 6: wgrad_v2_consumer<L, 6, PIPE>(s_buf, s_tab, nit, lane, pp); break;
-    default: wgrad_v2_consumer<L, 7, PIPE>(s_buf, s_tab, nit, lane, pp); break;
-  }
-}
-
-template <class L> constexpr size_t wgrad_v2_lds_bytes() {
+    case 0: wgrad_v2_consumer<L, 0, PIPE, BNB>(s_buf, s_tab, nit, lane, pp); break;
+    case 1: wgrad_v2_consumer<L, 1, PIPE, BNB>(s_buf, s_tab, nit, lane, pp); break;
+    case 2: wgrad_v2_consumer<L, 2, PIPE, BNB>(s_buf, s_tab, nit, lane, pp); break;
+    case 3: wgrad_v2_consumer<L, 3, PIPE, BNB>(s_buf, s_tab, nit, lane, pp); break;
+    case 4: wgrad_v2_consumer<L, 4, PIPE, BNB>(s_buf, s_tab, nit, lane, pp); break;
+    case 5: wgrad_v2_consumer<L, 5, PIPE, BNB>(s_buf, s_tab, nit, lane, pp); break;
+    case 6: wgrad_v2_consumer<L, 6, PIPE, BNB>(s_buf, s_tab, nit, lane, pp); break;
+    default: wgrad_v2_consumer<L, 7, PIPE, BNB>(s_buf, s_tab, nit, lane, pp); break;
+  }
+}
+
+template <class L> constexpr size_t wgrad_v2_lds_bytes(bool bnb = false) {
   constexpr bool gtab = !(L::S == 2 && L::HO % 4 == 0 && L::P == 1) && wgrad_v2_lds_floats<L>(true) * sizeof(float) <= 160 * 1024;
-  return sizeof(float) * wgrad_v2_lds_floats<L>(gtab);
-}
-
-}
+  return sizeof(float) * wgrad_v2_lds_floats<L>(gtab, bnb);
+}
+
+}
diff --git a/vae-gp-ode_amd/csrc/gp_launch.hpp b/vae-gp-ode_amd/csrc/gp_launch.hpp
--- a/vae-gp-ode_amd/csrc/gp_launch.hpp
+++ b/vae-gp-ode_amd/csrc/gp_launch.hpp
@@ -171,6 +171,16 @@
 int bn_bwd_apply(const float* x, const float* gy, const float* gamma, const float* beta, const float* save_mean, const float* save_invstd,
                  const float* gathered, const float* wts, int W, float count, float* gx, float* ggamma, float* gbeta, float* gx_chansum, int B, int C, int HW, int relu,
                  float* scratch, hipStream_t st);
+int bn_bwd_sums_split(const float* x, const float* gy, const float* gamma, const float* beta, const float* save_mean, const float* save_invstd,
+                      float* ggamma, float* gbeta, int B, int C, int HW, int relu, float* scratch, hipStream_t st);
+int bn_bwd_nsplit(int B);
+int conv2d_fwd_bnb(const float* g, const float* x, const float* gamma, const float* beta, const float* save_mean, const float* save_invstd,
+                   const float* bn_part, float count, const float* w, float* y, int B, int Ci, int H, int W, int Co, int K, int S, int P,
+                   int Ho, int Wo, hipStream_t st);
+int conv2d_bwd_weight_bnb(const float* g, const float* x, const float* gamma, const float* beta, const float* save_mean,
+                          const float* save_invstd, const float* bn_part, float count, const float* a, const float* a_bn, float* gw,
+                          float* gbias, float* scratch, int B, int Ci, int H, int W, int Co, int K, int S, int P, int Ho, int Wo,
+                          hipStream_t st);
 int bn_eval(const float* x, const float* gy, const float* gamma, const float* beta, const float* running_mean, const float* running_var,
             float eps, float* out, int B, int C, int HW, int relu, hipStream_t st);
 int bn_eval_table(const float* gamma, const float* beta, const float* running_mean, const float* running_var, float eps, float* table, int C,
diff --git a/vae-gp-ode_amd/csrc/vae_conv_tiled.hip b/vae-gp-ode_amd/csrc/vae_conv_tiled.hip
--- a/vae-gp-ode_amd/csrc/vae_conv_tiled.hip
+++ b/vae-gp-ode_amd/csrc/vae_conv_tiled.hip
@@ -707,4 +707,39 @@
   return -1;
 }
 
-}
+int conv_v2_dec4_bwd_data_bnb(const float* g, const BnBwdArgs& bn, const float* w, float* gx, int B, hipStream_t st);
+int wgrad_v2_dec4_bnb(const float* x, const float* g, const BnBwdArgs& bn, float* gw, float* gbias, float* scratch, float* part_b, int B,
+                      hipStream_t st, const float* in_bn);
+
+static int bnb_refusal(const char* who, int B, int Ci, int H, int W, int Co, int K, int S, int P, int Ho, int Wo, float count) {
+  if (B < 1) return set_error("%s: B >= 1", who);
+  if (!(count >= 1.f)) return set_error("%s: count is the number of elements per channel behind the sums, got %g", who, (double)count);
+  if (H != W || Ho != Wo || !matches<Dec4>(Ci, Co, H, Ho, K, S, P))
+    return set_error("%s: built for decnn.4's geometry only (gy (B, 32, 13, 13), K 5, stride 2, padding 1, 64 x 6 x 6 on the other side)", who);
+  if (!use_mfma()) return set_error("%s: matrix-core kernels only (GPODE_CONV_VALU is set)", who);
+  if (conv_v1()) return set_error("%s: second convolution engine only (GPODE_CONV_V1 is set)", who);
+  return 0;
+}
+
+int conv2d_fwd_bnb(const float* g, const float* x, const float* gamma, const float* beta, const float* save_mean, const float* save_invstd,
+                   const float* bn_part, float count, const float* w, float* y, int B, int Ci, int H, int W, int Co, int K, int S, int P,
+                   int Ho, int Wo, hipStream_t st) {
+  if (bnb_refusal("gpode_conv2d_fwd_bnb", B, Ci, H, W, Co, K, S, P, Ho, Wo, count)) return 1;
+  if (!aligned16(g, x, w, y)) return set_error("gpode_conv2d_fwd_bnb: g / x / w / y must be 16-byte aligned");
+  const BnBwdArgs bn{x, gamma, beta, save_mean, save_invstd, bn_part, bn_bwd_nsplit(B), count};
+  return conv_v2_dec4_bwd_data_bnb(g, bn, w, y, B, st);
+}
+
+int conv2d_bwd_weight_bnb(const float* g, const float* x, const float* gamma, const float* beta, const float* save_mean,
+                          const float* save_invstd, const float* bn_part, float count, const float* a, const float* a_bn, float* gw,
+                          float* gbias, float* scratch, int B, int Ci, int H, int W, int Co, int K, int S, int P, int Ho, int Wo,
+                          hipStream_t st) {
+  if (bnb_refusal("gpode_conv2d_bwd_weight_bnb", B, Ci, H, W, Co, K, S, P, Ho, Wo, count)) return 1;
+  if (!aligned16(g, x, a, a_bn)) return set_error("gpode_conv2d_bwd_weight_bnb: g / x / a / a_bn must be 16-byte aligned");
+  static_assert(256 * Dec4::CO <= 64 * Dec4::CI * 2, "the workgroups' channel sums fit the tail of the weight-gradient scratch");
+  float* part_b = scratch + (size_t)(B < 512 ? B : 512) * Co * Ci * K * K;
+  const BnBwdArgs bn{x, gamma, beta, save_mean, save_invstd, bn_part, bn_bwd_nsplit(B), count};
+  return wgrad_v2_dec4_bnb(a, g, bn, gw, gbias, scratch, part_b, B, st, a_bn);
+}
+
+}
diff --git a/vae-gp-ode_amd/csrc/vae_conv_v2.hip b/vae-gp-ode_amd/csrc/vae_conv_v2.hip
--- a/vae-gp-ode_amd/csrc/vae_conv_v2.hip
+++ b/vae-gp-ode_amd/csrc/vae_conv_v2.hip
@@ -7,13 +7,14 @@
 
 namespace gp {
 
-template <class L> static int launch_bwd_data_v2(const float* gy, const float* w, float* gx, int B, hipStream_t st, const char* what) {
+template <class L, bool BNB = false>
+static int launch_bwd_data_v2(const float* gy, const float* w, float* gx, int B, hipStream_t st, const char* what, const BnBwdArgs& bn = BnBwdArgs{}) {
   using E = BdV2<L>;
-  constexpr size_t lds = E::lds_bytes();
+  constexpr size_t lds = E::lds_bytes(BNB);
   static_assert(lds <= 160 * 1024, "LDS budget");
-  auto km = k_conv_bwd_data_v2<L>;
+  auto km = k_conv_bwd_data_v2<L, BNB>;
   if (set_max_lds((const void*)km, lds)) return 1;
-  hipLaunchKernelGGL(km, B < num_cus() ? B : num_cus(), E::NTHR, lds, st, gy, w, gx, B);
+  hipLaunchKernelGGL(km, B < num_cus() ? B : num_cus(), E::NTHR, lds, st, gy, w, gx, B, bn);
   return check_launch(what);
 }
 
@@ -23,6 +24,10 @@
 
 int conv_v2_dec4_bwd_data(const float* gy, const float* w, float* gx, int B, hipStream_t st) {
   return launch_bwd_data_v2<Dec4>(gy, w, gx, B, st, "conv_v2_dec4_bwd_data");
+}
+
+int conv_v2_dec4_bwd_data_bnb(const float* g, const BnBwdArgs& bn, const float* w, float* gx, int B, hipStream_t st) {
+  return launch_bwd_data_v2<Dec4, true>(g, w, gx, B, st, "conv_v2_dec4_bwd_data_bnb", bn);
 }
 
 template <class L, bool HAS_BN, bool STATS>
diff --git a/vae-gp-ode_amd/csrc/vae_norm.hip b/vae-gp-ode_amd/csrc/vae_norm.hip
--- a/vae-gp-ode_amd/csrc/vae_norm.hip
+++ b/vae-gp-ode_amd/csrc/vae_norm.hip
@@ -45,14 +45,6 @@
   if (threadIdx.x < NV) dst[threadIdx.x] = (red[0][threadIdx.x] + red[1][threadIdx.x]) + (red[2][threadIdx.x] + red[3][threadIdx.x]);
 }
 
-__device__ __forceinline__ void split_sums(const float* __restrict__ part, int nsplit, int C, int c, float& a, float& b) {
-  const int lane = threadIdx.x & 63;
-  const float in2[2] = {lane < nsplit ? part[((size_t)lane * C + c) * 2] : 0.f, lane < nsplit ? part[((size_t)lane * C + c) * 2 + 1] : 0.f};
-  float out2[2];
-  wave_sum_multi<2>(in2, out2);
-  a = out2[0];
-  b = out2[1];
-}
 
 __device__ __forceinline__ float chan_shift(const float* __restrict__ x, int HW, int c) {
   const int n = HW < 64 ? HW : 64, lane = threadIdx.x & 63;
@@ -185,12 +177,9 @@
     sa = out2[0];
     sb = out2[1];
   }
-  const float ic = 1.f / count, ca = sa * ic, cb = sb * ic, sc = g * is;
-  auto one = [&](float xv, float gv) {
-    const float xh = bn_xhat(xv, m, is);
-    if (relu && !(__fmaf_rn(xh, g, bt) > 0.f)) gv = 0.f;
-    return sc * (gv - ca - xh * cb);
-  };
+  float ca, cb, sc;
+  bn_bwd_consts(sa, sb, count, g, is, ca, cb, sc);
+  auto one = [&](float xv, float gv) { return bn_bwd_gx(xv, gv, m, is, g, bt, ca, cb, sc, relu); };
   float s0 = 0.f, t0 = 0.f;
   chan_slab(C, HW, c, b0, nb,
             [&](size_t i) {
@@ -432,6 +421,13 @@
   if (threadIdx.x == 0) { out[2 * blockIdx.x] = a; out[2 * blockIdx.x + 1] = b; }
 }
 
+__global__ __launch_bounds__(64) void k_reduce_affine(const float* __restrict__ part, int nsplit, int C, float* __restrict__ ggamma,
+                                                      float* __restrict__ gbeta) {
+  float a, b;
+  split_sums(part, nsplit, C, blockIdx.x, a, b);
+  if (threadIdx.x == 0) { gbeta[blockIdx.x] = a; ggamma[blockIdx.x] = b; }
+}
+
 struct Split { int ns, bps, used; };
 inline Split pick(int B) {
   Split s;
@@ -538,6 +534,17 @@
   hipLaunchKernelGGL(k_reduce_chan2, C, 64, 0, st, scratch, sp.used, C, sums);
   return check_launch("bn_bwd_sums");
 }
+
+int bn_bwd_sums_split(const float* x, const float* gy, const float* gamma, const float* beta, const float* save_mean, const float* save_invstd,
+                      float* ggamma, float* gbeta, int B, int C, int HW, int relu, float* scratch, hipStream_t st) {
+  if (B < 1 || C < 1 || HW < 1) return set_error("gpode_bn_bwd_sums_split: B, C, HW >= 1");
+  if ((HW & 3) == 0 && !(aligned16(x) && aligned16(gy))) return set_error("gpode_bn_bwd_sums_split: x / gy must be 16-byte aligned");
+  const Split sp = pick(B);
+  hipLaunchKernelGGL(k_bn_bwd_sums, dim3(C, sp.used), 256, 0, st, x, gy, gamma, beta, save_mean, save_invstd, B, C, HW, sp.bps, relu, scratch);
+  hipLaunchKernelGGL(k_reduce_affine, C, 64, 0, st, scratch, sp.used, C, ggamma, gbeta);
+  return check_launch("bn_bwd_sums_split");
+}
+int bn_bwd_nsplit(int B) { return pick(B).used; }
 
 int bn_bwd_apply(const float* x, const float* gy, const float* gamma, const float* beta, const float* save_mean, const float* save_invstd,
                  const float* gathered, const float* wts, int W, float count, float* gx, float* ggamma, float* gbeta, float* gx_chansum, int B, int C, int HW, int relu,
diff --git a/vae-gp-ode_amd/csrc/vae_wgrad_v2.hip b/vae-gp-ode_amd/csrc/vae_wgrad_v2.hip
--- a/vae-gp-ode_amd/csrc/vae_wgrad_v2.hip
+++ b/vae-gp-ode_amd/csrc/vae_wgrad_v2.hip
@@ -14,11 +14,28 @@
   auto kb = k_convT_wgrad_v2<L, true, PIPE>;
   if (set_max_lds((const void*)km, lds) || set_max_lds((const void*)kb, lds)) return 1;
   const int nwg = B < num_cus() ? B : num_cus();
-  if (in_bn) hipLaunchKernelGGL(kb, nwg, 768, lds, st, x, gy, scratch, B, in_bn);
-  else hipLaunchKernelGGL(km, nwg, 768, lds, st, x, gy, scratch, B, in_bn);
+  if (in_bn) hipLaunchKernelGGL(kb, nwg, 768, lds, st, x, gy, scratch, B, in_bn, BnBwdArgs{}, (float*)nullptr);
+  else hipLaunchKernelGGL(km, nwg, 768, lds, st, x, gy, scratch, B, in_bn, BnBwdArgs{}, (float*)nullptr);
   const size_t n = (size_t)L::CI * L::CO * L::K * L::K;
   if (reduce_job(RedJob{scratch, gw, nwg, (int)n, 1, L::CI / 16, L::CO / 16, L::K * L::K}, st)) return 1;
   return check_launch("convT_wgrad_v2");
+}
+
+template <class L, bool PIPE>
+static int launch_wgrad_v2_bnb(const float* x, const float* g, const BnBwdArgs& bn, float* gw, float* gbias, float* scratch, float* part_b,
+                               int B, hipStream_t st, const float* in_bn) {
+  constexpr size_t lds = wgrad_v2_lds_bytes<L>(true);
+  static_assert(lds <= 160 * 1024, "LDS budget");
+  auto km = k_convT_wgrad_v2<L, false, PIPE, true>;
+  auto kb = k_convT_wgrad_v2<L, true, PIPE, true>;
+  if (set_max_lds((const void*)km, lds) || set_max_lds((const void*)kb, lds)) return 1;
+  const int nwg = B < num_cus() ? B : num_cus();
+  if (in_bn) hipLaunchKernelGGL(kb, nwg, 768, lds, st, x, g, scratch, B, in_bn, bn, gbias ? part_b : (float*)nullptr);
+  else hipLaunchKernelGGL(km, nwg, 768, lds, st, x, g, scratch, B, in_bn, bn, gbias ? part_b : (float*)nullptr);
+  const size_t n = (size_t)L::CI * L::CO * L::K * L::K;
+  const RedJob jobs[2] = {RedJob{scratch, gw, nwg, (int)n, 1, L::CI / 16, L::CO / 16, L::K * L::K}, RedJob{part_b, gbias, nwg, L::CO, 0, 0, 0, 0}};
+  if (reduce_jobs(jobs, gbias ? 2 : 1, st)) return 1;
+  return check_launch(in_bn ? "convT_wgrad_v2_bn_bnb" : "convT_wgrad_v2_bnb");
 }
 
 int wgrad_v2_dec7(const float* x, const float* gy, float* gw, float* scratch, int B, hipStream_t st, const float* in_bn) {
@@ -28,4 +45,9 @@
   return launch_wgrad_v2<Dec4, true>(x, gy, gw, scratch, B, st, in_bn);
 }
 
+int wgrad_v2_dec4_bnb(const float* x, const float* g, const BnBwdArgs& bn, float* gw, float* gbias, float* scratch, float* part_b, int B,
+                      hipStream_t st, const float* in_bn) {
+  return launch_wgrad_v2_bnb<Dec4, true>(x, g, bn, gw, gbias, scratch, part_b, B, st, in_bn);
 }
+
+}
diff --git a/vae-gp-ode_amd/vae_ops.py b/vae-gp-ode_amd/vae_ops.py
--- a/vae-gp-ode_amd/vae_ops.py
+++ b/vae-gp-ode_amd/vae_ops.py
@@ -203,6 +203,35 @@
         _bwd_call('gpode_dec10_bn_bwd_apply', *head, _ptr(gathered), _ptr(sync.weights(c.device)), sync.world,
                   ctypes.c_float(sync.count_all(B * 784)), _ptr(gc), _ptr(gg), _ptr(gb), _ptr(cs), B, _ptr(scratch), _stream(), keep=(scratch,))
     return gc, gg, gb, cs
+
+
+_BN_FOLD = os.environ.get('GPODE_BN_FOLD', '1') != '0'
+_BN_FOLD_GEOM = (32, 64, 5, 2, 1, 6, 6, 13, 13)
+_BN_TWO_PASS_MIN = 2048
+
+
+class _FoldSlot:
+    __slots__ = ('pending',)
+
+    def __init__(self):
+        self.pending = None
+
+
+def _fold_source(ctx, geom):
+    if not (_BN_FOLD and _bn_sync is None and geom == _BN_FOLD_GEOM and ctx.needs_input_grad[0] and ctx.needs_input_grad[8]
+            and os.environ.get('GPODE_CONV_V1', '0') != '1'):
+        return None
+    return _FoldSlot()
+
+
+def _fold_take(slot, gy):
+    if slot is None or slot.pending is None:
+        return None
+    p, slot.pending = slot.pending, None
+    if gy.data_ptr() != p[0].data_ptr() or gy.shape != p[0].shape:
+        raise _lib.GpodeError('the BatchNorm behind decnn.4 handed over an un-applied gradient, but another one arrived (the activation '
+                              'has a second consumer?): set GPODE_BN_FOLD=0')
+    return p
 
 
 fused_bias_grads = 0
@@ -346,6 +375,7 @@
     @staticmethod
     def forward(ctx, c, gamma, beta, running_mean, running_var, nbt, momentum, eps, w, b, stride, pad, out_pad, bn=None, stats_for=None):
         pre = getattr(c, '_gpode_bnstats', None)
+        slot = getattr(c, '_gpode_fold', None)
         c, w = _chk(c, 'c'), _chk(w, 'weight')
         B, Cin, Hi, Wi = c.shape
         _, Cout, K, _ = w.shape
@@ -368,13 +398,38 @@
                       _stream())
         ctx.save_for_backward(c, gamma, beta, mean, invstd, table, w)
         ctx.geom = (B, Cout, Ht, Wt, Cin, K, stride, pad, Hi, Wi, b is not None)
+        ctx.fold_to = slot if (slot is not None and _bn_sync is None and B * Hi * Wi > _BN_TWO_PASS_MIN
+                               and all(ctx.needs_input_grad[:3])) else None
+        ctx.fold = _fold_source(ctx, (Cout, Cin, K, stride, pad, Hi, Wi, Ht, Wt))
+        if ctx.fold is not None:
+            y._gpode_fold = ctx.fold
         return y
+
+    @staticmethod
+    def _backward_folded(ctx, p):
+        global fused_bias_grads
+        c, gamma, beta, mean, invstd, table, w = ctx.saved_tensors
+        B, Cout, Ht, Wt, Cin, K, S, P, Hi, Wi, has_b = ctx.geom
+        g, x, bgamma, bbeta, bmean, binvstd, part, count = p
+        head = (_ptr(g), _ptr(x), _ptr(bgamma), _ptr(bbeta), _ptr(bmean), _ptr(binvstd), _ptr(part), ctypes.c_float(count))
+        gw, gb, ws = _new(w.shape, c), (_new((Cout,), c) if has_b else None), _wgrad_scratch(B, Cout, Cin, K, c)
+        _bwd_call('gpode_conv2d_bwd_weight_bnb', *head, _ptr(c), _ptr(table), _ptr(gw), _ptr(gb), _ptr(ws),
+                  B, Cout, Ht, Wt, Cin, K, S, P, Hi, Wi, _stream(), keep=(ws,))
+        fused_bias_grads += int(has_b)
+        ga = _new(c.shape, c)
+        _lib.call('gpode_conv2d_fwd_bnb', *head, _ptr(w), _ptr(ga), B, Cout, Ht, Wt, Cin, K, S, P, Hi, Wi, _stream())
+        gc, gg, gbeta, cs = _bn_bwd(ctx.sync, c, ga, gamma, beta, mean, invstd, 1)
+        gc._gpode_chansum = cs
+        return gc, gg, gbeta, None, None, None, None, None, gw, gb, None, None, None, None, None
 
     @staticmethod
     def backward(ctx, gy):
         c, gamma, beta, mean, invstd, table, w = ctx.saved_tensors
         B, Cout, Ht, Wt, Cin, K, S, P, Hi, Wi, has_b = ctx.geom
         gy = gy.contiguous()
+        p = _fold_take(ctx.fold, gy)
+        if p is not None:
+            return _BnReluConvT._backward_folded(ctx, p)
         gw = gb = None
         last_stage = _dec10_fused and (Cout, Cin, K, S, P, Hi, Wi, Ht, Wt) == (1, 16, 5, 1, 2, 28, 28, 28, 28)
         gw_rides = last_stage and ctx.needs_input_grad[8] and c.data_ptr() % 16 == 0
@@ -397,6 +452,12 @@
         else:
             ga = _new(c.shape, c)
             _lib.call('gpode_conv2d_fwd', _ptr(gy), _ptr(w), _ptr(None), _ptr(ga), B, Cout, Ht, Wt, Cin, K, S, P, Hi, Wi, _stream())
+            if ctx.fold_to is not None and ctx.sync is None and not c._backward_hooks and not c.retains_grad:
+                gg, gbeta, bs = _new((Cin,), c), _new((Cin,), c), _bn_scratch(B, Cin, c)
+                _lib.call('gpode_bn_bwd_sums_split', _ptr(c), _ptr(ga), _ptr(gamma), _ptr(beta), _ptr(mean), _ptr(invstd), _ptr(gg), _ptr(gbeta),
+                          B, Cin, Hi * Wi, 1, _ptr(bs), _stream())
+                ctx.fold_to.pending = (ga, c, gamma, beta, mean, invstd, bs, float(B * Hi * Wi))
+                return ga, gg, gbeta, None, None, None, None, None, gw, gb, None, None, None, None, None
             gc, gg, gbeta, cs = _bn_bwd(ctx.sync, c, ga, gamma, beta, mean, invstd, 1)
         gc._gpode_chansum = cs
         return gc, gg, gbeta, None, None, None, None, None, gw, gb, None, None, None, None, None
```
